# michalfratczak/habdec

Measured on AMD Instinct MI355X. Metric: IQ Msamples/s (batched 2.048 MS/s streams), higher is better.
Workload: dtype f32

## Files before the change

### habdec_amd/csrc/engine.cpp

```cpp
#include <hip/hip_runtime.h>
#include <rocfft/rocfft.h>

#include <algorithm>
#include <atomic>
#include <chrono>
#include <cmath>
#include <cstdio>
#include <cstdlib>
#include <cstring>
#include <memory>
#include <condition_variable>
#include <mutex>
#include <thread>
#include <string>
#include <vector>

#include "../../include/habdec_amd.h"
#include "dev_types.h"
#include "host/afc_tracker.hpp"
#include "host/decim_plan.hpp"
#include "host/fir_design.hpp"
#include "host/iq_file_batch.hpp"
#include "host/text_stage.hpp"
#include "host/tune_host.hpp"
#include "kernels/launch.h"

#define HDK(fn, ...) (e->fast ? hd::fast::fn(__VA_ARGS__) : hd::exact::fn(__VA_ARGS__))

namespace {

thread_local std::string g_err;
int fail(int code, const std::string& msg) { g_err = msg; return code; }

#define HD_HIP(call)                                                                                   \
    do {                                                                                               \
        hipError_t e_ = (call);                                                                        \
        if (e_ != hipSuccess) return fail(HD_ERR_DEVICE, std::string(#call) + ": " + hipGetErrorString(e_)); \
    } while (0)

template <typename T>
struct DevBuf {
    T* p = nullptr;
    size_t n = 0;
    hipError_t alloc(size_t count)
    {
        n = count;
        hipError_t e = hipMalloc(reinterpret_cast<void**>(&p), std::max<size_t>(count, 1) * sizeof(T));
        if (e == hipSuccess) e = hipMemset(p, 0, std::max<size_t>(count, 1) * sizeof(T));
        return e;
    }
    ~DevBuf() { if (p) (void)hipFree(p); }
};
template <typename T>
struct PinBuf {
    T* p = nullptr;
    T* dev = nullptr;
    size_t n = 0;
    hipError_t alloc(size_t count)
    {
        n = count;
        hipError_t e = hipHostMalloc(reinterpret_cast<void**>(&p), std::max<size_t>(count, 1) * sizeof(T), hipHostMallocMapped | hipHostMallocCoherent);
        if (e == hipSuccess) std::memset(p, 0, std::max<size_t>(count, 1) * sizeof(T));
        if (e == hipSuccess) e = hipHostGetDevicePointer(reinterpret_cast<void**>(&dev), p, 0);
        return e;
    }
    ~PinBuf() { if (p) (void)hipHostFree(p); }
};

struct SizeState {
    size_t stage_buf[2] = {0, 0};
    size_t pending = 0;
    size_t fft_fill = 0;
    size_t fir_buf = 0;
    uint32_t fir_T_run = 0;
    uint32_t head_n = 0;
    uint64_t head_call = ~0ull;
    bool head_aside = false;
    uint32_t tune_phase = 0;
    uint32_t front_phase = 0;
    uint32_t win_ub = 0, inflight_m = 0;
    uint32_t last_n2 = 0, last_pend_before = 0, last_m = 0;
    int last_buf = 0;
};

struct StreamHost {
    double baud = 300;
    float lp_bw = 1500, lp_trans = 0.025f;
    bool dc = false;
    hd::LowpassDesigner lp;
    bool taps_dirty = false;
    uint32_t tune_step = 0;
    uint32_t held = 0;
    bool sym_reset = true;
    hd::TextStage text;
    hd::AfcTracker afc;
    hd::SpectrumStats stats{};
    bool have_spectrum = false;
    uint64_t spectra = 0;
    uint32_t last_nbits = 0, last_nflips = 0;
    uint64_t flip_list_full = 0;
    uint64_t bits_total = 0;
    std::vector<uint32_t> last_words;
    uint32_t demod_ck[2] = {0, 0}, demod_ck_n = 0xFFFFFFFFu;
    uint64_t demod_ck_call = 0;
    uint64_t demod_ck_hash = 0xCBF29CE484222325ull;
    uint64_t demod_ck_calls = 0, demod_ck_unknown = 0;
    double tune_hz = 0;
    uint64_t tune_from = 0, retunes = 0;
    bool auto_afc = false;
    double afc_hold_s = 6.0, afc_min_hz = 100.0;
    uint64_t afc_elapsed = 0;
    double front_hz = 0;
    uint32_t front_step = 0;
    uint64_t front_from = 0;
};

}

struct hd_engine {
    hd_engine_config cfg{};
    double fs = 0, fsd = 0;
    std::vector<hd::DecimStage> stages;
    uint32_t S = 0, D = 1;
    uint32_t n1_cap = 0, n2_cap = 0;
    uint32_t taps_cap = 0, fir_hist_cap = 0;
    size_t fbuf_stride = 0;
    uint32_t tail_cap = 0, backlog_cap = 0, slot_words = 0, flips_cap = 0, max_R = 0, min_R = 4;
    int bins_sep = 8;
    bool decode_enabled = true;
    bool fast = false;
    bool one_stream = false;
    bool no_tail = false;
    uint32_t tail_max_n2 = 2048;
    int last_route = -1;
    struct PendingTail { bool valid = false; hd::TailArgs ta{}; int slot = 0; int r2 = 0, t2 = 0; } pend;
    DevBuf<float2> fft_tw;
    bool no_claim = false;
    uint32_t step_run = 0;
    bool no_cu_step = false;
    uint32_t ring_run = 0;
    uint32_t ring_short_pct = 25;
    static constexpr uint32_t kS1Loaders = 2;
#ifndef HD_S1_SLOTS_BATCH
#define HD_S1_SLOTS_BATCH 4
#endif
    static constexpr uint32_t kS1Slots = HD_S1_SLOTS_BATCH;
    PinBuf<unsigned int> ring_gave_up;
    std::string fail_cause;
    bool device_failed = false;
    uint64_t step_launches = 0;
    DevBuf<unsigned int> step_ctr;
    uint32_t pend_max_taps = 0;
    bool dec_wgs_forced = false;
#ifdef HD_TIMING_EXPERIMENT
    int cu_exp = 0;
#else
    static constexpr int cu_exp = 0;
#endif
    uint32_t n_cus = 0, dec_wgs_per_cu = 0;
    hipStream_t qa = nullptr, qb = nullptr, qc = nullptr;
    hipStream_t qh = nullptr;
    DevBuf<float2> staging2;
    hipEvent_t ev_copy[2] = {nullptr, nullptr}, ev_staging_free[2] = {nullptr, nullptr};
    bool staging_used[2] = {false, false};
    uint64_t host_calls = 0, host_calls_in_place = 0;
    uint32_t timing_every = 8;
    hd_timing last_timing{};
    static constexpr uint32_t kLpFftMinTaps = 1024;
    uint32_t lpf_N[2] = {0, 0};
    rocfft_plan lpf_fwd[2] = {nullptr, nullptr}, lpf_inv[2] = {nullptr, nullptr};
    rocfft_execution_info lpf_info = nullptr;
    DevBuf<char> lpf_workbuf;
    DevBuf<float2> lpf_x, lpf_k;
    PinBuf<uint32_t> lpf_ntaps;
    uint32_t lpf_k_N = 0;
    bool lpf_k_stale = true;
    uint64_t lpf_calls = 0;

    DevBuf<float2> staging, dec1, dec1b, dec1c, hist1[2], hist2[2], fbuf[3], fft_in, spec, filtered;
    DevBuf<float> stage_taps[2], lp_taps, power, demod, tail, weight;
    DevBuf<unsigned long long> flipmask;
    DevBuf<uint32_t> flips_dbg;
    DevBuf<hd::SymState> d_symstate;
    DevBuf<hd::DemodCarry> carry[2];
    DevBuf<float2> fir_head;
    DevBuf<float> tune_tab;
    DevBuf<uint32_t> demod_ck_acc;
    uint32_t head_cap = 0;
    DevBuf<hd::SymbolParams> d_sym;
    PinBuf<hd::SymbolParams> h_sym;
    static constexpr int kSlots = 4;
    struct CallSlot {
        DevBuf<hd::StreamCall> d_call;
        PinBuf<hd::StreamCall> h_call;
        PinBuf<uint32_t> h_slots;
        PinBuf<hd::SpectrumStatsDev> h_stats;
        PinBuf<uint2> h_tune;
        PinBuf<uint2> h_front;
        bool timed = false, timed_step = false;
        hipEvent_t ev_front = nullptr, ev_done = nullptr, ev_params = nullptr, ev_spec = nullptr, t0 = nullptr, t1 = nullptr, t2 = nullptr, t3 = nullptr;
        bool busy = false;
        uint32_t seq = 0;
        uint64_t total_in = 0;
        uint32_t r1 = 1;
        ~CallSlot() { for (hipEvent_t ev : {ev_front, ev_done, ev_params, ev_spec, t0, t1, t2, t3}) if (ev) (void)hipEventDestroy(ev); }
    } slot[kSlots];
    uint64_t calls = 0;
    uint64_t delivered = 0;
    int cur = 0;
    int hist_cur = 0;
    int carry_cur = 0;
    bool sym_dirty = true;

    std::vector<StreamHost> st;
    std::vector<SizeState> mirror, mirror_next;
    std::recursive_mutex mtx;
    bool in_callback = false;
    hd_sentence_cb sentence_cb = nullptr; void* sentence_user = nullptr;
    hd_match_cb match_cb = nullptr; void* match_user = nullptr;
    hd_chars_cb chars_cb = nullptr; void* chars_user = nullptr;
    uint64_t sentences_ok = 0;

    ~hd_engine()
    {
        for (rocfft_plan pl : {lpf_fwd[0], lpf_fwd[1], lpf_inv[0], lpf_inv[1]}) if (pl) rocfft_plan_destroy(pl);
        if (lpf_info) rocfft_execution_info_destroy(lpf_info);
        if (qa) (void)hipStreamDestroy(qa);
        if (qb && qb != qa) (void)hipStreamDestroy(qb);
        if (qc && qc != qa) (void)hipStreamDestroy(qc);
        if (qh) (void)hipStreamDestroy(qh);
        for (hipEvent_t ev : {ev_copy[0], ev_copy[1], ev_staging_free[0], ev_staging_free[1]}) if (ev) (void)hipEventDestroy(ev);
    }
};

namespace {

std::once_flag g_rocfft_once;

hd::SymbolParams symbol_params(const hd_engine* e, const StreamHost& s)
{
    hd::SymbolParams p{};
    p.float_abs = e->cfg.lookup_mode ? 1u : 0u;
    p.min_held = 0xFFFFFFFFu;
    p.spb = 0; p.R = 4;
    if (e->fsd > 0 && s.baud > 0) {
        const double spb = std::round(e->fsd / s.baud);
        if (spb >= 1 && spb < 1e9) {
            p.spb = (uint32_t)spb;
            p.R = (uint32_t)std::max(4, int(p.spb / 4));
            p.min_held = (uint32_t)std::ceil(e->fsd / s.baud * 3);
        }
    }
    return p;
}

float cutoff_rel(const hd_engine* e, const StreamHost& s) { return (float)(s.lp_bw / e->fsd); }

int check_stream(const hd_engine* e, uint32_t s)
{
    if (!e) return fail(HD_ERR_INVALID, "null engine");
    if (s >= e->S) return fail(HD_ERR_INVALID, "stream index out of range");
    return HD_OK;
}

}

extern "C" {

const char* hd_last_error(void) { return g_err.c_str(); }

uint32_t hd_min_chunk(uint32_t decimation)
{
    std::vector<hd::DecimStage> st;
    if (!hd::decim_plan(decimation, st)) return 0;
    uint64_t need = decimation ? decimation : 1;
    uint64_t r = 1;
    for (const auto& g : st) { need = std::max<uint64_t>(need, (uint64_t)(g.taps.size() - 1) * r); r *= (uint64_t)g.ratio; }
    const uint64_t d = decimation ? decimation : 1;
    return (uint32_t)((need + d - 1) / d * d);
}

void hd_engine_config_default(hd_engine_config* c)
{
    std::memset(c, 0, sizeof(*c));
    c->device = 0; c->n_streams = 1; c->max_chunk = 65536; c->sampling_rate = 2.048e6; c->decimation = 64;
    c->baud = 300; c->rtty_bits = 8; c->rtty_stops = 2; c->lowpass_bw_hz = 1500; c->lowpass_trans = 0.025f;
    c->dc_remove = 0; c->lookup_mode = 1; c->enable_spectrum = 1; c->ungated = 0; c->keep_filtered = 0; c->pipeline = 0; c->arith = HD_ARITH_EXACT;
}

int hd_engine_create(const hd_engine_config* cfg, hd_engine** out)
{
    if (!cfg || !out) return fail(HD_ERR_INVALID, "null argument");
    *out = nullptr;
    if (cfg->n_streams < 1) return fail(HD_ERR_INVALID, "n_streams must be >= 1");
    if (!(cfg->sampling_rate > 0)) return fail(HD_ERR_INVALID, "sampling_rate must be > 0");
    if (cfg->max_chunk < 1) return fail(HD_ERR_INVALID, "max_chunk must be >= 1");
    if (cfg->arith != HD_ARITH_EXACT && cfg->arith != HD_ARITH_FAST) return fail(HD_ERR_INVALID, "arith must be HD_ARITH_EXACT (0) or HD_ARITH_FAST (1)");
    std::unique_ptr<hd_engine> e(new hd_engine);
    e->cfg = *cfg;
    e->fast = cfg->arith == HD_ARITH_FAST;
    if (!hd::decim_plan(cfg->decimation, e->stages))
        return fail(HD_ERR_INVALID, "Unsupported decimation factor: " + std::to_string(cfg->decimation));
    e->S = cfg->n_streams;
    e->D = cfg->decimation;
    if (cfg->max_chunk % e->D) return fail(HD_ERR_INVALID, "max_chunk must be a multiple of the decimation factor");
    e->fs = (double)(float)cfg->sampling_rate;
    e->fsd = e->fs / (double)e->D;
    e->decode_enabled = cfg->ungated || !(e->fsd > 4 * 40e3);
    if (cfg->baud > 0 && e->fsd / cfg->baud < 3.5)
        return fail(HD_ERR_UNSUPPORTED, "symbol rate above a third of the decimated rate (fewer than 4 samples per bit): the symbol extractor's windows would overlap");
    {
        const float rel = (float)(500.0f / e->fsd);
        e->bins_sep = std::max(8, (int)std::round((double)rel * (double)hd::kFftBins));
    }

    int ndev = 0;
    if (hipGetDeviceCount(&ndev) != hipSuccess || ndev <= cfg->device || cfg->device < 0)
        return fail(HD_ERR_DEVICE, "no HIP device " + std::to_string(cfg->device) + " (this library has no CPU path)");
    HD_HIP(hipSetDevice(cfg->device));
    HD_HIP(hipStreamCreateWithFlags(&e->qa, hipStreamNonBlocking));
    e->one_stream = cfg->pipeline == 0;
    e->no_tail = getenv("HD_NO_TAIL") != nullptr;
    e->no_claim = getenv("HD_NO_CLAIM") != nullptr;
    if (const char* v = getenv("HD_STEP_RUN")) e->step_run = (uint32_t)atoi(v);
    e->no_cu_step = getenv("HD_NO_CU_STEP") != nullptr;
    if (const char* v = getenv("HD_RING_RUN")) e->ring_run = (uint32_t)atoi(v);
    if (const char* v = getenv("HD_RING_SHORT_PCT")) e->ring_short_pct = std::min<uint32_t>((uint32_t)atoi(v), 100u);
    if (const char* v = getenv("HD_TAIL_MAX_N2")) e->tail_max_n2 = (uint32_t)strtoul(v, nullptr, 0);
    {
        hipDeviceProp_t prop;
        HD_HIP(hipGetDeviceProperties(&prop, cfg->device));
        e->n_cus = (uint32_t)prop.multiProcessorCount;
        e->dec_wgs_per_cu = cfg->pipeline ? 6u : 8u;
        if (const char* v = getenv("HD_DEC_WGS_PER_CU")) { e->dec_wgs_per_cu = (uint32_t)atoi(v); e->dec_wgs_forced = true; }
#ifdef HD_TIMING_EXPERIMENT
        if (const char* v = getenv("HD_CU_EXP")) e->cu_exp = atoi(v);
#endif
    }
    for (hipEvent_t* ev : {&e->ev_copy[0], &e->ev_copy[1], &e->ev_staging_free[0], &e->ev_staging_free[1]}) HD_HIP(hipEventCreateWithFlags(ev, hipEventDisableTiming));
    if (e->one_stream) e->qb = e->qc = e->qa;
    else {
        if (!e->qb) HD_HIP(hipStreamCreateWithFlags(&e->qb, hipStreamNonBlocking));
        HD_HIP(hipStreamCreateWithFlags(&e->qc, hipStreamNonBlocking));
    }
    for (auto& sl : e->slot) {
        static const unsigned ev_flags = (unsigned)hipEventDisableSystemFence;
        HD_HIP(hipEventCreateWithFlags(&sl.ev_front, hipEventDisableTiming | ev_flags));
        HD_HIP(hipEventCreateWithFlags(&sl.ev_done, hipEventDisableTiming | ev_flags));
        HD_HIP(hipEventCreateWithFlags(&sl.ev_params, hipEventDisableTiming | ev_flags));
        HD_HIP(hipEventCreateWithFlags(&sl.ev_spec, hipEventDisableTiming | ev_flags));
        for (hipEvent_t* ev : {&sl.t0, &sl.t1, &sl.t2, &sl.t3}) HD_HIP(hipEventCreateWithFlags(ev, ev_flags));
    }

    const uint32_t S = e->S;
    const uint32_t r0 = e->stages.size() > 0 ? e->stages[0].ratio : 1;
    e->n1_cap = cfg->max_chunk / r0;
    e->n2_cap = cfg->max_chunk / e->D;
    const uint32_t m_cap = ((e->n2_cap + hd::kFirBatch - 1) / hd::kFirBatch) * hd::kFirBatch + hd::kFirBatch;
    e->taps_cap = (m_cap | 1u) + 1u;
    e->fir_hist_cap = (e->taps_cap + 1u) & ~1u;
    e->fbuf_stride = (size_t)e->fir_hist_cap + hd::kFirBatch + e->n2_cap + 2;
    e->fbuf_stride = (e->fbuf_stride + 1) & ~(size_t)1;
    e->backlog_cap = hd::kVentLimit + 1 + m_cap;
    e->tail_cap = 1u;
    while (e->tail_cap < hd::kVentLimit + 1 + m_cap + 1024) e->tail_cap <<= 1;

    e->st.resize(S);
    e->mirror.resize(S);
    e->mirror_next.resize(S);
    for (auto& s : e->st) {
        s.baud = cfg->baud; s.lp_bw = cfg->lowpass_bw_hz; s.lp_trans = cfg->lowpass_trans; s.dc = cfg->dc_remove != 0;
        s.text.framer.nbits = cfg->rtty_bits; s.text.framer.nstops = cfg->rtty_stops;
        s.lp.float_trig = cfg->lookup_mode != 0;
    }
    {
        const hd::SymbolParams p = symbol_params(e.get(), e->st[0]);
        const uint32_t spb = std::max<uint32_t>(p.spb, 1);
        uint32_t bits = 3u * e->backlog_cap / spb + 64u;
        bits = std::max<uint32_t>(256u, (bits + 31u) & ~31u);
        e->slot_words = (uint32_t)(sizeof(hd::BitsHeader) / 4) + bits / 32;
        e->max_R = std::max<uint32_t>(p.R, 4);
        e->min_R = e->max_R;
    }
    e->flips_cap = cfg->keep_filtered ? 256 : 0;

    HD_HIP(e->staging.alloc((size_t)S * cfg->max_chunk));
    if (e->stages.size() == 2) for (auto* b : {&e->dec1, &e->dec1b, &e->dec1c}) HD_HIP(b->alloc((size_t)S * e->n1_cap));
    HD_HIP(e->step_ctr.alloc(2 * 16 * 32 + 32));
    HD_HIP(e->ring_gave_up.alloc(4));
    e->ring_gave_up.p[0] = 0;
    if (!e->no_claim && e->n_cus % 32u == 0) {
        const uint32_t n_xcd = e->n_cus / 32u;
        HD_HIP(hipDeviceSynchronize());
        const uint32_t seen = HDK(probe_xcc_mask, e->qa, e->n_cus, e->step_ctr.p + 2 * 16 * 32);
        if (n_xcd > 16 || seen != (n_xcd >= 32 ? 0xFFFFFFFFu : (1u << n_xcd) - 1u)) e->no_claim = true;
    } else
        e->no_claim = true;
    if (e->stages.size() >= 1) {
        for (auto& h : e->hist1) HD_HIP(h.alloc((size_t)S * (e->stages[0].taps.size() - 1)));
        HD_HIP(e->stage_taps[0].alloc(e->stages[0].taps.size() + 1));
        HD_HIP(hipMemcpy(e->stage_taps[0].p, e->stages[0].taps.data(), e->stages[0].taps.size() * 4, hipMemcpyHostToDevice));
    }
    if (e->stages.size() == 2) {
        for (auto& h : e->hist2) HD_HIP(h.alloc((size_t)S * (e->stages[1].taps.size() - 1)));
        HD_HIP(e->stage_taps[1].alloc(e->stages[1].taps.size() + 1));
        HD_HIP(hipMemcpy(e->stage_taps[1].p, e->stages[1].taps.data(), e->stages[1].taps.size() * 4, hipMemcpyHostToDevice));
    }
    for (auto& b : e->fbuf) HD_HIP(b.alloc((size_t)S * e->fbuf_stride));
    HD_HIP(e->lp_taps.alloc((size_t)S * e->taps_cap));
    HD_HIP(e->demod.alloc((size_t)S * m_cap));
    if (cfg->keep_filtered) HD_HIP(e->filtered.alloc((size_t)S * m_cap));
    HD_HIP(e->tail.alloc((size_t)S * e->tail_cap));
    HD_HIP(e->weight.alloc((size_t)S * e->tail_cap));
    HD_HIP(e->flipmask.alloc((size_t)S * (e->tail_cap / 64)));
    HD_HIP(e->d_symstate.alloc(S));
    if (e->flips_cap) HD_HIP(e->flips_dbg.alloc((size_t)S * e->flips_cap));
    for (auto& c : e->carry) HD_HIP(c.alloc(S));
    e->head_cap = std::min<uint32_t>(e->taps_cap, 8192u);
    HD_HIP(e->fir_head.alloc((size_t)S * e->head_cap));
    HD_HIP(e->demod_ck_acc.alloc((size_t)2 * S));
    HD_HIP(e->d_sym.alloc(S));
    HD_HIP(e->h_sym.alloc(S));
    for (auto& sl : e->slot) {
        HD_HIP(sl.d_call.alloc(S));
        HD_HIP(sl.h_call.alloc(S));
        HD_HIP(sl.h_slots.alloc((size_t)S * e->slot_words));
        HD_HIP(sl.h_tune.alloc(S));
        HD_HIP(sl.h_front.alloc(S));
    }
    {
        std::vector<float> tab(4 * hd::kTuneTable);
        hd::tune_tables(tab.data(), tab.data() + 2 * hd::kTuneTable);
        HD_HIP(e->tune_tab.alloc(tab.size()));
        HD_HIP(hipMemcpy(e->tune_tab.p, tab.data(), tab.size() * sizeof(float), hipMemcpyHostToDevice));
    }
    if (cfg->enable_spectrum) {
        HD_HIP(e->fft_in.alloc((size_t)S * hd::kFftBins));
        HD_HIP(e->spec.alloc((size_t)S * hd::kFftBins));
        HD_HIP(e->power.alloc((size_t)S * hd::kFftBins));
        for (auto& sl : e->slot) HD_HIP(sl.h_stats.alloc(S));
        {
            std::vector<float2> tw(hd::kFftBins);
            for (size_t m = 0; m < hd::kFftBins; ++m) {
                const double a = 2.0 * 3.14159265358979323846264338327950288 * (double)m / (double)hd::kFftBins;
                tw[m] = make_float2((float)std::cos(a), (float)-std::sin(a));
            }
            HD_HIP(e->fft_tw.alloc(hd::kFftBins));
            HD_HIP(hipMemcpy(e->fft_tw.p, tw.data(), tw.size() * sizeof(float2), hipMemcpyHostToDevice));
        }
    }
    if (e->fast && e->taps_cap >= hd_engine::kLpFftMinTaps && getenv("HD_NO_LP_FFT") == nullptr) {
        std::call_once(g_rocfft_once, [] { rocfft_setup(); });
        uint32_t N = 1;
        while (N < m_cap + e->taps_cap) N <<= 1;
        e->lpf_N[1] = N; e->lpf_N[0] = N / 2;
        size_t wmax = 0;
        for (int w = 0; w < 2; ++w) {
            const size_t len = e->lpf_N[w];
            if (rocfft_plan_create(&e->lpf_fwd[w], rocfft_placement_inplace, rocfft_transform_type_complex_forward, rocfft_precision_single, 1, &len, S, nullptr) != rocfft_status_success ||
                rocfft_plan_create(&e->lpf_inv[w], rocfft_placement_inplace, rocfft_transform_type_complex_inverse, rocfft_precision_single, 1, &len, S, nullptr) != rocfft_status_success)
                return fail(HD_ERR_DEVICE, "rocfft_plan_create (low-pass transforms) failed");
            for (rocfft_plan pl : {e->lpf_fwd[w], e->lpf_inv[w]}) { size_t wsz = 0; rocfft_plan_get_work_buffer_size(pl, &wsz); wmax = std::max(wmax, wsz); }
        }
        if (rocfft_execution_info_create(&e->lpf_info) != rocfft_status_success) return fail(HD_ERR_DEVICE, "rocfft_execution_info_create failed");
        if (wmax) { HD_HIP(e->lpf_workbuf.alloc(wmax)); rocfft_execution_info_set_work_buffer(e->lpf_info, e->lpf_workbuf.p, wmax); }
        HD_HIP(e->lpf_x.alloc((size_t)S * N));
        HD_HIP(e->lpf_k.alloc((size_t)S * N));
        HD_HIP(e->lpf_ntaps.alloc(S));
    }
    {
        hd_engine::CallSlot& sl = e->slot[0];
        hipStream_t q = e->qa;
        const uint32_t T1 = e->stages.size() > 0 ? (uint32_t)e->stages[0].taps.size() : 0, T2 = e->stages.size() > 1 ? (uint32_t)e->stages[1].taps.size() : 0;
        if (e->stages.empty()) HDK(launch_passthrough, q, S, 1, e->staging.p, cfg->max_chunk, e->fbuf[0].p, e->fbuf_stride, sl.d_call.p, e->fir_hist_cap);
        if (e->stages.size() >= 1)
            HDK(launch_decimate, q, e->stages[0].ratio, T1, S, 1, e->staging.p, cfg->max_chunk, e->hist1[0].p, e->hist1[1].p, e->stage_taps[0].p,
                                e->stages.size() == 1 ? e->fbuf[0].p : e->dec1.p, e->stages.size() == 1 ? e->fbuf_stride : e->n1_cap, sl.d_call.p, 0,
                                e->stages.size() == 1, e->fir_hist_cap, nullptr);
        if (e->stages.size() >= 1)
            HDK(launch_decimate_tuned, q, e->stages[0].ratio, T1, S, 1, e->staging.p, cfg->max_chunk, e->hist1[0].p, e->hist1[1].p, e->stage_taps[0].p,
                                      e->stages.size() == 1 ? e->fbuf[0].p : e->dec1.p, e->stages.size() == 1 ? e->fbuf_stride : e->n1_cap, sl.d_call.p,
                                      e->stages.size() == 1, e->fir_hist_cap, nullptr, 0u, sl.h_front.dev, e->tune_tab.p);
        if (e->stages.size() == 2)
            HDK(launch_decimate, q, e->stages[1].ratio, T2, S, 1, e->dec1.p, e->n1_cap, e->hist2[0].p, e->hist2[1].p, e->stage_taps[1].p, e->fbuf[0].p,
                                e->fbuf_stride, sl.d_call.p, 1, 1, e->fir_hist_cap, nullptr);
        HDK(launch_chunk_post, q, S, e->fbuf[0].p, e->fbuf_stride, sl.d_call.p, e->fir_hist_cap, nullptr, e->tune_tab.p);
        if (cfg->enable_spectrum) {
            HDK(launch_fft_feed, q, S, e->fbuf[0].p, e->fbuf_stride, e->fft_in.p, sl.d_call.p, e->fir_hist_cap);
            hd::launch_spectrum_wave(q, S, e->fft_in.p, e->fft_tw.p, e->spec.p, e->power.p, sl.h_stats.dev, sl.d_call.p, e->fsd, e->bins_sep, 0u);
        }
        HDK(launch_fir_demod, q, S, 0, 0, e->fbuf[0].p, e->fbuf_stride, e->lp_taps.p, e->taps_cap, e->demod.p, e->demod.n / S, nullptr, e->carry[0].p,
                             e->carry[1].p, sl.d_call.p, e->fir_hist_cap, e->tail.p, e->tail_cap, e->d_symstate.p, e->fbuf[1].p,
                             e->fir_head.p, e->head_cap, e->fbuf[2].p);
        HDK(launch_symbols, q, S, 1, 1, e->max_R, e->tail.p, e->tail_cap, e->d_symstate.p, e->flipmask.p, e->weight.p, e->d_sym.p, sl.d_call.p,
                           sl.h_slots.dev, e->slot_words, nullptr, 0, e->min_R, 0u);
        HD_HIP(hipStreamSynchronize(q));
        HD_HIP(hipGetLastError());
        for (auto& h : e->hist1) if (h.p) HD_HIP(hipMemset(h.p, 0, h.n * sizeof(float2)));
        for (auto& h : e->hist2) if (h.p) HD_HIP(hipMemset(h.p, 0, h.n * sizeof(float2)));
        for (auto& c : e->carry) HD_HIP(hipMemset(c.p, 0, c.n * sizeof(hd::DemodCarry)));
        HD_HIP(hipMemset(e->d_symstate.p, 0, S * sizeof(hd::SymState)));
        if (const char* b0 = getenv("HD_SYM_BASE0")) {
            hd::SymState st0{};
            st0.base = st0.cached = st0.run_pos = (uint32_t)strtoul(b0, nullptr, 0);
            std::vector<hd::SymState> v(S, st0);
            HD_HIP(hipMemcpy(e->d_symstate.p, v.data(), S * sizeof(hd::SymState), hipMemcpyHostToDevice));
        }
    }
    HD_HIP(hipDeviceSynchronize());
    *out = e.release();
    return HD_OK;
}

void hd_engine_destroy(hd_engine* e)
{
    if (!e) return;
    (void)hipSetDevice(e->cfg.device);
    (void)hipDeviceSynchronize();
    delete e;
}

uint32_t hd_engine_streams(const hd_engine* e) { return e ? e->S : 0; }
uint32_t hd_engine_decimation(const hd_engine* e) { return e ? e->D : 0; }
double hd_engine_decimated_rate(const hd_engine* e) { return e ? e->fsd : 0; }
uint64_t hd_engine_sentences_ok(const hd_engine* e) { return e ? e->sentences_ok : 0; }
void hd_engine_set_timing(hd_engine* e, int on) { if (e) e->timing_every = on < 0 ? 0u : (uint32_t)on; }
int hd_engine_timing(hd_engine* e, hd_timing* out)
{
    if (!e || !out) return fail(HD_ERR_INVALID, "null argument");
    *out = e->last_timing;
    out->host_calls_in_place = e->host_calls_in_place;
    out->lowpass_fft_calls = e->lpf_calls;
    return HD_OK;
}

extern "C" int hd_debug_step_counters(hd_engine* e, unsigned int* out32)
{
    if (!e || !out32) return HD_ERR_INVALID;
    std::vector<unsigned int> h(2 * 16 * 32);
    if (hipDeviceSynchronize() != hipSuccess || hipMemcpy(h.data(), e->step_ctr.p, h.size() * 4, hipMemcpyDeviceToHost) != hipSuccess) return HD_ERR_DEVICE;
    for (int i = 0; i < 32; ++i) out32[i] = h[(size_t)i * 32];
    return HD_OK;
}

void hd_set_sentence_callback(hd_engine* e, hd_sentence_cb cb, void* user) { if (e) { e->sentence_cb = cb; e->sentence_user = user; } }
void hd_set_match_callback(hd_engine* e, hd_match_cb cb, void* user) { if (e) { e->match_cb = cb; e->match_user = user; } }
void hd_set_chars_callback(hd_engine* e, hd_chars_cb cb, void* user) { if (e) { e->chars_cb = cb; e->chars_user = user; } }


int hd_stream_set_baud(hd_engine* e, uint32_t s, double baud)
{
    if (int r = check_stream(e, s)) return r;
    std::lock_guard<std::recursive_mutex> l(e->mtx);
    if (baud > 0 && e->fsd / baud < 3.5)
        return fail(HD_ERR_UNSUPPORTED, "symbol rate above a third of the decimated rate (fewer than 4 samples per bit): the symbol extractor's windows would overlap");
    StreamHost probe = e->st[s];
    probe.baud = baud;
    const hd::SymbolParams p = symbol_params(e, probe);
    if (p.spb) {
        const uint32_t need = 3u * e->backlog_cap / p.spb + 64u;
        if (need > (e->slot_words - sizeof(hd::BitsHeader) / 4) * 32)
            return fail(HD_ERR_CAPACITY, "baud too high for the result slots sized at engine creation");
        if (p.R > e->max_R) e->max_R = p.R;
        if (p.R < e->min_R) e->min_R = std::max<uint32_t>(p.R, 4);
    }
    e->st[s].baud = baud;
    e->st[s].sym_reset = true;
    e->sym_dirty = true;
    return HD_OK;
}
int hd_stream_set_rtty(hd_engine* e, uint32_t s, uint32_t bits, float stops)
{
    if (int r = check_stream(e, s)) return r;
    std::lock_guard<std::recursive_mutex> l(e->mtx);
    e->st[s].text.framer.nbits = bits;
    e->st[s].text.framer.nstops = stops;
    return HD_OK;
}
int hd_stream_set_lowpass_bw(hd_engine* e, uint32_t s, float hz)
{
    if (int r = check_stream(e, s)) return r;
    std::lock_guard<std::recursive_mutex> l(e->mtx);
    StreamHost& st = e->st[s];
    st.lp_bw = hz;
    if (st.lp.design(cutoff_rel(e, st), st.lp_trans)) st.taps_dirty = true;
    return HD_OK;
}
int hd_stream_set_lowpass_trans(hd_engine* e, uint32_t s, float trans)
{
    if (int r = check_stream(e, s)) return r;
    std::lock_guard<std::recursive_mutex> l(e->mtx);
    StreamHost& st = e->st[s];
    st.lp_trans = trans;
    if (st.lp.design(cutoff_rel(e, st), st.lp_trans)) st.taps_dirty = true;
    return HD_OK;
}
int hd_stream_set_dc_remove(hd_engine* e, uint32_t s, int on)
{
    if (int r = check_stream(e, s)) return r;
    std::lock_guard<std::recursive_mutex> l(e->mtx);
    e->st[s].dc = on != 0;
    return HD_OK;
}
int hd_stream_reset_frequency_correction(hd_engine* e, uint32_t s, double c)
{
    if (int r = check_stream(e, s)) return r;
    std::lock_guard<std::recursive_mutex> l(e->mtx);
    e->st[s].afc.reset(c, hd::kFftBins, e->fsd);
    return HD_OK;
}
int hd_stream_set_tune(hd_engine* e, uint32_t s, double offset_hz)
{
    if (int r = check_stream(e, s)) return r;
    std::lock_guard<std::recursive_mutex> l(e->mtx);
    uint32_t d = 0;
    if (!hd::tune_step(offset_hz, e->fsd, &d)) return fail(HD_ERR_INVALID, "tuning offset outside (-fs_dec/2, fs_dec/2)");
    StreamHost& st = e->st[s];
    st.tune_hz = offset_hz; st.tune_step = d; st.tune_from = e->calls;
    if (offset_hz == 0) e->mirror[s].tune_phase = 0;
    return HD_OK;
}
int hd_stream_set_front_tune(hd_engine* e, uint32_t s, double offset_hz)
{
    if (int r = check_stream(e, s)) return r;
    std::lock_guard<std::recursive_mutex> l(e->mtx);
    if (e->stages.empty()) return fail(HD_ERR_UNSUPPORTED, "an engine without a decimation stage has no input-rate tuning: hd_stream_set_tune is the same thing there");
    uint32_t d = 0;
    if (!hd::tune_step(offset_hz, e->fs, &d)) return fail(HD_ERR_INVALID, "tuning offset outside (-fs/2, fs/2)");
    StreamHost& st = e->st[s];
    st.front_hz = offset_hz; st.front_step = d; st.front_from = e->calls;
// ... 55 lines not shown
    if (!sl.busy) return HD_OK;
    if (e->pend.valid && &e->slot[e->pend.slot] == &sl) { if (const int r = run_pending_tail(e)) return r; }
    const auto w0 = std::chrono::steady_clock::now();
    HD_HIP(hipEventSynchronize(sl.ev_done));
    const auto w1 = std::chrono::steady_clock::now();
    sl.busy = false;
    if (sl.timed) {
        float a = 0, b = 0;
        HD_HIP(hipEventElapsedTime(&b, sl.t1, sl.t2));
        if (sl.timed_step) a = b; else HD_HIP(hipEventElapsedTime(&a, sl.t0, sl.t3));
        e->last_timing.ms_total = a;
        e->last_timing.ms_front = b;
        e->last_timing.samples = sl.total_in;
        e->last_timing.front_bytes = sl.total_in * 8 + (sl.total_in / sl.r1) * 8;
        ++e->last_timing.timed_calls;
    }
    int rc = HD_OK;
    {
        const auto t_lim = std::chrono::steady_clock::now() + std::chrono::milliseconds(200);
        const bool timing_experiment = e->cu_exp != 0;
        auto await = [&](const volatile uint32_t* tag, const char* what, uint32_t s) {
            for (uint32_t spins = 0; *tag != sl.seq; ++spins) {
                if (std::chrono::steady_clock::now() > t_lim) {
                    e->device_failed = true;
                    e->fail_cause = std::string(what) + " of stream " + std::to_string(s) + " does not carry its call's tag 200 ms after the completion event";
                    rc = fail(HD_ERR_DEVICE, e->fail_cause + ": the results of this engine are unreliable -- destroy the engine");
                    return;
                }
                if (spins > 64u) std::this_thread::yield();
            }
        };
        for (uint32_t s = 0; s < e->S && !e->device_failed && !timing_experiment; ++s) {
            await(&reinterpret_cast<const volatile hd::BitsHeader*>(sl.h_slots.p + (size_t)s * e->slot_words)->seq, "result slot", s);
            if (!e->device_failed && e->cfg.enable_spectrum && sl.h_stats.p && sl.h_call.p[s].fft_run)
                await(reinterpret_cast<const volatile uint32_t*>(&sl.h_stats.p[s].seq), "spectrum statistics", s);
        }
        std::atomic_thread_fence(std::memory_order_acquire);
    }
    if (e->ring_gave_up.p && e->ring_gave_up.p[0] && !e->device_failed) {
        e->device_failed = true;
        e->fail_cause = "k_stage1_cu (loader / consumer waves): a bounded wait ran out inside a launch (word " + std::to_string(e->ring_gave_up.p[0]) + ")";
    }
    if (e->device_failed && rc == HD_OK)
        rc = fail(HD_ERR_DEVICE, e->fail_cause + ": the results of this and of every later call of this engine are unreliable -- destroy the engine");
    if (e->device_failed) {
        e->last_timing.host_wait_us = std::chrono::duration<double, std::micro>(w1 - w0).count();
        e->last_timing.host_text_us = 0;
        return rc;
    }
    for (uint32_t s = 0; s < e->S; ++s) {
        StreamHost& st = e->st[s];
        const hd::StreamCall& c = sl.h_call.p[s];
        if (c.fft_run) {
            std::memcpy(&st.stats, &sl.h_stats.p[s], sizeof(st.stats));
            st.have_spectrum = true;
            ++st.spectra;
        }
        const bool past_batch_gate = c.fir_m || c.clear_pending;
        if (past_batch_gate && e->cfg.enable_spectrum) st.afc.step(st.have_spectrum, st.stats, hd::kFftBins, e->fsd);
        st.afc_elapsed += c.n_in;
        if (st.auto_afc && (double)st.afc_elapsed >= st.afc_hold_s * e->fs && std::abs(st.afc.correction) > st.afc_min_hz) {
            const double corr = st.afc.correction;
            uint32_t d = 0;
            if (hd::tune_step(st.tune_hz + corr, e->fsd, &d)) {
                st.tune_hz += corr; st.tune_step = d; st.tune_from = e->calls;
                if (!d) e->mirror[s].tune_phase = 0;
                st.afc.reset(corr, hd::kFftBins, e->fsd);
                st.afc_elapsed = 0;
                ++st.retunes;
            }
        }
        const uint32_t* slot = sl.h_slots.p + (size_t)s * e->slot_words;
        const hd::BitsHeader* hdr = reinterpret_cast<const hd::BitsHeader*>(slot);
        SizeState& sz = e->mirror[s];
        st.held = hdr->held_after;
        sz.inflight_m -= c.fir_m;
        sz.win_ub = hdr->uncached + sz.inflight_m;
        st.last_nbits = hdr->nbits; st.last_nflips = hdr->nflips;
        st.bits_total += hdr->nbits;
        st.demod_ck[0] = hdr->demod_ck[0]; st.demod_ck[1] = hdr->demod_ck[1]; st.demod_ck_n = hdr->demod_n; st.demod_ck_call = e->delivered;
        if (hdr->demod_n != 0xFFFFFFFFu) {
            for (const uint32_t x : {hdr->demod_n, hdr->demod_ck[0], hdr->demod_ck[1]}) st.demod_ck_hash = (st.demod_ck_hash ^ x) * 0x100000001B3ull;
            ++st.demod_ck_calls;
        } else ++st.demod_ck_unknown;
        if (hdr->overflow & 1u) rc = fail(HD_ERR_CAPACITY, "symbol result slot overflow on stream " + std::to_string(s));
        if (hdr->overflow & 2u) ++st.flip_list_full;
        const uint32_t* words = slot + sizeof(hd::BitsHeader) / 4;
        st.last_words.assign(words, words + (hdr->nbits + 31) / 32);
        if (!c.fir_m) continue;
        if (hdr->nbits) st.text.framer.push_packed(words, hdr->nbits);
        const std::string chars = st.text.run(hdr->nbits != 0, [&](const hd::SentenceMatch& m) {
            ++e->sentences_ok;
            if (e->sentence_cb) { e->in_callback = true; e->sentence_cb(e->sentence_user, s, m.callsign.c_str(), m.data.c_str(), m.crc.c_str()); e->in_callback = false; }
        }, [&](const hd::SentenceMatch& m, bool ok) {
            if (e->match_cb) { e->in_callback = true; e->match_cb(e->match_user, s, m.callsign.c_str(), m.data.c_str(), m.crc.c_str(), ok ? 1 : 0); e->in_callback = false; }
        });
        if (!chars.empty() && e->chars_cb) { e->in_callback = true; e->chars_cb(e->chars_user, s, chars.data(), chars.size()); e->in_callback = false; }
    }
    e->last_timing.host_wait_us = std::chrono::duration<double, std::micro>(w1 - w0).count();
    e->last_timing.host_text_us = std::chrono::duration<double, std::micro>(std::chrono::steady_clock::now() - w1).count();
    return rc;
}

int deliver(hd_engine* e, uint64_t depth)
{
    int rc = HD_OK;
    while (e->calls - e->delivered > depth) {
        if (const int r = collect(e, e->slot[e->delivered % hd_engine::kSlots])) rc = r;
        ++e->delivered;
    }
    return rc;
}

int flush_locked(hd_engine* e)
{
    if (e->delivered < e->calls) { if (const int r = run_pending_tail(e)) return r; }
    return deliver(e, 0);
}


enum class Route : uint32_t {
    separate = 0,
    tail = 2,
    step = 3,
};

struct CallPlan {
    size_t nst = 0;
    uint32_t R1 = 1, R2 = 1, T1 = 0, T2 = 0;
    uint32_t max_in = 0, min_in = 0xFFFFFFFFu, max_n1 = 0, max_n2 = 0, max_m = 0, max_taps = 0, max_new = 0, max_pend = 0;
    uint64_t total_in = 0;
    bool any_fft = false, any_dc = false, any_zero1 = false, any_tune = false, any_lp_restart = false;
    bool any_front = false;
};

struct CallRoute {
    Route route = Route::separate;
    int tail_lanes = 64;
    hd::TailArgs ta{}, ta_step{};
    bool lean = false, free_front = false, host_params = false, any_post = false, spectrum_on_qc = false;
    const hd::StreamCall* dcall = nullptr;
    float2* feed = nullptr;
};

struct CallBufs {
    float2 *fcur, *fnext, *fprev, *d1;
    int hin, hout, cin, cout;
};

CallBufs call_bufs(const hd_engine* e)
{
    CallBufs b;
    b.fcur = e->fbuf[e->cur].p; b.fnext = e->fbuf[(e->cur + 1) % 3].p; b.fprev = e->fbuf[(e->cur + 2) % 3].p;
    b.d1 = (e->calls % 3 == 0) ? e->dec1.p : (e->calls % 3 == 1) ? e->dec1b.p : e->dec1c.p;
    b.hin = e->hist_cur; b.hout = e->hist_cur ^ 1;
    b.cin = e->carry_cur; b.cout = e->carry_cur ^ 1;
    return b;
}

int plan_call(hd_engine* e, hd_engine::CallSlot& sl, const uint32_t* n_per_stream, uint32_t n_uniform, CallPlan& p, bool& redesigned)
{
    p = CallPlan{};
    p.nst = e->stages.size();
    if (p.nst > 0) { p.R1 = e->stages[0].ratio; p.T1 = (uint32_t)e->stages[0].taps.size(); }
    if (p.nst > 1) { p.R2 = e->stages[1].ratio; p.T2 = (uint32_t)e->stages[1].taps.size(); }
    redesigned = false;
    for (uint32_t s = 0; s < e->S; ++s) {
        StreamHost& st = e->st[s];
        SizeState& nx = e->mirror_next[s];
        nx = e->mirror[s];
        hd::StreamCall c{};
        const uint32_t n = n_per_stream ? n_per_stream[s] : n_uniform;
        c.n_in = n;
        c.n1 = n / p.R1;
        c.n2 = c.n1 / p.R2;
        if (n) {
            if (p.nst > 0) { const size_t want = (size_t)n + p.T1 + p.R1; if (nx.stage_buf[0] < want) { nx.stage_buf[0] = want; c.zero_hist1 = 1; } }
            if (p.nst > 1) { const size_t want = (size_t)c.n1 + p.T2 + p.R2; if (nx.stage_buf[1] < want) { nx.stage_buf[1] = want; c.zero_hist2 = 1; } }
        }
        c.dc_remove = st.dc && c.n2;
        sl.h_tune.p[s] = make_uint2(st.tune_step, nx.tune_phase);
        if (st.tune_step) { p.any_tune = true; nx.tune_phase += c.n2 * st.tune_step; }
        sl.h_front.p[s] = make_uint2(st.front_step, nx.front_phase);
        if (st.front_step | nx.front_phase) { p.any_front = true; nx.front_phase += n * st.front_step; }
        c.pend_before = (uint32_t)nx.pending;
        nx.pending += c.n2;
        c.fft_fill = (uint32_t)nx.fft_fill;
        if (e->cfg.enable_spectrum && n && nx.fft_fill < (size_t)hd::kFftBins && c.n2) {
            c.fft_take = (uint32_t)std::min<size_t>(hd::kFftBins - nx.fft_fill, c.n2);
            nx.fft_fill += c.fft_take;
        }
        if (e->cfg.enable_spectrum && n && nx.fft_fill >= (size_t)hd::kFftBins) { c.fft_run = 1; nx.fft_fill = 0; p.any_fft = true; }
        const bool past_batch_gate = n && nx.pending >= hd::kFirBatch;
        nx.last_m = 0;
        if (past_batch_gate && !e->decode_enabled) { c.clear_pending = 1; nx.pending = 0; }
        else if (past_batch_gate) {
            const uint32_t m = (uint32_t)(nx.pending - nx.pending % hd::kFirBatch);
            st.lp.batch = m;
            if (st.lp.design(cutoff_rel(e, st), st.lp_trans)) {
                st.taps_dirty = true;
                redesigned = true;
            }
            const uint32_t T = (uint32_t)st.lp.taps.size();
            if (!T) return fail(HD_ERR_UNSUPPORTED, "low-pass transition width leaves no taps (reference filters nothing then)");
            if (T > e->taps_cap) return fail(HD_ERR_CAPACITY, "low-pass tap count exceeds engine capacity");
            if (nx.fir_buf < (size_t)m + T) { nx.fir_buf = (size_t)m + T; c.fir_zero_hist = 1; }
            c.fir_m = m; c.fir_taps = T;
            c.fir_taps_prev = hd::sc_pack_taps_prev(nx.fir_T_run ? nx.fir_T_run : T, nx.head_n, !nx.head_aside && nx.head_call + 1 == e->calls, false);
            nx.fir_T_run = T;
            nx.head_n = std::min<uint32_t>(m, std::min<uint32_t>(e->head_cap, 0x3FFFu)); nx.head_call = e->calls; nx.head_aside = false;
            nx.pending -= m;
            nx.last_m = m;
            p.max_m = std::max(p.max_m, m);
            p.max_taps = std::max(p.max_taps, T);
            p.any_lp_restart |= c.fir_zero_hist != 0;
            const uint32_t pending_windows = st.sym_reset ? std::max(st.held, nx.win_ub) : nx.win_ub;
            p.max_new = std::max(p.max_new, pending_windows + m + 64u);
            nx.inflight_m += m;
            nx.win_ub += m;
        }
        if (!c.fir_m && nx.head_n && !nx.head_aside) {
            if (nx.head_call + 1 == e->calls) c.fir_taps_prev = hd::sc_pack_taps_prev(0, nx.head_n, false, true);
            else nx.head_n = 0;
            nx.head_aside = true;
        }
        c.pend_after = (uint32_t)nx.pending;
        p.max_pend = std::max(p.max_pend, std::max(c.pend_before, c.pend_after));
        nx.last_n2 = c.n2; nx.last_pend_before = c.pend_before; nx.last_buf = e->cur;
        sl.h_call.p[s] = c;
        p.max_in = std::max(p.max_in, n); p.min_in = std::min(p.min_in, n); p.max_n1 = std::max(p.max_n1, c.n1); p.max_n2 = std::max(p.max_n2, c.n2);
        p.any_dc |= c.dc_remove != 0;
        p.any_zero1 |= c.zero_hist1 != 0;
        p.total_in += n;
    }
    sl.total_in = p.total_in;
    sl.r1 = p.R1;
    sl.seq = (uint32_t)(e->calls + 1u);
    if (!sl.seq) sl.seq = 1u;
    return HD_OK;
}

void route_call(hd_engine* e, hd_engine::CallSlot& sl, const CallPlan& p, CallRoute& r)
{
    const uint32_t S = e->S;
    const int R2 = (int)p.R2, T2 = (int)p.T2;
    r = CallRoute{};
    r.tail_lanes = S >= 2 * e->n_cus ? 64 : 256;
    const bool tail = p.nst == 2 && !p.any_dc && !e->no_tail && p.max_n2 <= e->tail_max_n2 &&
                      ((r.tail_lanes == 256 && p.max_n2 >= 512u && HDK(tail_layout, r.ta, r.tail_lanes, R2, T2, p.max_taps, e->max_R, e->min_R, e->tail_cap, p.max_pend, 64 * 1024, 4)) ||
                       HDK(tail_layout, r.ta, r.tail_lanes, R2, T2, p.max_taps, e->max_R, e->min_R, e->tail_cap, p.max_pend, 64 * 1024));
    const uint32_t step_lds = (p.R1 == 32 || p.R1 == 64) ? HDK(step_lds_bytes, (int)p.R1, (int)p.T1) : 0u;
    const bool step = tail && !p.any_front && e->cfg.pipeline && !e->one_stream && p.min_in == p.max_in && p.max_in && step_lds &&
                      HDK(tail_layout, r.ta_step, 64, R2, T2, p.max_taps, e->max_R, e->min_R, e->tail_cap, p.max_pend, step_lds);
    r.route = step ? Route::step : tail ? Route::tail : Route::separate;
    r.any_post = p.any_dc || (p.any_tune && !tail);
    r.lean = tail && !e->one_stream;
    r.free_front = !tail && p.nst == 2 && !e->one_stream;
    r.host_params = tail && !step && e->one_stream;
    r.dcall = r.host_params ? sl.h_call.dev : sl.d_call.p;
    r.feed = (e->cfg.enable_spectrum && !r.any_post) ? e->fft_in.p : nullptr;
    if (r.route != Route::separate || !e->cfg.enable_spectrum || r.any_post || !p.any_fft) return;
    for (uint32_t s = 0; s < S; ++s) {
        hd::StreamCall& c = sl.h_call.p[s];
        if (c.fft_run == 1 && c.fft_fill == 0 && c.fft_take == (uint32_t)hd::kFftBins) { c.fft_take = 0; c.fft_run = 2; }
    }
    r.spectrum_on_qc = !e->one_stream && p.nst != 0;
    for (uint32_t s = 0; s < S && r.spectrum_on_qc; ++s) r.spectrum_on_qc = sl.h_call.p[s].fft_run != 1u;
}

void fill_tail(const hd_engine* e, const hd_engine::CallSlot& sl, const CallPlan& p, const CallRoute& r, const CallBufs& b, hd::TailArgs& t)
{
    t.dec1 = b.d1; t.dec1_stride = e->n1_cap; t.hist2_in = e->hist2[b.hin].p; t.hist2_out = e->hist2[b.hout].p; t.taps2 = e->stage_taps[1].p;
    t.fbuf = b.fcur; t.fbuf_next = b.fnext; t.fbuf_stride = e->fbuf_stride; t.fir_hist_cap = e->fir_hist_cap;
    t.lp_taps = e->lp_taps.p; t.taps_stride = e->taps_cap; t.demod = e->demod.p; t.demod_stride = e->demod.n / e->S;
    t.filtered = e->cfg.keep_filtered ? e->filtered.p : nullptr; t.carry_in = e->carry[b.cin].p; t.carry_out = e->carry[b.cout].p;
    t.tune = p.any_tune ? sl.h_tune.dev : nullptr; t.tune_tab = e->tune_tab.p;
    t.call = r.dcall; t.fft_in = r.feed; t.head_buf = e->fir_head.p; t.fbuf_prev = b.fprev; t.head_cap = e->head_cap;
    t.n_streams = e->S;
    t.ring = e->tail.p; t.ring_cap = e->tail_cap; t.sym = e->d_symstate.p; t.flipmask = e->flipmask.p; t.wsum = e->weight.p;
    t.sp = e->d_sym.p; t.slots = sl.h_slots.dev; t.slot_words = e->slot_words; t.seq = sl.seq;
    t.flips_dbg = e->flips_cap ? e->flips_dbg.p : nullptr; t.flips_cap = e->flips_cap;
    t.fft_tw = r.feed ? e->fft_tw.p : nullptr;
    t.spec = e->spec.p; t.power = e->power.p; t.stats = sl.h_stats.dev; t.rate = e->fsd; t.bins_sep = e->bins_sep;
}

hd::StepClaim make_claim(const hd_engine* e, const CallPlan& p, uint32_t lin_wgs ,
                         uint32_t run_len_cu )
{
    hd::StepClaim claim{};
    const int R1 = (int)p.R1, T1 = (int)p.T1;
    const uint64_t S = e->S;
    const uint32_t ntiles = run_len_cu ? HDK(ring_tiles, R1, T1, p.max_in) : (p.max_n1 + 63) / 64, n_xcd = e->n_cus / 32u, run_len = run_len_cu ? run_len_cu : e->step_run >= 2 ? e->step_run : 4u;
    const uint64_t runs = S * ntiles / run_len;
    const bool shape_ok = run_len_cu ? (HDK(stage1_cu_supported, R1, T1) && p.max_in % 2048u == 0) : ((R1 == 32 || R1 == 64) && p.max_n1 % 64 == 0);
    if (!e->no_claim && (p.nst == 2 || (run_len_cu && p.nst == 1)) && shape_ok && p.min_in == p.max_in && p.max_in && !p.any_zero1 && n_xcd && e->n_cus % 32u == 0 && n_xcd <= 16 &&
        ntiles && (ntiles % run_len == 0 || (run_len_cu && R1 >= 32 && (S * ntiles) % run_len == 0)) && runs % n_xcd == 0 && S * ntiles < (1ull << 32) && (uint64_t)ntiles * S >= 4ull * lin_wgs) {
        claim.ctr = e->step_ctr.p + (size_t)(e->step_launches & 1u) * 16 * 32;
        claim.ctr_next = e->step_ctr.p + (size_t)((e->step_launches & 1u) ^ 1u) * 16 * 32;
        claim.n_xcd = n_xcd; claim.runs_per_xcd = (uint32_t)(runs / n_xcd); claim.run_len = run_len;
        if (run_len_cu && R1 >= 32 && e->ring_short_pct) {
            const uint32_t tpx = claim.runs_per_xcd * run_len, whole = (uint32_t)((uint64_t)tpx * (100u - e->ring_short_pct) / 100u) / run_len;
            claim.tiles_per_xcd = tpx; claim.short_from = whole; claim.runs_per_xcd = whole + (tpx - whole * run_len);
        }
    }
    return claim;
}

uint32_t pick_ring_run(const hd_engine* e, uint32_t R1, uint32_t ntiles)
{
    const uint64_t S = e->S;
    const uint32_t n_xcd = e->n_cus / 32u ? e->n_cus / 32u : 1u, want = R1 >= 32 ? 4u : 8u;
    auto ok = [&](uint32_t r) { return r >= 2u && r <= ntiles && (R1 >= 32 ? (S * ntiles) % r == 0 : ntiles % r == 0) && (S * ntiles / r) % n_xcd == 0; };
    if (e->ring_run >= 2 && ok(e->ring_run)) return e->ring_run;
    for (uint32_t d = 0; d <= 8u; ++d) {
        if (ok(want + d)) return want + d;
        if (d && d < want && ok(want - d)) return want - d;
    }
    return 2u;
}

int enqueue_uploads(hd_engine* e, hd_engine::CallSlot& sl, const CallRoute& r)
{
    const uint32_t S = e->S;
    hipStream_t qa = e->qa;
    if (e->last_route >= 0 && e->last_route != (int)r.route) {
        if (const int rc = run_pending_tail(e)) return rc;
        HD_HIP(hipStreamSynchronize(qa)); HD_HIP(hipStreamSynchronize(e->qb));
    }
    e->last_route = (int)r.route;
    e->last_timing.path = (uint32_t)r.route;
    if (!r.lean && !r.free_front && e->calls >= 2 && !e->one_stream) HD_HIP(hipStreamWaitEvent(qa, e->slot[(e->calls - 2) % hd_engine::kSlots].ev_done, 0));
    const bool step = r.route == Route::step;
    sl.timed = e->timing_every && (e->calls % e->timing_every) == 0;
    sl.timed_step = sl.timed && step;
    if (sl.timed && !step) HD_HIP(hipEventRecord(sl.t0, qa));
    if (!r.lean && !r.free_front && !r.host_params) {
        HDK(launch_fetch_params, e->qc, sl.h_call.dev, sl.d_call.p, S * sizeof(hd::StreamCall));
        if (!e->one_stream) { HD_HIP(hipEventRecord(sl.ev_params, e->qc)); HD_HIP(hipStreamWaitEvent(qa, sl.ev_params, 0)); }
    }
    for (uint32_t s = 0; s < S; ++s) {
        StreamHost& st = e->st[s];
        if (!st.taps_dirty) continue;
        HD_HIP(hipMemcpyAsync(e->lp_taps.p + (size_t)s * e->taps_cap, st.lp.taps.data(), st.lp.taps.size() * 4, hipMemcpyHostToDevice, qa));
        st.taps_dirty = false;
        e->lpf_k_stale = true;
    }
    if (e->sym_dirty) {
        uint32_t mr = 4;
        for (uint32_t s = 0; s < S; ++s) {
            e->h_sym.p[s] = symbol_params(e, e->st[s]);
            e->h_sym.p[s].reset = e->st[s].sym_reset ? 1u : 0u;
            mr = std::max(mr, e->h_sym.p[s].R);
        }
        e->max_R = mr;
        { uint32_t lo = mr; for (uint32_t s2 = 0; s2 < S; ++s2) lo = std::min(lo, std::max<uint32_t>(e->h_sym.p[s2].R, 4)); e->min_R = lo; }
        HD_HIP(hipMemcpyAsync(e->d_sym.p, e->h_sym.p, S * sizeof(hd::SymbolParams), hipMemcpyHostToDevice, qa));
        e->sym_dirty = false;
        for (uint32_t s = 0; s < S; ++s)
            if (e->st[s].sym_reset) { e->st[s].sym_reset = false; e->sym_dirty = true; }
    }
    return HD_OK;
}

int enqueue_step(hd_engine* e, hd_engine::CallSlot& sl, const CallPlan& p, CallRoute& r, const float2* iq, size_t stride)
{
    const uint32_t S = e->S;
    const int R1 = (int)p.R1, T1 = (int)p.T1, R2 = (int)p.R2, T2 = (int)p.T2;
    hipStream_t qa = e->qa;
    const CallBufs b = call_bufs(e);
    const uint32_t ring_nt = HDK(ring_tiles, R1, T1, p.max_in), ring_run = pick_ring_run(e, p.R1, ring_nt), n_xcd = e->n_cus / 32u;
    const bool runs_ok = ring_nt && n_xcd && ring_run >= 2u && ((uint64_t)S * ring_nt) % ring_run == 0 && ((uint64_t)S * ring_nt / ring_run) % n_xcd == 0;
    const bool cu_shape = !e->no_cu_step && !e->no_claim && !p.any_zero1 && p.max_in % 2048u == 0 && runs_ok && HDK(step_cu_supported, R1, T1, R2, T2);
    const uint32_t cu_tail = cu_shape ? HDK(step_cu_tail_lds, R1, T1) : 0u;
    if (cu_tail) {
        hd::TailArgs tacu{};
        if (HDK(tail_layout, tacu, 64, R2, T2, p.max_taps, e->max_R, e->min_R, e->tail_cap, p.max_pend, cu_tail)) r.ta_step = tacu;
    }
    fill_tail(e, sl, p, r, b, r.ta_step);
    hd_engine::PendingTail prev = e->pend;
    hd_engine::CallSlot* ps = prev.valid ? &e->slot[prev.slot] : nullptr;
    const int cu_exp = e->cu_exp;
    const bool want_cu = cu_tail && ((cu_exp & 1) || (r.ta_step.lds_bytes <= cu_tail && (!prev.valid || prev.ta.lds_bytes <= cu_tail)));
    const hd::StepClaim claim = make_claim(e, p, 0, want_cu ? ring_run : 0u);
    bool launched = false;
    if (want_cu && claim.ctr) {
        const uint32_t tb = std::max(r.ta_step.lds_bytes, prev.valid ? prev.ta.lds_bytes : 0u);
        hd::StepClaim cl = claim;
        if (cu_exp & 2) { cl.runs_per_xcd = 0; cl.tiles_per_xcd = 0; cl.short_from = 0xFFFFFFFFu; }
        launched = HDK(launch_step_cu, qa, R1, T1, prev.valid ? prev.r2 : R2, prev.valid ? prev.t2 : T2, S, e->n_cus, iq, stride,
                                      e->hist1[b.hin].p, e->hist1[b.hout].p, e->stage_taps[0].p, b.d1, e->n1_cap, sl.h_call.dev, sl.d_call.p, prev.ta,
                                      (prev.valid && !(cu_exp & 1)) ? S : 0u, p.max_in, cl, tb,
                                      sl.timed ? sl.t1 : nullptr, sl.timed ? sl.t2 : ps ? ps->ev_done : nullptr);
    }
    e->last_timing.step_variant = launched ? 1u : 0u;
    if (launched) ++e->step_launches;
    else {
        if (sl.timed) HD_HIP(hipEventRecord(sl.t1, qa));
        const hd::StepClaim fb = (want_cu && claim.ctr) ? hd::StepClaim{} : claim;
        const uint32_t wgs = (fb.ctr ? 8u : 32u) * e->n_cus;
        if (prev.valid && prev.ta.lds_bytes > HDK(step_lds_bytes, R1, T1)) {
            if (const int rc = run_pending_tail(e)) return rc;
            prev.valid = false; ps = nullptr;
        }
        if (!HDK(launch_step, qa, R1, T1, prev.valid ? prev.r2 : R2, prev.valid ? prev.t2 : T2, S, p.max_n1, iq, stride, e->hist1[b.hin].p,
                             e->hist1[b.hout].p, e->stage_taps[0].p, b.d1, e->n1_cap, sl.h_call.dev, sl.d_call.p, wgs, prev.ta, prev.valid ? S : 0u,
                             p.any_zero1 ? 0u : p.max_in, fb))
            return fail(HD_ERR_INVALID, "no step kernel for this decimation plan");
        if (fb.ctr) ++e->step_launches;
    }
    if (sl.timed && !launched) HD_HIP(hipEventRecord(sl.t2, qa));
    if (ps && (!launched || sl.timed)) HD_HIP(hipEventRecord(ps->ev_done, qa));
    HD_HIP(hipGetLastError());
    return HD_OK;
}

void call_spectrum(hd_engine* e, hipStream_t q, hd_engine::CallSlot& sl, const CallPlan& p, const CallRoute& r)
{
    if (!(e->cfg.enable_spectrum && p.max_n2)) return;
    const float2* fcur = e->fbuf[e->cur].p;
    if (r.any_post || p.nst == 0) HDK(launch_fft_feed, q, e->S, fcur, e->fbuf_stride, e->fft_in.p, r.dcall, e->fir_hist_cap);
    if (!p.any_fft) return;
    hd::launch_spectrum_wave(q, e->S, e->fft_in.p, e->fft_tw.p, e->spec.p, e->power.p, sl.h_stats.dev, r.dcall, e->fsd, e->bins_sep, sl.seq, fcur, e->fbuf_stride, e->fir_hist_cap);
}

int enqueue_front(hd_engine* e, hd_engine::CallSlot& sl, const CallPlan& p, const CallRoute& r, const float2* iq, size_t stride)
{
    const uint32_t S = e->S, R1 = p.R1, T1 = p.T1;
    const bool tail = r.route == Route::tail;
    hipStream_t qa = e->qa;
    const CallBufs b = call_bufs(e);
    if (p.nst == 0) {
        if (sl.timed) HD_HIP(hipEventRecord(sl.t1, qa));
        HDK(launch_passthrough, qa, S, p.max_in, iq, stride, b.fcur, e->fbuf_stride, r.dcall, e->fir_hist_cap);
        if (sl.timed) HD_HIP(hipEventRecord(sl.t2, qa));
    } else {
        const bool single = p.nst == 1;
        float2* out1 = single ? b.fcur : b.d1;
        const size_t out1_stride = single ? e->fbuf_stride : e->n1_cap;
        const uint32_t wgs_cu = (R1 == 64 && !e->dec_wgs_forced && e->dec_wgs_per_cu > 4u) ? 4u : e->dec_wgs_per_cu;
        const uint32_t lin1 = (p.min_in == p.max_in && p.max_in) ? wgs_cu * e->n_cus : 0u;
        bool s1_cu = false;
        if (!p.any_front && (single ? R1 == 4 : R1 != 4) && p.min_in == p.max_in && p.max_in && !e->no_cu_step && !p.any_zero1 && p.max_in % 2048u == 0 && HDK(stage1_cu_supported, (int)R1, (int)T1)) {
            const hd::StepClaim cl = make_claim(e, p, 0, pick_ring_run(e, R1, HDK(ring_tiles, (int)R1, (int)T1, p.max_in)));
            if (cl.ctr) {
                if (sl.timed) HD_HIP(hipEventRecord(sl.t1, qa));
                s1_cu = HDK(launch_stage1_cu, qa, (int)R1, (int)T1, e->n_cus, iq, stride, e->hist1[b.hin].p, e->hist1[b.hout].p, e->stage_taps[0].p, out1, out1_stride,
                                             p.max_in, cl, e->ring_gave_up.dev, hd_engine::kS1Loaders, 16u, (e->cfg.pipeline && !tail && !single) ? hd_engine::kS1Slots : 8u,
                                             single ? r.dcall : nullptr, e->fir_hist_cap, single ? r.feed : nullptr);
                if (s1_cu) ++e->step_launches;
            }
        }
        e->last_timing.step_variant = s1_cu ? 1u : 0u;
        if (!s1_cu) {
            if (sl.timed) HD_HIP(hipEventRecord(sl.t1, qa));
            const hd::StreamCall* call1 = (r.lean || r.free_front) ? sl.h_call.dev : r.dcall;
            if (!(p.any_front ? HDK(launch_decimate_tuned, qa, R1, T1, S, p.max_n1, iq, stride, e->hist1[b.hin].p, e->hist1[b.hout].p, e->stage_taps[0].p, out1, out1_stride,
                                                          call1, single ? 1 : 0, e->fir_hist_cap, single ? r.feed : nullptr, lin1, sl.h_front.dev, e->tune_tab.p)
                              : HDK(launch_decimate, qa, R1, T1, S, p.max_n1, iq, stride, e->hist1[b.hin].p, e->hist1[b.hout].p, e->stage_taps[0].p, out1, out1_stride,
                                                    call1, 0, single ? 1 : 0, e->fir_hist_cap, single ? r.feed : nullptr, lin1)))
                return fail(HD_ERR_INVALID, "no kernel for this decimation stage");
        }
        if (sl.timed) HD_HIP(hipEventRecord(sl.t2, qa));
        if (r.free_front) HDK(launch_fetch_params, qa, sl.h_call.dev, sl.d_call.p, S * sizeof(hd::StreamCall));
        if (!single && !tail) {
            if (!HDK(launch_decimate, qa, p.R2, p.T2, S, p.max_n2, b.d1, e->n1_cap, e->hist2[b.hin].p, e->hist2[b.hout].p, e->stage_taps[1].p, b.fcur,
                                     e->fbuf_stride, r.dcall, 1, 1, e->fir_hist_cap, r.feed))
                return fail(HD_ERR_INVALID, "no kernel for this decimation stage");
        }
    }
    if (!tail) {
        if (r.any_post) HDK(launch_chunk_post, qa, S, b.fcur, e->fbuf_stride, r.dcall, e->fir_hist_cap, p.any_tune ? sl.h_tune.dev : nullptr, e->tune_tab.p);
        if (!r.spectrum_on_qc) call_spectrum(e, qa, sl, p, r);
    }
    if (!e->one_stream) HD_HIP(hipEventRecord(sl.ev_front, qa));
    if (r.spectrum_on_qc) {
        HD_HIP(hipStreamWaitEvent(e->qc, sl.ev_front, 0));
        call_spectrum(e, e->qc, sl, p, r);
        HD_HIP(hipEventRecord(sl.ev_spec, e->qc));
    }
    return HD_OK;
}

int lowpass_transforms(hd_engine* e, const CallPlan& p, const CallRoute& r, const CallBufs& b, uint32_t* lpN)
{
    *lpN = 0;
    if (!e->fast || !e->lpf_N[1] || p.max_taps < hd_engine::kLpFftMinTaps || !p.max_m || p.any_lp_restart) return HD_OK;
    const uint32_t S = e->S, Lmax = p.max_m + p.max_taps - 1;
    const int w = Lmax <= e->lpf_N[0] ? 0 : Lmax <= e->lpf_N[1] ? 1 : -1;
    if (w < 0) return HD_OK;
    const uint32_t N = e->lpf_N[w];
    hipStream_t qb = e->qb;
    rocfft_execution_info_set_stream(e->lpf_info, qb);
    if (e->lpf_k_stale || e->lpf_k_N != N) {
        for (uint32_t s = 0; s < S; ++s) e->lpf_ntaps.p[s] = (uint32_t)e->st[s].lp.taps.size();
        HDK(launch_lp_taps_gather, qb, S, e->lp_taps.p, e->taps_cap, e->lpf_ntaps.dev, e->lpf_k.p, N);
        void* kb[1] = {e->lpf_k.p};
        if (rocfft_execute(e->lpf_fwd[w], kb, nullptr, e->lpf_info) != rocfft_status_success) return fail(HD_ERR_DEVICE, "rocfft_execute (low-pass taps) failed");
        e->lpf_k_N = N; e->lpf_k_stale = false;
    }
    HDK(launch_lp_gather, qb, S, b.fcur, e->fbuf_stride, e->lpf_x.p, N, r.dcall, e->fir_hist_cap, e->fir_head.p, e->head_cap, b.fprev);
    void* xb[1] = {e->lpf_x.p};
    if (rocfft_execute(e->lpf_fwd[w], xb, nullptr, e->lpf_info) != rocfft_status_success) return fail(HD_ERR_DEVICE, "rocfft_execute (low-pass forward) failed");
    HDK(launch_lp_mul, qb, S, e->lpf_x.p, e->lpf_k.p, N, r.dcall);
    if (rocfft_execute(e->lpf_inv[w], xb, nullptr, e->lpf_info) != rocfft_status_success) return fail(HD_ERR_DEVICE, "rocfft_execute (low-pass inverse) failed");
    ++e->lpf_calls;
    *lpN = N;
    return HD_OK;
}

int enqueue_back(hd_engine* e, hd_engine::CallSlot& sl, const CallPlan& p, CallRoute& r)
{
    const uint32_t S = e->S;
    hipStream_t qb = e->qb;
    const CallBufs b = call_bufs(e);
    if (!e->one_stream) HD_HIP(hipStreamWaitEvent(qb, sl.ev_front, 0));
    const bool ev_ride = !sl.timed && e->one_stream;
    if (r.route == Route::tail) {
        if (r.lean) HDK(launch_fetch_params, qb, sl.h_call.dev, sl.d_call.p, S * sizeof(hd::StreamCall));
        fill_tail(e, sl, p, r, b, r.ta);
        if (!HDK(launch_tail, qb, r.tail_lanes, (int)p.R2, (int)p.T2, S, r.ta, ev_ride ? sl.ev_done : nullptr)) return fail(HD_ERR_INVALID, "stream tail refused a shape it was selected for");
    } else {
        uint32_t lpN = 0;
        if (const int rc = lowpass_transforms(e, p, r, b, &lpN)) return rc;
        HDK(launch_fir_demod, qb, S, p.max_m, lpN ? 0u : p.max_taps, b.fcur, e->fbuf_stride, e->lp_taps.p, e->taps_cap, e->demod.p, e->demod.n / S,
                             e->cfg.keep_filtered ? e->filtered.p : nullptr, e->carry[b.cin].p, e->carry[b.cout].p, r.dcall, e->fir_hist_cap,
                             e->tail.p, e->tail_cap, e->d_symstate.p, b.fnext, e->fir_head.p, e->head_cap, b.fprev, e->demod_ck_acc.p,
                             lpN ? e->lpf_x.p : nullptr, lpN, lpN ? 1.0f / (float)lpN : 1.0f);
        HDK(launch_symbols, qb, S, p.max_m, p.max_new, e->max_R, e->tail.p, e->tail_cap, e->d_symstate.p, e->flipmask.p, e->weight.p, e->d_sym.p,
                           r.dcall, sl.h_slots.dev, e->slot_words, e->flips_cap ? e->flips_dbg.p : nullptr, e->flips_cap, e->min_R, sl.seq, ev_ride ? sl.ev_done : nullptr,
                           e->demod_ck_acc.p);
    }
    if (sl.timed) HD_HIP(hipEventRecord(sl.t3, qb));
    if (r.spectrum_on_qc) HD_HIP(hipStreamWaitEvent(qb, sl.ev_spec, 0));
    if (!ev_ride) HD_HIP(hipEventRecord(sl.ev_done, qb));
    HD_HIP(hipGetLastError());
    return HD_OK;
}

void commit_call(hd_engine* e, hd_engine::CallSlot& sl, const CallPlan& p, const CallRoute& r)
{
    e->mirror.swap(e->mirror_next);
    sl.busy = true;
    if (r.route == Route::step) {
        e->pend.valid = true; e->pend.ta = r.ta_step; e->pend.slot = (int)(e->calls % hd_engine::kSlots);
        e->pend.r2 = (int)p.R2; e->pend.t2 = (int)p.T2; e->pend_max_taps = p.max_taps;
    }
    e->cur = (e->cur + 1) % 3;
    e->carry_cur ^= 1;
    if (p.max_in && p.nst) e->hist_cur ^= 1;
    ++e->calls;
}

}

extern "C" {

int hd_flush(hd_engine* e)
{
    if (!e) return fail(HD_ERR_INVALID, "null engine");
    std::lock_guard<std::recursive_mutex> lock(e->mtx);
    if (e->in_callback) return fail(HD_ERR_INVALID, "hd_flush cannot be called from a sentence / character callback (the delivery it would join is the one running)");
    HD_HIP(hipSetDevice(e->cfg.device));
    const int rc = flush_locked(e);
    if (e->device_failed) return fail(HD_ERR_DEVICE, "this engine is in its failed state (" + e->fail_cause + ") -- destroy the engine");
    return rc;
}

int hd_process_device(hd_engine* e, const void* d_iq, size_t stride, const uint32_t* n_per_stream, uint32_t n_uniform)
{
    if (!e) return fail(HD_ERR_INVALID, "null engine");
    if (!d_iq) return fail(HD_ERR_INVALID, "null IQ pointer");
    if ((reinterpret_cast<uintptr_t>(d_iq) & 15) || (stride & 1)) return fail(HD_ERR_INVALID, "IQ base must be 16-byte aligned and stream_stride even");
    std::lock_guard<std::recursive_mutex> lock(e->mtx);
    if (e->in_callback) return fail(HD_ERR_INVALID, "hd_process_* cannot be called from a sentence / character callback");
    if (e->device_failed) return fail(HD_ERR_DEVICE, "this engine is in its failed state (" + e->fail_cause + "): no new calls are accepted -- destroy the engine");
    const auto h0 = std::chrono::steady_clock::now();
    HD_HIP(hipSetDevice(e->cfg.device));
    const size_t nst = e->stages.size();
    const uint32_t T1 = nst > 0 ? (uint32_t)e->stages[0].taps.size() : 0, T2 = nst > 1 ? (uint32_t)e->stages[1].taps.size() : 0;
    const uint32_t R1 = nst > 0 ? e->stages[0].ratio : 1;

    for (uint32_t s = 0; s < e->S; ++s) {
        const uint32_t n = n_per_stream ? n_per_stream[s] : n_uniform;
        if (n > e->cfg.max_chunk) return fail(HD_ERR_CAPACITY, "more samples than max_chunk");
        if (n % e->D) return fail(HD_ERR_INVALID, "sample count must be a multiple of the decimation factor (queue the remainder)");
        if (n && nst > 0 && n + 1 < T1) return fail(HD_ERR_UNSUPPORTED, "chunk shorter than the first stage's history (undefined in the reference)");
        if (n && nst > 1 && n / R1 + 1 < T2) return fail(HD_ERR_UNSUPPORTED, "chunk shorter than the second stage's history (undefined in the reference)");
    }
    if (const int rc = deliver(e, hd_engine::kSlots - 1)) return rc;
    bool tables_dirty = e->sym_dirty;
    for (uint32_t s = 0; s < e->S && !tables_dirty; ++s) tables_dirty = e->st[s].taps_dirty;
    if (tables_dirty) { if (const int rc = flush_locked(e)) return rc; }
    hd_engine::CallSlot& sl = e->slot[e->calls % hd_engine::kSlots];
    CallPlan p;
    bool redesigned = false;
    do {
        if (redesigned) { if (const int rc = flush_locked(e)) return rc; }
        if (const int rc = plan_call(e, sl, n_per_stream, n_uniform, p, redesigned)) return rc;
    } while (redesigned);
    CallRoute r;
    route_call(e, sl, p, r);

    const float2* iq = static_cast<const float2*>(d_iq);
    int rc = enqueue_uploads(e, sl, r);
    if (!rc) rc = r.route == Route::step ? enqueue_step(e, sl, p, r, iq, stride) : enqueue_front(e, sl, p, r, iq, stride);
    if (!rc && r.route != Route::step) rc = enqueue_back(e, sl, p, r);
// ... 299 lines not shown
```

### habdec_amd/csrc/kernels/decimate.hip

```cpp
#include <hip/hip_runtime.h>
#include <hip/hip_ext.h>
#include <type_traits>
#include <cstdlib>

#include "launch.h"
#include "tune.h"
#include "tail_body.h"
#include "stage1_ring.h"

#ifndef HD_FRONT_SWEEPS
#define HD_FRONT_SWEEPS 2
#endif
#define HD_DEC_MAXW 4

namespace hd {
namespace HD_ARITH_NS {

#ifdef HD_STAMP_DEC
#ifndef HD_STAMP_DEC_D
#define HD_STAMP_DEC_D 32
#endif
__device__ unsigned long long g_dec_stamps[4096 * 8];
extern "C" void HD_DBG_NAME(hd_debug_dec_stamps)(unsigned long long* host, size_t n) { (void)hipMemcpyFromSymbol(host, HIP_SYMBOL(g_dec_stamps), n * 8); }
#define DSTAMP_DECL unsigned long long ds_t = __builtin_amdgcn_s_memtime(), ds_acc[4] = {0, 0, 0, 0}; const unsigned long long ds_r0 = __builtin_amdgcn_s_memrealtime(); unsigned long long ds_r1 = 0
// ... 222 lines not shown
        if (claimed && done + 2 == count)
            ticket = draw();
        if (claimed && done + 1 == count) {
            const unsigned int tk = drawn(ticket);
            if (tk == claim.runs_per_xcd) retire();
            if (tk < claim.runs_per_xcd) {
                const uint32_t g0 = (xcd * claim.runs_per_xcd + tk) * claim.run_len;
                pf_s = g0 / lin_ntiles;
                const uint32_t pf_tile = g0 - pf_s * lin_ntiles;
                pf_do = true; pf_which = pf_tile;
                count = (uint32_t)__builtin_amdgcn_readfirstlane((int)(count + claim.run_len));
                jump = true; jump_s = pf_s; jump_first = pf_tile;
            }
        } else
        if (done + 1 < count) {
            uint32_t pf_tile = tile_i + 1;
            if (linear && pf_tile == ntiles) {
                pf_tile = 0; ++pf_s;
                if (!uniform_n) c_next = *reinterpret_cast<const CallHead*>(call + pf_s);
                if constexpr (TUNED) ft.tn_next = ftune[pf_s];
                pf_zero_hist = (stage == 0 ? c_next.zero_hist1 : c_next.zero_hist2) != 0;
            }
            pf_do = true; pf_which = pf_tile;
        }
        if (pf_do) load_tile(pf_which, true);
        DSTAMP(2);

        float2 yq[OPL];
        if constexpr (OPL == 1 && D >= 32 && (D % 16) == 0) {
            constexpr int CH = 16;
            constexpr int NS = T + JS;
            constexpr int NCH = NS / CH;
            static_assert(NCH >= 3, "filter shorter than three chunks");
            static_assert((TO - 1) * (RD + 2) + (NCH * CH + CH - 1) + 2 * ((NCH * CH + CH - 1) / D) < 2 * dec_tile_f4<D, T, TO>(),
                          "the look-ahead read of the last chunk must stay inside the workgroup's LDS");
            f32x2 acc = {0.f, 0.f};
            f32x4 xa[8], xb[8];
            f32x2 ka[8], kb[8];
            auto rd = [&](f32x4 (&x)[8], f32x2 (&k)[8], const int c, auto j0, auto j1) {
                const float2* pc = p + c * CH + 2 * ((c * CH) / D);
#pragma unroll
                for (int q = 0; q < 8; ++q) x[q] = *reinterpret_cast<const f32x4*>(pc + 2 * q);
                const float* tb = taps + (c * CH - JS);
#pragma unroll
                for (int j = 0; j < 16; j += 2) {
                    k[j >> 1].x = (j >= decltype(j0)::value && j < decltype(j1)::value) ? tb[j] : 0.f;
                    k[j >> 1].y = (j + 1 >= decltype(j0)::value && j + 1 < decltype(j1)::value) ? tb[j + 1] : 0.f;
                }
            };
            auto mac_part = [&](const f32x4 (&x)[8], const f32x2 (&k)[8], auto j0, auto j1) {
                HD_FIR_ARITH
#pragma unroll
                for (int j = decltype(j0)::value; j < decltype(j1)::value; ++j) {
                    const f32x2 smp = (j & 1) ? x[j >> 1].zw : x[j >> 1].xy;
                    acc = acc + smp * ((j & 1) ? k[j >> 1].y : k[j >> 1].x);
                }
            };
            using I0 = std::integral_constant<int, 0>;
            using I16 = std::integral_constant<int, 16>;
            using IJS = std::integral_constant<int, JS>;
            using IRem = std::integral_constant<int, NS % CH>;
            rd(xa, ka, 0, IJS{}, I16{});
            rd(xb, kb, 1, I0{}, I16{});
            if constexpr (JS == 0) ring_mac16_asm(acc, xa, ka); else mac_part(xa, ka, IJS{}, I16{});
            int c = 1;
#pragma unroll 1
            for (; c + 1 < NCH; c += 2) {
                rd(xa, ka, c + 1, I0{}, I16{});
                ring_mac16_asm(acc, xb, kb);
                if (c + 2 < NCH) rd(xb, kb, c + 2, I0{}, I16{});
                else rd(xb, kb, NCH, I0{}, IRem{});
                ring_mac16_asm(acc, xa, ka);
            }
            if constexpr ((NCH - 1) % 2) {
                rd(xa, ka, NCH, I0{}, IRem{});
                ring_mac16_asm(acc, xb, kb);
                if constexpr (NS % CH) mac_part(xa, ka, I0{}, IRem{});
            } else {
                if constexpr (NS % CH) mac_part(xb, kb, I0{}, IRem{});
            }
            yq[0] = make_float2(acc.x, acc.y);
        } else
        if constexpr (OPL == 1) {
            float ar = 0.f, ai = 0.f;
            auto mac = [&](float xr, float xi, float k) { HD_FIR_ARITH ar = ar + xr * k; ai = ai + xi * k; };
            constexpr int B = D >= 32 ? 32 : 16;
            constexpr int NS = T + JS;
            constexpr int NFULL = NS / B;
            {
                constexpr int END = NS < B ? NS : B;
    #pragma unroll
                for (int jj = 0; jj + 1 < END + 1; jj += 2) {
                    if (jj + 1 < END || jj < END) {
                        const float4 x = *reinterpret_cast<const float4*>(p + jj + 2 * (jj / D));
                        if (jj >= JS && jj < END) mac(x.x, x.y, taps[jj - JS]);
                        if (jj + 1 < END) mac(x.z, x.w, taps[jj + 1 - JS]);
                    }
                }
            }
            if (NFULL > 1) {
    #pragma unroll 1
                for (int b = 1; b < NFULL; ++b) {
                    const int j0 = b * B;
                    const float2* pb = p + j0 + 2 * (j0 / D);
                    const float* tb = taps + (j0 - JS);
                    float4 x[B / 2];
    #pragma unroll
                    for (int q = 0; q < B / 2; ++q) x[q] = *reinterpret_cast<const float4*>(pb + 2 * q + 2 * ((2 * q) / D));
    #pragma unroll
                    for (int q = 0; q < B / 2; ++q) {
                        mac(x[q].x, x[q].y, tb[2 * q]);
                        mac(x[q].z, x[q].w, tb[2 * q + 1]);
                    }
                }
            }
            if (NS >= B && NS % B) {
                constexpr int J0 = NFULL * B;
    #pragma unroll
                for (int jj = J0; jj < NS; jj += 2) {
                    const float4 x = *reinterpret_cast<const float4*>(p + jj + 2 * (jj / D));
                    mac(x.x, x.y, taps[jj - JS]);
                    if (jj + 1 < NS) mac(x.z, x.w, taps[jj + 1 - JS]);
                }
            }
            yq[0] = make_float2(ar, ai);
        } else {
            float ar[OPL], ai[OPL];
#pragma unroll
            for (int q = 0; q < OPL; ++q) { ar[q] = 0.f; ai[q] = 0.f; }
            constexpr int B = 16;
            constexpr int W = (OPL - 1) * D + T + JS;
            constexpr int NB = (W + B - 1) / B;
            constexpr int B_LO = (JS + (OPL - 1) * D + B - 1) / B;
            constexpr int B_HI = (T + JS) / B - 1;
            auto edge_block = [&](auto bc) {
                HD_FIR_ARITH
                constexpr int j0 = decltype(bc)::value * B;
#pragma unroll
                for (int k = 0; k < B; k += 2) {
                    if (j0 + k < W) {
                        const float4 x = *reinterpret_cast<const float4*>(p + j0 + k + 2 * ((j0 + k) / RD));
#pragma unroll
                        for (int q = 0; q < OPL; ++q) {
                            const int t0 = j0 + k - JS - q * D, t1 = t0 + 1;
                            if (t0 >= 0 && t0 < T) { ar[q] = ar[q] + x.x * taps[t0]; ai[q] = ai[q] + x.y * taps[t0]; }
                            if (t1 >= 0 && t1 < T) { ar[q] = ar[q] + x.z * taps[t1]; ai[q] = ai[q] + x.w * taps[t1]; }
                        }
                    }
                }
            };
            auto for_blocks = [&](auto lo, auto hi, auto self) {
                if constexpr (decltype(lo)::value < decltype(hi)::value) {
                    edge_block(lo);
                    self(std::integral_constant<int, decltype(lo)::value + 1>{}, hi, self);
                }
            };
            constexpr int HEAD_END = B_LO < NB ? (B_LO <= B_HI ? B_LO : NB) : NB;
            for_blocks(std::integral_constant<int, 0>{}, std::integral_constant<int, HEAD_END>{}, for_blocks);
            if constexpr (B_LO <= B_HI) {
#pragma unroll 1
                for (int b = B_LO; b <= B_HI; ++b) {
                    HD_FIR_ARITH
                    const int j0 = b * B;
                    const float2* pb = p + j0 + 2 * (j0 / RD);
                    const float* tb = taps + (j0 - JS);
                    float4 x[B / 2];
#pragma unroll
                    for (int k = 0; k < B / 2; ++k) x[k] = *reinterpret_cast<const float4*>(pb + 2 * k + 2 * ((2 * k) / RD));
#pragma unroll
                    for (int k = 0; k < B / 2; ++k) {
#pragma unroll
                        for (int q = 0; q < OPL; ++q) {
                            const float k0 = tb[2 * k - q * D], k1 = tb[2 * k + 1 - q * D];
                            ar[q] = ar[q] + x[k].x * k0; ai[q] = ai[q] + x[k].y * k0;
                            ar[q] = ar[q] + x[k].z * k1; ai[q] = ai[q] + x[k].w * k1;
                        }
                    }
                }
                for_blocks(std::integral_constant<int, B_HI + 1>{}, std::integral_constant<int, NB>{}, for_blocks);
            }
#pragma unroll
            for (int q = 0; q < OPL; ++q) yq[q] = make_float2(ar[q], ai[q]);
        }
        const uint32_t o = (tile_i * TO + threadIdx.x) * OPL;
#pragma unroll
        for (int q = 0; q < OPL; ++q) { y_prev[q] = yq[q]; ytile[threadIdx.x * OPL + q] = yq[q]; }
        nv_prev = o < nout ? min((uint32_t)OPL, nout - o) : 0u;
        dst_prev = out + (size_t)s * out_stride + (final_stage ? (size_t)fir_hist_cap + c.pend_before : 0) + o;
        nf_prev = (fft_in && o < c.fft_take) ? min((uint32_t)OPL, c.fft_take - o) : 0u;
        fdst_prev = fft_in ? fft_in + (size_t)s * kFftBins + c.fft_fill + o : nullptr;
        __syncthreads();
        DSTAMP(3);
        ++tile_i;
        const bool seam = tile_i == ntiles;
        if (seam) {
            if (n) {
                float2* hout = hist_out + (size_t)s * (T - 1);
                const float2* in_s = in + (size_t)s * in_stride;
                for (uint32_t j = threadIdx.x; j < (uint32_t)(T - 1); j += TO) {
                    const uint32_t idx = n - (T - 1) + j;
                    if constexpr (TUNED) {
                        const uint2 tn = ft.tn;
                        const float2 x = in_s[idx];
                        float yr = x.x, yi = x.y;
                        if (tn.x | tn.y) tune_rotate1(ftab, tn.y + idx * tn.x, x.x, x.y, yr, yi);
                        hout[j] = idx < nout ? ytile[idx] : make_float2(yr, yi);
                    } else
                    hout[j] = idx < nout ? ytile[idx] : in_s[idx];
                }
            }
            if (!jump && done + 1 < count) {
                __syncthreads();
                ++s; tile_i = 0; c = c_next;
                if constexpr (TUNED) ft.tn = ft.tn_next;
                leave_copy(s);
            }
        }
        if (jump) {
            __syncthreads();
            s = jump_s; tile_i = jump_first; jump = false;
            if constexpr (TUNED) ft.tn = ftune[s];
            if (!tile_i) leave_copy(s);
        }
    }
    store_prev();
    flush_copy();
    DSTAMP_WRITE();
}

template <int D, int T, int TO>
__global__ __launch_bounds__(TO) __attribute__((amdgpu_waves_per_eu(D == 64 ? 1 : 2, TO == 64 ? 2 : HD_DEC_MAXW))) void k_decimate(const float2* __restrict__ in, size_t in_stride,
                                                   const float2* __restrict__ hist_in, float2* __restrict__ hist_out,
                                                   const float* __restrict__ taps,
                                                   float2* __restrict__ out, size_t out_stride,
                                                   const StreamCall* __restrict__ call, int stage, int final_stage,
                                                   uint32_t fir_hist_cap, uint32_t tiles_per_wg, float2* __restrict__ fft_in,
                                                   uint32_t n_streams, uint32_t lin_ntiles, StreamCall* __restrict__ call_copy,
                                                   const uint32_t uniform_n, const StepClaim claim)
{
    __shared__ float4 tile4[dec_tile_f4<D, T, TO>()];
    decimate_body<D, T, TO>(in, in_stride, hist_in, hist_out, taps, out, out_stride, call, stage, final_stage, fir_hist_cap, tiles_per_wg, fft_in,
                            n_streams, lin_ntiles, call_copy, blockIdx.x, blockIdx.y, gridDim.x, tile4, TO == 64 ? uniform_n : 0u,
                            TO == 64 ? claim : StepClaim{});
}

template <int TO> constexpr bool front_tab_in_lds()
{
#ifdef HD_FRONT_TAB_GLOBAL
    return false;
#else
    return TO > 64;
#endif
}

template <int D, int T, int TO>
__global__ __launch_bounds__(TO) __attribute__((amdgpu_waves_per_eu(D == 64 ? 1 : 2, TO == 64 ? 2 : HD_DEC_MAXW))) void k_decimate_tuned(const float2* __restrict__ in, size_t in_stride,
                                                   const float2* __restrict__ hist_in, float2* __restrict__ hist_out,
                                                   const float* __restrict__ taps,
                                                   float2* __restrict__ out, size_t out_stride,
                                                   const StreamCall* __restrict__ call, int final_stage,
                                                   uint32_t fir_hist_cap, uint32_t tiles_per_wg, float2* __restrict__ fft_in,
                                                   uint32_t n_streams, uint32_t lin_ntiles,
                                                   const uint2* __restrict__ ftune, const float* __restrict__ ftab)
{
    constexpr bool kLds = front_tab_in_lds<TO>();
    __shared__ float4 tile4[dec_tile_f4<D, T, TO>()];
    __shared__ float4 tab4[kLds ? kTuneTable : 1];
    if constexpr (kLds) {
        for (uint32_t i = threadIdx.x; i < kTuneTable; i += TO) tab4[i] = reinterpret_cast<const float4*>(ftab)[i];
        __syncthreads();
    }
    decimate_body<D, T, TO, true>(in, in_stride, hist_in, hist_out, taps, out, out_stride, call, 0, final_stage, fir_hist_cap, tiles_per_wg, fft_in,
                                  n_streams, lin_ntiles, nullptr, blockIdx.x, blockIdx.y, gridDim.x, tile4, 0u, StepClaim{}, ftune,
                                  kLds ? reinterpret_cast<const float*>(tab4) : ftab);
}

template <int D, int T, int D2, int T2>
__global__ __launch_bounds__(64) __attribute__((amdgpu_waves_per_eu(D == 64 ? 1 : 2, 2))) void k_step(const float2* __restrict__ in, size_t in_stride,
                                                   const float2* __restrict__ hist_in, float2* __restrict__ hist_out,
                                                   const float* __restrict__ taps,
                                                   float2* __restrict__ out, size_t out_stride,
                                                   const StreamCall* __restrict__ call, uint32_t n_streams, uint32_t lin_ntiles,
                                                   StreamCall* __restrict__ call_copy, const TailArgs ta, const uint32_t n_tail,
                                                   const uint32_t uniform_n, const StepClaim claim)
{
    constexpr int kF4 = dec_tile_f4<D, T, 64>() > (int)(kStepLdsBytes / 16) ? dec_tile_f4<D, T, 64>() : (int)(kStepLdsBytes / 16);
    __shared__ float4 tile4[kF4];
    if (blockIdx.x < n_tail) {
#define HD_STEP_PRIO 3
        __builtin_amdgcn_s_setprio(HD_STEP_PRIO);
        tail_body<64, 4, D2, T2>(ta, blockIdx.x, reinterpret_cast<unsigned char*>(tile4));
        return;
    }
    decimate_body<D, T, 64>(in, in_stride, hist_in, hist_out, taps, out, out_stride, call, 0, 0, 0u, 0u, nullptr, n_streams, lin_ntiles, call_copy,
                            blockIdx.x - n_tail, 0u, gridDim.x - n_tail, tile4, uniform_n, claim);
}

template <int T, int D2, int T2>
__global__ __launch_bounds__(512) void k_step_cu(const RingArgs ra, const StreamCall* __restrict__ call, StreamCall* __restrict__ call_copy,
                                                 const TailArgs ta, const uint32_t n_tail, const uint32_t n_streams, const uint32_t tail_bytes )
{
    extern __shared__ __attribute__((aligned(16))) unsigned char cu_lds[];
    RingCtl* ctl = reinterpret_cast<RingCtl*>(cu_lds);
    unsigned char* slots = cu_lds + kRingCtlBytes;
    unsigned char* tails = slots + 4 * kWorkSlotBytes;
    ring_ctl_init(ctl, 0u);
    __syncthreads();
    const uint32_t simd = (__builtin_amdgcn_s_getreg((2 - 1) << 11 | 4 << 6 | 4)) & 3u;
    uint32_t rank = 0;
    if ((threadIdx.x & 63u) == 0) rank = __hip_atomic_fetch_add(&ctl->simd_rank[simd], 1u, __ATOMIC_RELAXED, __HIP_MEMORY_SCOPE_WORKGROUP);
    rank = (uint32_t)__builtin_amdgcn_readfirstlane((int)rank);
    uint32_t w = rank ? 4u + simd : simd;
    if (rank < 2u && (threadIdx.x & 63u) == 0) (void)__hip_atomic_fetch_or(&ctl->roles_taken, 1u << w, __ATOMIC_RELAXED, __HIP_MEMORY_SCOPE_WORKGROUP);
    __syncthreads();
    if (rank >= 2u) {
        uint32_t pick = 0;
        if ((threadIdx.x & 63u) == 0) {
            for (;;) {
                const uint32_t taken = __hip_atomic_load(&ctl->roles_taken, __ATOMIC_RELAXED, __HIP_MEMORY_SCOPE_WORKGROUP);
                pick = (uint32_t)__builtin_ctz(~taken);
                if (!(__hip_atomic_fetch_or(&ctl->roles_taken, 1u << pick, __ATOMIC_RELAXED, __HIP_MEMORY_SCOPE_WORKGROUP) & (1u << pick))) break;
            }
        }
        w = (uint32_t)__builtin_amdgcn_readfirstlane((int)pick);
    }
    if (w < 4u) {
        ring_worker<T>(ra, slots + w * (uint32_t)kWorkSlotBytes, w);
    } else {
        const uint32_t k = w - 4u, lane = threadIdx.x & 63u;
        const uint32_t s = blockIdx.x * 4u + k;
        if (s < n_streams) {
            if (s < n_tail) {
                __builtin_amdgcn_s_setprio(HD_STEP_PRIO);
                tail_body<64, 4, D2, T2>(ta, s, tails + k * tail_bytes);
                __builtin_amdgcn_s_setprio(0);
            }
            if (call_copy && lane < 4) reinterpret_cast<uint4*>(call_copy + s)[lane] = reinterpret_cast<const uint4*>(call + s)[lane];
        }
        ring_worker<T>(ra, n_tail ? tails + k * tail_bytes : slots + w * (uint32_t)kWorkSlotBytes, w);
    }
}

template <int T, int D>
__global__ __launch_bounds__(D == 4 ? 1024 : D == 64 ? 256 : 512) void k_stage1_cu(const RingArgs ra, const uint32_t n_loaders, const uint32_t n_slots )
{
    extern __shared__ __attribute__((aligned(16))) unsigned char cu_lds[];
    if constexpr (D == 32 || D == 64) {
        ring_worker<T, D>(ra, cu_lds + (threadIdx.x >> 6) * (uint32_t)work_slot_bytes<D>(), threadIdx.x >> 6);
    } else {
    unsigned char* ring = cu_lds;
    RingCtl* ctl = reinterpret_cast<RingCtl*>(cu_lds + n_slots * ring_slot_bytes<T>());
    ring_ctl_init(ctl, n_loaders);
    __syncthreads();
    const uint32_t simd = (__builtin_amdgcn_s_getreg((2 - 1) << 11 | 4 << 6 | 4)) & 3u;
    uint32_t rank = 0;
    if ((threadIdx.x & 63u) == 0) rank = __hip_atomic_fetch_add(&ctl->simd_rank[simd], 1u, __ATOMIC_RELAXED, __HIP_MEMORY_SCOPE_WORKGROUP);
    rank = (uint32_t)__builtin_amdgcn_readfirstlane((int)rank);
    uint32_t w = simd < 2u ? (rank ? 2u + simd : simd) : 4u + 2u * (simd - 2u) + rank;
    if (rank < 2u && (threadIdx.x & 63u) == 0) (void)__hip_atomic_fetch_or(&ctl->roles_taken, 1u << w, __ATOMIC_RELAXED, __HIP_MEMORY_SCOPE_WORKGROUP);
    __syncthreads();
    if (rank >= 2u) {
        uint32_t pick = 0;
        if ((threadIdx.x & 63u) == 0) {
            for (;;) {
                const uint32_t taken = __hip_atomic_load(&ctl->roles_taken, __ATOMIC_RELAXED, __HIP_MEMORY_SCOPE_WORKGROUP);
                pick = (uint32_t)__builtin_ctz(~taken);
                if (!(__hip_atomic_fetch_or(&ctl->roles_taken, 1u << pick, __ATOMIC_RELAXED, __HIP_MEMORY_SCOPE_WORKGROUP) & (1u << pick))) break;
            }
        }
        w = (uint32_t)__builtin_amdgcn_readfirstlane((int)pick);
    }
    const RingGeom geom{ring, n_slots};
    const uint32_t h0 = n_slots / 2u;
    if (w < n_loaders) ring_loader<T>(ra, geom, ctl, (n_loaders == 1u || w == 0u) ? 0u : h0, n_loaders == 1u ? n_slots : (w == 0u ? h0 : n_slots - h0), w);
    else ring_consumer<T, D>(ra, geom, ctl, w == 2, w);
    }
}

__global__ void k_xcc_probe(unsigned int* mask)
{
    if (threadIdx.x == 0) atomicOr(mask, 1u << (__builtin_amdgcn_s_getreg((3 << 11) | (0 << 6) | 20) & 15u));
}

__global__ void k_passthrough(const float2* __restrict__ in, size_t in_stride, float2* __restrict__ out, size_t out_stride,
                              const StreamCall* __restrict__ call, uint32_t fir_hist_cap)
{
    const uint32_t s = blockIdx.y;
    const StreamCall c = call[s];
    const uint32_t i = blockIdx.x * blockDim.x + threadIdx.x;
    if (i < c.n_in) out[(size_t)s * out_stride + fir_hist_cap + c.pend_before + i] = in[(size_t)s * in_stride + i];
}

__global__ __launch_bounds__(64) void k_dc_remove(float2* __restrict__ fbuf, size_t stride, const StreamCall* __restrict__ call,
                                                   uint32_t fir_hist_cap, const uint2* __restrict__ tune, const float* __restrict__ tab)
{
    const uint32_t s = blockIdx.x;
    const StreamCall c = call[s];
    const uint2 tn = tune ? tune[s] : make_uint2(0u, 0u);
    const bool dc = c.dc_remove != 0, rot = tn.x != 0u;
    if (!c.n2 || !(dc || rot)) return;
    float2* x = fbuf + (size_t)s * stride + fir_hist_cap + c.pend_before;
    const int lane = threadIdx.x;
    const float2 x0 = x[0];
    float wr = 0.97f * x0.x, wi = 0.97f * x0.y;
    for (uint32_t base = 0; base < c.n2; base += 64) {
        const uint32_t i = base + lane;
        float2 v = i < c.n2 ? x[i] : make_float2(0.f, 0.f);
        float yr = v.x, yi = v.y;
        if (dc) {
            yr = 0.f; yi = 0.f;
#pragma unroll 8
            for (int k = 0; k < 64; ++k) {
                const float xr = __builtin_bit_cast(float, __builtin_amdgcn_readlane(__builtin_bit_cast(int, v.x), k));
                const float xi = __builtin_bit_cast(float, __builtin_amdgcn_readlane(__builtin_bit_cast(int, v.y), k));
                const float sr = 0.97f * wr, si = 0.97f * wi;
                const float nr = xr + sr, ni = xi + si;
                if (lane == k) { yr = nr - wr; yi = ni - wi; }
                if (base + k < c.n2) { wr = nr; wi = ni; }
            }
        }
        if (rot) tune_rotate1(tab, tn.y + i * tn.x, yr, yi, yr, yi);
        if (i < c.n2) x[i] = make_float2(yr, yi);
    }
}

template <int D, int T, int TO, bool TUNED = false>
static void launch_one(hipStream_t st, uint32_t n_streams, uint32_t max_out, const float2* in, size_t in_stride,
                       const float2* hist_in, float2* hist_out, const float* taps, float2* out, size_t out_stride,
                       const StreamCall* call, int stage, int final_stage, uint32_t fir_hist_cap, float2* fft_in, uint32_t lin_wgs, StreamCall* call_copy,
                       uint32_t uniform_n, const StepClaim& claim, const uint2* ftune = nullptr, const float* ftab = nullptr)
{
    constexpr uint32_t TOUT = TO * dec_opl<D>();
    const uint32_t ntiles = (max_out + TOUT - 1) / TOUT;
    if constexpr (TUNED) {
        if (TO == 64 && lin_wgs && (uint64_t)ntiles * n_streams >= 4ull * lin_wgs) {
            hipLaunchKernelGGL((k_decimate_tuned<D, T, TO>), dim3(lin_wgs), dim3(TO), 0, st, in, in_stride, hist_in, hist_out, taps, out, out_stride, call,
                               final_stage, fir_hist_cap, 0u, fft_in, n_streams, ntiles, ftune, ftab);
            return;
        }
        uint32_t per = 1;
        while (per < 16 && (uint64_t)((ntiles + 2 * per - 1) / (2 * per)) * n_streams >= 2048) per *= 2;
        hipLaunchKernelGGL((k_decimate_tuned<D, T, TO>), dim3((ntiles + per - 1) / per, n_streams), dim3(TO), 0, st, in, in_stride, hist_in, hist_out, taps,
                           out, out_stride, call, final_stage, fir_hist_cap, per, fft_in, n_streams, 0u, ftune, ftab);
        return;
    }
    if (TO == 64 && lin_wgs && (uint64_t)ntiles * n_streams >= 4ull * lin_wgs) {
        hipLaunchKernelGGL((k_decimate<D, T, TO>), dim3(lin_wgs), dim3(TO), 0, st, in, in_stride, hist_in, hist_out, taps, out, out_stride, call,
                           stage, final_stage, fir_hist_cap, 0u, fft_in, n_streams, ntiles, call_copy, final_stage ? 0u : uniform_n,
                           (final_stage || !uniform_n) ? StepClaim{} : claim);
        return;
    }
    uint32_t per = 1;
    while (per < 16 && (uint64_t)((ntiles + 2 * per - 1) / (2 * per)) * n_streams >= 2048) per *= 2;
    dim3 grid((ntiles + per - 1) / per, n_streams);
    hipLaunchKernelGGL((k_decimate<D, T, TO>), grid, dim3(TO), 0, st, in, in_stride, hist_in, hist_out, taps, out, out_stride, call,
                       stage, final_stage, fir_hist_cap, per, fft_in, n_streams, 0u, (StreamCall*)nullptr, 0u, StepClaim{});
}

bool launch_decimate(hipStream_t st, int ratio, int ntaps, uint32_t n_streams, uint32_t max_out, const float2* in, size_t in_stride,
                     const float2* hist_in, float2* hist_out, const float* taps, float2* out, size_t out_stride, const StreamCall* call,
                     int stage, int final_stage, uint32_t fir_hist_cap, float2* fft_in, uint32_t lin_wgs, StreamCall* call_copy,
                     uint32_t uniform_n, const StepClaim& claim)
{
    if (!max_out) return true;
#define HD_CASE(D, T, TO) \
    if (ratio == D && ntaps == T) { launch_one<D, T, TO>(st, n_streams, max_out, in, in_stride, hist_in, hist_out, taps, out, out_stride, call, stage, final_stage, fir_hist_cap, fft_in, lin_wgs, call_copy, uniform_n, claim); return true; }
    HD_CASE(2, 69, 256) HD_CASE(4, 139, 256) HD_CASE(8, 280, 256) HD_CASE(8, 54, 256)
    HD_CASE(16, 107, 128) HD_CASE(32, 212, 64) HD_CASE(32, 174, 64) HD_CASE(64, 348, 64)
#undef HD_CASE
    return false;
}

bool launch_decimate_tuned(hipStream_t st, int ratio, int ntaps, uint32_t n_streams, uint32_t max_out, const float2* in, size_t in_stride,
                           const float2* hist_in, float2* hist_out, const float* taps, float2* out, size_t out_stride, const StreamCall* call,
                           int final_stage, uint32_t fir_hist_cap, float2* fft_in, uint32_t lin_wgs, const uint2* ftune, const float* ftab)
{
    if (!max_out) return true;
#define HD_CASE(D, T, TO) \
    if (ratio == D && ntaps == T) { launch_one<D, T, TO, true>(st, n_streams, max_out, in, in_stride, hist_in, hist_out, taps, out, out_stride, call, 0, final_stage, fir_hist_cap, fft_in, lin_wgs, nullptr, 0u, StepClaim{}, ftune, ftab); return true; }
    HD_CASE(2, 69, 256) HD_CASE(4, 139, 256) HD_CASE(8, 280, 256) HD_CASE(8, 54, 256)
    HD_CASE(16, 107, 128) HD_CASE(32, 212, 64) HD_CASE(32, 174, 64) HD_CASE(64, 348, 64)
#undef HD_CASE
    return false;
}

uint32_t step_lds_bytes(int ratio, int ntaps)
{
    auto sz = [](int f4) { return (uint32_t)(f4 > (int)(kStepLdsBytes / 16) ? f4 : (int)(kStepLdsBytes / 16)) * 16u; };
    if (ratio == 32 && ntaps == 212) return sz(dec_tile_f4<32, 212, 64>());
    if (ratio == 32 && ntaps == 174) return sz(dec_tile_f4<32, 174, 64>());
    if (ratio == 64 && ntaps == 348) return sz(dec_tile_f4<64, 348, 64>());
    return 0;
}

bool launch_step(hipStream_t st, int ratio, int ntaps, int ratio2, int ntaps2, uint32_t n_streams, uint32_t n_out, const float2* in, size_t in_stride,
                 const float2* hist_in, float2* hist_out, const float* taps, float2* out, size_t out_stride, const StreamCall* call,
                 StreamCall* call_copy, uint32_t stage1_wgs, const TailArgs& ta, uint32_t n_tail, uint32_t uniform_n, const StepClaim& claim)
{
#define HD_STEP_CASE(D, T, D2, T2)                                                                                                    \
    if (ratio == D && ntaps == T && ratio2 == D2 && ntaps2 == T2) {                                                                   \
        const uint32_t ntiles = (n_out + 63) / 64;                                                                                    \
        hipLaunchKernelGGL((k_step<D, T, D2, T2>), dim3(n_tail + stage1_wgs), dim3(64), 0, st, in, in_stride, hist_in, hist_out, taps, out, \
                           out_stride, call, n_streams, ntiles, call_copy, ta, n_tail, uniform_n, claim);                             \
        return true;                                                                                                                  \
    }
    HD_STEP_CASE(32, 212, 2, 69) HD_STEP_CASE(32, 174, 4, 139) HD_STEP_CASE(64, 348, 4, 139)
#undef HD_STEP_CASE
    return false;
}

uint32_t ring_tiles(int ratio, int ntaps, uint32_t n)
{
    if (ratio != 32 && ratio != 64) return n / 2048u;
    const uint32_t adv = 64u - (uint32_t)((ntaps - 1 + ratio - 1) / ratio), rows = n / (uint32_t)ratio;
    return rows >= 64u ? (rows + adv - 1u) / adv : 0u;
}

static bool ring_limits_ok(uint32_t ntiles, const StepClaim& claim, bool workers = false )
{
    const uint64_t total = claim.tiles_per_xcd ? (uint64_t)claim.tiles_per_xcd * claim.n_xcd : (uint64_t)claim.runs_per_xcd * claim.n_xcd * claim.run_len;
    if (workers) return ntiles && claim.run_len >= 2u && total % ntiles == 0 && total < (1ull << 32) &&
                        (!claim.tiles_per_xcd || (uint64_t)claim.tiles_per_xcd == (uint64_t)(claim.short_from < claim.runs_per_xcd ? claim.short_from : claim.runs_per_xcd) * claim.run_len +
                                                                                    (claim.runs_per_xcd - (claim.short_from < claim.runs_per_xcd ? claim.short_from : claim.runs_per_xcd)));
    return ntiles && ntiles <= 4096u && claim.run_len && ntiles % claim.run_len == 0 && total < (1ull << 24) && total / ntiles <= (1ull << 20);
}

uint32_t step_cu_tail_lds(int ratio, int ntaps)
{
    if (ratio != 32 || (ntaps != 212 && ntaps != 174)) return 0;
    return ((163840u - (uint32_t)kRingCtlBytes - 4u * (uint32_t)kWorkSlotBytes) / 4u) & ~15u;
}

bool launch_step_cu(hipStream_t st, int ratio, int ntaps, int ratio2, int ntaps2, uint32_t n_streams, uint32_t n_cus, const float2* in, size_t in_stride,
                    const float2* hist_in, float2* hist_out, const float* taps, float2* out, size_t out_stride, const StreamCall* call,
                    StreamCall* call_copy, const TailArgs& ta, uint32_t n_tail, uint32_t uniform_n, const StepClaim& claim, uint32_t tail_bytes,
                    hipEvent_t ev_start, hipEvent_t ev_stop)
{
    if (ratio != 32 || !claim.ctr || !uniform_n || uniform_n % 2048u) return false;
    const uint32_t ntiles = ring_tiles(ratio, ntaps, uniform_n);
    if (!ring_limits_ok(ntiles, claim, true)) return false;
    if (tail_bytes < (uint32_t)kWorkSlotBytes) tail_bytes = (uint32_t)kWorkSlotBytes;
    tail_bytes = (tail_bytes + 15u) & ~15u;
    RingArgs ra{in, in_stride, hist_in, hist_out, taps, out, out_stride, uniform_n, ntiles, claim, nullptr, nullptr, 0u, nullptr};
#define HD_CU_CASE(T, D2, T2)                                                                                                         \
    if (ntaps == T && ratio2 == D2 && ntaps2 == T2) {                                                                                 \
        const uint32_t lds = (uint32_t)kRingCtlBytes + (n_tail ? 4u * (uint32_t)kWorkSlotBytes + 4u * tail_bytes : 8u * (uint32_t)kWorkSlotBytes); \
        if (lds > 163840u) return false;                                                                                              \
        static bool attr_set[64] = {};                              \
        int dev_ = 0;                                                                                                                 \
        if (hipGetDevice(&dev_) != hipSuccess || dev_ < 0 || dev_ >= 64) return false;                                                \
        if (!attr_set[dev_]) {                                                                                                        \
            if (hipFuncSetAttribute(reinterpret_cast<const void*>(k_step_cu<T, D2, T2>), hipFuncAttributeMaxDynamicSharedMemorySize, 163840) != hipSuccess) return false; \
            attr_set[dev_] = true;                                                                                                    \
        }                                                                                                                             \
        const dim3 grid_(n_cus > (n_streams + 3u) / 4u ? n_cus : (n_streams + 3u) / 4u);                                             \
             \
        if (ev_start || ev_stop) hipExtLaunchKernelGGL((k_step_cu<T, D2, T2>), grid_, dim3(512), lds, st, ev_start, ev_stop, 0u, ra, call, call_copy, ta, n_tail, n_streams, tail_bytes); \
        else hipLaunchKernelGGL((k_step_cu<T, D2, T2>), grid_, dim3(512), lds, st, ra, call, call_copy, ta, n_tail, n_streams, tail_bytes); \
        return true;                                                                                                                  \
    }
    HD_CU_CASE(212, 2, 69) HD_CU_CASE(174, 4, 139)
#undef HD_CU_CASE
    return false;
}

bool step_cu_supported(int ratio, int ntaps, int ratio2, int ntaps2)
{
    return ratio == 32 && ((ntaps == 212 && ratio2 == 2 && ntaps2 == 69) || (ntaps == 174 && ratio2 == 4 && ntaps2 == 139));
}

bool stage1_cu_supported(int ratio, int ntaps)
{
    return (ratio == 32 && (ntaps == 212 || ntaps == 174)) || (ratio == 64 && ntaps == 348) || (ratio == 8 && ntaps == 54) || (ratio == 4 && ntaps == 139);
}

bool launch_stage1_cu(hipStream_t st, int ratio, int ntaps, uint32_t n_cus, const float2* in, size_t in_stride, const float2* hist_in, float2* hist_out,
                      const float* taps, float2* out, size_t out_stride, uint32_t uniform_n, const StepClaim& claim, unsigned int* gave_up, uint32_t n_loaders, uint32_t n_waves,
                      uint32_t n_slots, const StreamCall* final_call, uint32_t fir_hist_cap, float2* fft_in)
{
    if (n_loaders != 1u) n_loaders = 2u;
    if (ratio <= 4) {
        n_loaders = 1u;
        n_waves = 16u;
    }
    if (n_slots < 2u * n_loaders || n_slots > 8u) n_slots = 8u;
    if (n_waves < 8u || n_waves > 16u) n_waves = 8u;
    if (!claim.ctr || !uniform_n || uniform_n % 2048u) return false;
    const uint32_t ntiles = ring_tiles(ratio, ntaps, uniform_n);
    if (!ring_limits_ok(ntiles, claim, ratio >= 32)) return false;
    if ((ratio <= 4) != (final_call != nullptr)) return false;
    RingArgs ra{in, in_stride, hist_in, hist_out, taps, out, out_stride, uniform_n, ntiles, claim, gave_up, final_call, fir_hist_cap, fft_in};
#define HD_S1_CASE(D, T)                                                                                                              \
    if (ratio == D && ntaps == T) {                                                                                                   \
        static_assert(D >= 32 || (uint32_t)ring_bytes<T, kRingNSLAlone>() <= 163840u, "eight tile slots must fit a CU's LDS");       \
        const uint32_t workers = D == 32 ? 8u : n_slots <= 4u ? 3u : 4u;             \
        const uint32_t lds = D >= 32 ? workers * (uint32_t)work_slot_bytes<(D >= 32 ? D : 32)>() : n_slots * (uint32_t)ring_slot_bytes<T>() + (uint32_t)kRingCtlBytes; \
        static bool attr_set[64] = {};                                                                                                \
        int dev_ = 0;                                                                                                                 \
        if (hipGetDevice(&dev_) != hipSuccess || dev_ < 0 || dev_ >= 64) return false;                                                \
        if (!attr_set[dev_]) {                                                                                                        \
            if (hipFuncSetAttribute(reinterpret_cast<const void*>(k_stage1_cu<T, D>), hipFuncAttributeMaxDynamicSharedMemorySize, 163840) != hipSuccess) return false; \
            attr_set[dev_] = true;                                                                                                    \
        }                                                                                                                             \
        hipLaunchKernelGGL((k_stage1_cu<T, D>), dim3(n_cus), dim3(64u * (D == 4 ? n_waves : D >= 32 ? workers : 8u)), lds, st, ra, n_loaders, n_slots);   \
        return true;                                                                                                                  \
    }
    HD_S1_CASE(32, 212) HD_S1_CASE(32, 174) HD_S1_CASE(64, 348) HD_S1_CASE(8, 54) HD_S1_CASE(4, 139)
#undef HD_S1_CASE
    return false;
}

uint32_t probe_xcc_mask(hipStream_t st, uint32_t n_cus, unsigned int* d_word)
{
    if (hipMemsetAsync(d_word, 0, 4, st) != hipSuccess) return 0;
    hipLaunchKernelGGL(k_xcc_probe, dim3(n_cus * 8u), dim3(64), 0, st, d_word);
    unsigned int h = 0;
    if (hipMemcpyAsync(&h, d_word, 4, hipMemcpyDeviceToHost, st) != hipSuccess || hipStreamSynchronize(st) != hipSuccess) return 0;
    return h;
}

void launch_passthrough(hipStream_t st, uint32_t n_streams, uint32_t max_n, const float2* in, size_t in_stride, float2* out,
                        size_t out_stride, const StreamCall* call, uint32_t fir_hist_cap)
{
    if (!max_n) return;
    dim3 grid((max_n + 255) / 256, n_streams);
    hipLaunchKernelGGL(k_passthrough, grid, dim3(256), 0, st, in, in_stride, out, out_stride, call, fir_hist_cap);
}

void launch_chunk_post(hipStream_t st, uint32_t n_streams, float2* fbuf, size_t stride, const StreamCall* call, uint32_t fir_hist_cap,
                       const uint2* tune, const float* tune_tab)
{
    hipLaunchKernelGGL(k_dc_remove, dim3(n_streams), dim3(64), 0, st, fbuf, stride, call, fir_hist_cap, tune, tune_tab);
}

}
}
```

### habdec_amd/csrc/kernels/launch.h

```cpp
#pragma once
#include <hip/hip_runtime.h>
#include <stddef.h>
#include <stdint.h>

#include "../dev_types.h"

namespace hd {

struct DemodCarry {
    float re, im;
    uint32_t primed;
    uint32_t _pad;
};

struct StepClaim {
    unsigned int* ctr = nullptr;
    unsigned int* ctr_next = nullptr;
    uint32_t n_xcd = 0, runs_per_xcd = 0, run_len = 0;
    uint32_t short_from = 0xFFFFFFFFu, tiles_per_xcd = 0;
};

struct TailArgs {
    const float2* dec1; size_t dec1_stride;
    const float2* hist2_in; float2* hist2_out; const float* taps2;
    float2* fbuf; float2* fbuf_next; size_t fbuf_stride; uint32_t fir_hist_cap;
    const float* lp_taps; uint32_t taps_stride;
    float* demod; size_t demod_stride; float2* filtered;
    const DemodCarry* carry_in; DemodCarry* carry_out;
    const StreamCall* call; float2* fft_in;
    float2* head_buf ; const float2* fbuf_prev ; uint32_t head_cap, n_streams;
    float* ring; uint32_t ring_cap; SymState* sym; unsigned long long* flipmask; float* wsum; const SymbolParams* sp;
    uint32_t* slots; uint32_t slot_words; uint32_t* flips_dbg; uint32_t flips_cap;
    uint32_t seq;
    const float2* fft_tw; float2* spec; float* power; SpectrumStatsDev* stats; double rate; int bins_sep;
    uint32_t pend_max, f_off, v_off, ws_off, words_off, tp_off, h2_off, flips_off, fl_cap, strips_off, dyn_off, lds_bytes;
    uint32_t op;
    const uint2* tune; const float* tune_tab;
};

constexpr uint32_t kStepLdsBytes = 20480;

void launch_spectrum_wave(hipStream_t st, uint32_t n_streams, const float2* fft_in, const float2* tw4096, float2* spec, float* power,
                          SpectrumStatsDev* stats, const StreamCall* call, double rate, int bins_sep,
                          uint32_t seq ,
                          const float2* chunk = nullptr ,
                          size_t chunk_stride = 0, uint32_t fir_hist_cap = 0);

namespace exact {
#include "launch_decls.inc"
}
namespace fast {
#include "launch_decls.inc"
}

}
```

### habdec_amd/csrc/kernels/stage1_ring.h

```cpp
#pragma once
#include <hip/hip_runtime.h>

#include "arith.h"
#include "launch.h"

namespace hd {
namespace HD_ARITH_NS {

typedef float r_f32x2 __attribute__((ext_vector_type(2)));
typedef float r_f32x4 __attribute__((ext_vector_type(4)));

constexpr int kRingRowBytes = 272;
constexpr int kRingNSLAlone = 4;
constexpr int kWorkSlotBytes = 64 * kRingRowBytes;
constexpr int kRingCtlBytes = 384;
constexpr uint32_t kRingSpinLimit = 1u << 22;
template <int T> constexpr int ring_halo_rows() { return (T - 1 + 31) / 32; }
template <int T> constexpr int ring_slot_bytes() { return (64 + ring_halo_rows<T>()) * kRingRowBytes; }
template <int T, int NSL = kRingNSLAlone> constexpr int ring_bytes() { return 2 * NSL * ring_slot_bytes<T>() + kRingCtlBytes; }
template <int T> constexpr int ring_adv() { return 64 - ring_halo_rows<T>(); }

__host__ __device__ constexpr uint32_t ring_sys_tiles(uint32_t n, uint32_t adv) { return (n / 32u + adv - 1u) / adv; }

#ifdef HD_STAMP_RING
__device__ unsigned long long g_ring_stamps[512 * 8 * 8];
extern "C" void HD_DBG_NAME(hd_debug_ring_stamps)(unsigned long long* host, size_t n) { (void)hipMemcpyFromSymbol(host, HIP_SYMBOL(g_ring_stamps), n * 8); }
#define RSTAMP_DECL unsigned long long rs_t = __builtin_amdgcn_s_memtime(), rs_acc[6] = {0, 0, 0, 0, 0, 0}; const unsigned long long rs_r0 = __builtin_amdgcn_s_memrealtime()
#define RSTAMP(i) do { const unsigned long long t_ = __builtin_amdgcn_s_memtime(); rs_acc[i] += t_ - rs_t; rs_t = t_; } while (0)
#define RSTAMP_WRITE(wave_, n_) do { if ((threadIdx.x & 63u) == 0 && blockIdx.x < 512 && (wave_) < 8u) { unsigned long long* g_ = g_ring_stamps + ((size_t)blockIdx.x * 8 + (wave_)) * 8; \
        for (int i_ = 0; i_ < 5; ++i_) g_[i_] = rs_acc[i_]; g_[5] = (n_); g_[6] = rs_r0; g_[7] = __builtin_amdgcn_s_memrealtime(); } } while (0)
#else
#define RSTAMP_DECL do { } while (0)
#define RSTAMP(i) do { } while (0)
#define RSTAMP_WRITE(wave_, n_) do { } while (0)
#endif

#ifdef HD_RING_FAULT
__device__ unsigned int g_ring_fault_fired, g_ring_fault_mode;
static void ring_fault_arm(unsigned int mode) { const unsigned int z = 0; (void)hipMemcpyToSymbol(HIP_SYMBOL(g_ring_fault_mode), &mode, sizeof mode); (void)hipMemcpyToSymbol(HIP_SYMBOL(g_ring_fault_fired), &z, sizeof z); }
extern "C" void HD_DBG_NAME(hd_debug_ring_fault_arm)() { ring_fault_arm(0u); }
extern "C" void HD_DBG_NAME(hd_debug_ring_fault_arm_starve)() { ring_fault_arm(1u); }
#endif

constexpr uint32_t kSlotFree = 0u, kSlotReady = 1u, kSlotTaken = 2u;
struct RingCtl {
    unsigned long long slot[16];
    uint32_t live;
    uint32_t run_tail;
    uint32_t run_head;
    uint32_t _pad0;
    uint32_t run_q[4];
    uint32_t simd_rank[4];
    uint32_t roles_taken;
    uint32_t _pad[3];
};
static_assert(sizeof(RingCtl) <= kRingCtlBytes, "ring control block");
__device__ __forceinline__ void ring_ctl_init(RingCtl* ctl, const uint32_t n_live)
{
    const uint32_t i = threadIdx.x;
    if (i < (uint32_t)kRingCtlBytes / 4u) reinterpret_cast<uint32_t*>(ctl)[i] = i == (uint32_t)offsetof(RingCtl, live) / 4u ? n_live : 0u;
}

struct RingGeom {
    unsigned char* ring; uint32_t nb;
};

struct RingArgs {
    const float2* in; size_t in_stride;
    const float2* hist_in; float2* hist_out;
    const float* taps;
    float2* out; size_t out_stride;
    uint32_t n;
    uint32_t ntiles;
    StepClaim claim;
    unsigned int* gave_up;
    const StreamCall* call; uint32_t fir_hist_cap; float2* fft_in;
};

__device__ __forceinline__ uint32_t lds_addr_of(const void* p)
{
    return (uint32_t)(uintptr_t)(const __attribute__((address_space(3))) void*)p;
}

__device__ __forceinline__ void wait_vmcnt(uint32_t n)
{
#define HD_VMC(k) case k: asm volatile("s_waitcnt vmcnt(" #k ")" ::: "memory"); break;
    switch (n) {
        HD_VMC(0) HD_VMC(1) HD_VMC(2) HD_VMC(3) HD_VMC(4) HD_VMC(5) HD_VMC(6) HD_VMC(7) HD_VMC(8) HD_VMC(9)
        HD_VMC(10) HD_VMC(11) HD_VMC(12) HD_VMC(13) HD_VMC(14) HD_VMC(15) HD_VMC(16) HD_VMC(17) HD_VMC(18) HD_VMC(19)
        HD_VMC(20) HD_VMC(21) HD_VMC(22) HD_VMC(23) HD_VMC(24) HD_VMC(25) HD_VMC(26) HD_VMC(27) HD_VMC(28) HD_VMC(29)
        HD_VMC(30) HD_VMC(31) HD_VMC(32) HD_VMC(33) HD_VMC(34) HD_VMC(35) HD_VMC(36) HD_VMC(37) HD_VMC(38) HD_VMC(39)
        HD_VMC(40) HD_VMC(41) HD_VMC(42) HD_VMC(43) HD_VMC(44) HD_VMC(45) HD_VMC(46) HD_VMC(47) HD_VMC(48) HD_VMC(49)
        HD_VMC(50) HD_VMC(51) HD_VMC(52) HD_VMC(53) HD_VMC(54) HD_VMC(55) HD_VMC(56) HD_VMC(57) HD_VMC(58) HD_VMC(59)
        HD_VMC(60) HD_VMC(61) HD_VMC(62)
        default: asm volatile("s_waitcnt vmcnt(63)" ::: "memory"); break;
    }
#undef HD_VMC
}

__device__ __forceinline__ void glds16(const void* base, uint32_t off, uint32_t lds_dst)
{
    unsigned keep;
    asm volatile("s_mov_b32 %0, m0\n\ts_mov_b32 m0, %3\n\ts_nop 0\n\tglobal_load_lds_dwordx4 %1, %2\n\ts_mov_b32 m0, %0"
                 : "=&s"(keep) : "v"(off), "s"(base), "s"(lds_dst) : "memory");
}
__device__ __forceinline__ void glds4(const void* base, uint32_t off, uint32_t lds_dst)
{
    unsigned keep;
    asm volatile("s_mov_b32 %0, m0\n\ts_mov_b32 m0, %3\n\ts_nop 0\n\tglobal_load_lds_dword %1, %2\n\ts_mov_b32 m0, %0"
                 : "=&s"(keep) : "v"(off), "s"(base), "s"(lds_dst) : "memory");
}

template <bool HEAD_KEPT = false >
__device__ __forceinline__ void glds16_x17(const void* base, const uint32_t (&off)[17], uint32_t lds_dst)
{
    unsigned keep, scc_keep;
#define HD_GLDS_BODY_POLICY " nt"
#define HD_G1(n) "global_load_lds_dwordx4 %" #n ", %19" HD_GLDS_BODY_POLICY "\n\ts_add_u32 m0, m0, 0x400\n\ts_nop 0\n\t"
#define HD_G1D(n) "global_load_lds_dwordx4 %" #n ", %19\n\ts_add_u32 m0, m0, 0x400\n\ts_nop 0\n\t"
#define HD_G17_OPS : "=&s"(keep), "=&s"(scc_keep)                                                                                                                   \
                   : "v"(off[0]), "v"(off[1]), "v"(off[2]), "v"(off[3]), "v"(off[4]), "v"(off[5]), "v"(off[6]), "v"(off[7]), "v"(off[8]), "v"(off[9]),              \
                     "v"(off[10]), "v"(off[11]), "v"(off[12]), "v"(off[13]), "v"(off[14]), "v"(off[15]), "v"(off[16]), "s"(base), "s"(lds_dst)                      \
                   : "memory"
    if constexpr (HEAD_KEPT)
        asm volatile("s_cselect_b32 %1, 1, 0\n\ts_mov_b32 %0, m0\n\ts_mov_b32 m0, %20\n\ts_nop 0\n\t"
                     HD_G1D(2) HD_G1D(3) HD_G1(4) HD_G1(5) HD_G1(6) HD_G1(7) HD_G1(8) HD_G1(9) HD_G1(10) HD_G1(11) HD_G1(12) HD_G1(13) HD_G1(14) HD_G1(15) HD_G1(16) HD_G1D(17)
                     "global_load_lds_dwordx4 %18, %19\n\ts_mov_b32 m0, %0\n\ts_cmp_lg_u32 %1, 0" HD_G17_OPS);
    else
        asm volatile("s_cselect_b32 %1, 1, 0\n\ts_mov_b32 %0, m0\n\ts_mov_b32 m0, %20\n\ts_nop 0\n\t"
                     HD_G1(2) HD_G1(3) HD_G1(4) HD_G1(5) HD_G1(6) HD_G1(7) HD_G1(8) HD_G1(9) HD_G1(10) HD_G1(11) HD_G1(12) HD_G1(13) HD_G1(14) HD_G1(15) HD_G1(16) HD_G1D(17)
                     "global_load_lds_dwordx4 %18, %19\n\ts_mov_b32 m0, %0\n\ts_cmp_lg_u32 %1, 0" HD_G17_OPS);
#undef HD_G17_OPS
#undef HD_G1D
#undef HD_G1
}
template <int HR>
__device__ __forceinline__ void glds4_rows(const void* base, const uint32_t (&off)[HR], uint32_t lds_dst)
{
#pragma unroll
    for (int r = 0; r < HR; ++r) glds4(base, off[r], lds_dst + (uint32_t)r * kRingRowBytes);
}

__device__ __forceinline__ const void* uniform_ptr(const void* p)
{
    const uint64_t b = reinterpret_cast<uint64_t>(p);
    return reinterpret_cast<const void*>(((uint64_t)(uint32_t)__builtin_amdgcn_readfirstlane((int)(uint32_t)(b >> 32)) << 32) |
                                         (uint64_t)(uint32_t)__builtin_amdgcn_readfirstlane((int)(uint32_t)b));
}

template <int T>
__device__ __forceinline__ void ring_loader(const RingArgs& a, const RingGeom& geo, RingCtl* __restrict__ ctl, const uint32_t slot0, const uint32_t nslots,
                                            const uint32_t stamp_row )
{
    constexpr int HR = ring_halo_rows<T>();
    constexpr int SLOT = ring_slot_bytes<T>();
    constexpr int NBODY = 17;
    constexpr int NHALO = (HR * 17 + 63) / 64;
    const uint32_t lane = threadIdx.x & 63u;
    const uint32_t gs = slot0 + lane;
    const uint32_t my_dst = lds_addr_of(geo.ring) + gs * (uint32_t)SLOT;

    uint32_t boff[NBODY], hoff[NHALO], hist_off[HR];
#pragma unroll
    for (int i = 0; i < NBODY; ++i) { const uint32_t P = 64u * i + lane, row = P / 17u, col = P - row * 17u; boff[i] = row * 256u + (col < 16u ? col : 15u) * 16u; }
#pragma unroll
    for (int i = 0; i < NHALO; ++i) {
        uint32_t P = 64u * i + lane; if (P >= (uint32_t)(HR * 17)) P = HR * 17 - 1;
        const uint32_t row = P / 17u, col = P - row * 17u; hoff[i] = row * 256u + (col < 16u ? col : 15u) * 16u;
    }
#pragma unroll
    for (int r = 0; r < HR; ++r) {
        const int h = (r - HR) * 32 + (int)(lane >> 1) + (T - 1);
        hist_off[r] = (uint32_t)(h < 0 ? 0 : h) * 8u + (lane & 1u) * 4u;
    }

    const uint32_t run_len = a.claim.run_len;
    bool have = false, ended = false, claimed = false;
    uint32_t s = 0, tile = 0, left = 0, my_run = 0;
    uint32_t issued = 0, landed = 0;
    uint32_t inflight_instr = 0;
    unsigned long long fifo = 0, sfifo = 0;
    const uint32_t max_fly = nslots >= 3u ? 3u : 2u;
    uint32_t my_state = 0, my_desc = 0;
    uint32_t idle_spins = 0;
    RSTAMP_DECL;

    for (;;) {
        RSTAMP(0);
        unsigned long long w = 0;
        if (lane < nslots) w = __hip_atomic_load(&ctl->slot[gs], __ATOMIC_RELAXED, __HIP_MEMORY_SCOPE_WORKGROUP);
        if (my_state == 2u && (uint32_t)(w >> 32) == kSlotFree) my_state = 0u;
        while (issued != landed) {
            const uint32_t ib = __builtin_amdgcn_s_getreg((32 - 1) << 11 | 0 << 6 | 7);
            const uint32_t oldest = (uint32_t)(fifo & 0xFFu), younger = inflight_instr - oldest;
            if (((ib & 15u) | (((ib >> 22) & 3u) << 4)) > younger) break;
            wait_vmcnt(younger);
            const uint32_t lslot = (uint32_t)(sfifo & 0xFFu) - slot0;
            inflight_instr -= oldest; fifo >>= 8; sfifo >>= 8;
            ++landed;
#ifdef HD_RING_FAULT
            if (landed == 2u && g_ring_fault_mode == 0u) {
                unsigned int won = 1u;
                if (lane == 0) won = atomicCAS(&g_ring_fault_fired, 0u, 1u);
                if ((unsigned int)__builtin_amdgcn_readfirstlane((int)won) == 0u) { RSTAMP_WRITE(stamp_row, issued); return; }
            }
#endif
            if (lane == lslot) {
                __hip_atomic_store(&ctl->slot[gs], ((unsigned long long)kSlotReady << 32) | my_desc, __ATOMIC_RELEASE, __HIP_MEMORY_SCOPE_WORKGROUP);
                my_state = 2u;
            }
        }
        RSTAMP(2);
        if (!have && !ended) {
            if (!claimed) {
                uint32_t idx = 0;
                if (lane == 0) idx = __hip_atomic_fetch_add(&ctl->run_head, 1u, __ATOMIC_RELAXED, __HIP_MEMORY_SCOPE_WORKGROUP);
                my_run = (uint32_t)__builtin_amdgcn_readfirstlane((int)idx);
                claimed = true;
            }
            const uint32_t tail = __hip_atomic_load(&ctl->run_tail, __ATOMIC_ACQUIRE, __HIP_MEMORY_SCOPE_WORKGROUP);
            if ((int32_t)(tail - my_run) > 0) {
                const uint32_t rr = (uint32_t)__builtin_amdgcn_readfirstlane((int)ctl->run_q[my_run & 3u]);
                claimed = false;
                if (rr != 0xFFFFFFFFu) {
                    const uint32_t g0 = rr * run_len;
                    s = g0 / a.ntiles; tile = g0 - s * a.ntiles; left = run_len; have = true;
                } else {
                    ended = true;
                }
            }
        }
        unsigned long long free_mask = 0;
        if (have && issued - landed < max_fly && inflight_instr + (uint32_t)(NBODY + (HR > NHALO ? HR : NHALO)) <= 63u)
            free_mask = __ballot(lane < nslots && my_state == 0u);
        if (free_mask) {
            const uint32_t slot = (uint32_t)__builtin_amdgcn_readfirstlane((int)__builtin_ctzll(free_mask));
            const uint32_t dst = (uint32_t)__builtin_amdgcn_readlane((int)my_dst, (int)slot);
            if (lane == slot) { my_state = 1u; my_desc = (s << 12) | tile; }
            uint32_t cnt = NBODY;
            const unsigned char* body = reinterpret_cast<const unsigned char*>(a.in + (size_t)s * a.in_stride) + (size_t)tile * (64u * 256u);
            if (tile == 0) {
                const unsigned char* hb = reinterpret_cast<const unsigned char*>(a.hist_in + (size_t)s * (T - 1));
                glds4_rows<HR>(hb, hist_off, dst);
                cnt += HR;
            } else {
                const unsigned char* hb = body - HR * 256;
#pragma unroll
                for (int i = 0; i < NHALO; ++i) {
                    if (64 * (i + 1) <= HR * 17 || lane < (uint32_t)(HR * 17 - 64 * i)) glds16(hb, hoff[i], dst + 1024u * i);
                }
                cnt += NHALO;
            }
            glds16_x17(body, boff, dst + (uint32_t)(HR * kRingRowBytes));
            fifo |= (unsigned long long)cnt << (8u * (issued - landed));
            sfifo |= (unsigned long long)(slot0 + slot) << (8u * (issued - landed));
            inflight_instr += cnt;
            ++issued;
            ++tile; --left;
            if (!left) have = false;
            idle_spins = 0;
            RSTAMP(1);
            continue;
        }
        if (!have && ended && issued == landed) break;
        if (issued == landed && ++idle_spins > kRingSpinLimit) {
            if (lane == 0) __hip_atomic_store(a.gave_up, 0x10000u, __ATOMIC_RELAXED, __HIP_MEMORY_SCOPE_SYSTEM);
            break;
        }
        __builtin_amdgcn_s_sleep(1);
        RSTAMP(3);
    }
    if (lane == 0) (void)__hip_atomic_fetch_sub(&ctl->live, 1u, __ATOMIC_RELEASE, __HIP_MEMORY_SCOPE_WORKGROUP);
    RSTAMP_WRITE(stamp_row, issued);
}

__device__ __forceinline__ void ring_mac16_asm(r_f32x2& acc, const r_f32x4 (&x)[8], const r_f32x2 (&kp)[8])
{
#ifdef HD_FAST_ARITH
#define HD_FMA_E(xi, ki) "v_pk_fma_f32 %0, %" #xi ", %" #ki ", %0 op_sel_hi:[1,0,1]\n\t"
#define HD_FMA_O(xi, ki) "v_pk_fma_f32 %0, %" #xi ", %" #ki ", %0 op_sel:[0,1,0]\n\t"
    asm volatile(
        HD_FMA_E(1, 17) HD_FMA_O(2, 17) HD_FMA_E(3, 18) HD_FMA_O(4, 18) HD_FMA_E(5, 19) HD_FMA_O(6, 19) HD_FMA_E(7, 20) HD_FMA_O(8, 20)
        HD_FMA_E(9, 21) HD_FMA_O(10, 21) HD_FMA_E(11, 22) HD_FMA_O(12, 22) HD_FMA_E(13, 23) HD_FMA_O(14, 23) HD_FMA_E(15, 24) "v_pk_fma_f32 %0, %16, %24, %0 op_sel:[0,1,0]"
        : "+v"(acc)
        : "v"(x[0].xy), "v"(x[0].zw), "v"(x[1].xy), "v"(x[1].zw), "v"(x[2].xy), "v"(x[2].zw), "v"(x[3].xy), "v"(x[3].zw),
          "v"(x[4].xy), "v"(x[4].zw), "v"(x[5].xy), "v"(x[5].zw), "v"(x[6].xy), "v"(x[6].zw), "v"(x[7].xy), "v"(x[7].zw),
          "s"(kp[0]), "s"(kp[1]), "s"(kp[2]), "s"(kp[3]), "s"(kp[4]), "s"(kp[5]), "s"(kp[6]), "s"(kp[7]));
#undef HD_FMA_E
#undef HD_FMA_O
#else
    r_f32x2 t0, t1, t2, t3;
#define HD_MUL_E(t, xi, ki) "v_pk_mul_f32 %" #t ", %" #xi ", %" #ki " op_sel_hi:[1,0]\n\t"
#define HD_MUL_O(t, xi, ki) "v_pk_mul_f32 %" #t ", %" #xi ", %" #ki " op_sel:[0,1]\n\t"
#define HD_ADD(t) "v_pk_add_f32 %0, %0, %" #t "\n\t"
    asm volatile(
        HD_MUL_E(1, 5, 21) HD_MUL_O(2, 6, 21) HD_MUL_E(3, 7, 22)
        HD_ADD(1) HD_MUL_O(4, 8, 22)
        HD_ADD(2) HD_MUL_E(1, 9, 23)
        HD_ADD(3) HD_MUL_O(2, 10, 23)
        HD_ADD(4) HD_MUL_E(3, 11, 24)
        HD_ADD(1) HD_MUL_O(4, 12, 24)
        HD_ADD(2) HD_MUL_E(1, 13, 25)
        HD_ADD(3) HD_MUL_O(2, 14, 25)
        HD_ADD(4) HD_MUL_E(3, 15, 26)
        HD_ADD(1) HD_MUL_O(4, 16, 26)
        HD_ADD(2) HD_MUL_E(1, 17, 27)
        HD_ADD(3) HD_MUL_O(2, 18, 27)
        HD_ADD(4) HD_MUL_E(3, 19, 28)
        HD_ADD(1) HD_MUL_O(4, 20, 28)
        HD_ADD(2) HD_ADD(3) "v_pk_add_f32 %0, %0, %4"
        : "+v"(acc), "=&v"(t0), "=&v"(t1), "=&v"(t2), "=&v"(t3)
        : "v"(x[0].xy), "v"(x[0].zw), "v"(x[1].xy), "v"(x[1].zw), "v"(x[2].xy), "v"(x[2].zw), "v"(x[3].xy), "v"(x[3].zw),
          "v"(x[4].xy), "v"(x[4].zw), "v"(x[5].xy), "v"(x[5].zw), "v"(x[6].xy), "v"(x[6].zw), "v"(x[7].xy), "v"(x[7].zw),
          "s"(kp[0]), "s"(kp[1]), "s"(kp[2]), "s"(kp[3]), "s"(kp[4]), "s"(kp[5]), "s"(kp[6]), "s"(kp[7]));
#undef HD_MUL_E
#undef HD_MUL_O
#undef HD_ADD
#endif
}
#ifdef HD_FAST_ARITH
__device__ __forceinline__ void ring_fma16x2(r_f32x2& a, r_f32x2& b, const r_f32x4 (&x)[8], const r_f32x2 (&kp)[8])
{
#define HD_FMA_A(xi, ki) "v_pk_fma_f32 %0, %" #xi ", %" #ki ", %0 op_sel_hi:[1,0,1]\n\t"
#define HD_FMA_B(xi, ki) "v_pk_fma_f32 %1, %" #xi ", %" #ki ", %1 op_sel:[0,1,0]\n\t"
    asm volatile(
        HD_FMA_A(2, 18) HD_FMA_B(3, 18) HD_FMA_A(4, 19) HD_FMA_B(5, 19) HD_FMA_A(6, 20) HD_FMA_B(7, 20) HD_FMA_A(8, 21) HD_FMA_B(9, 21)
        HD_FMA_A(10, 22) HD_FMA_B(11, 22) HD_FMA_A(12, 23) HD_FMA_B(13, 23) HD_FMA_A(14, 24) HD_FMA_B(15, 24) HD_FMA_A(16, 25) "v_pk_fma_f32 %1, %17, %25, %1 op_sel:[0,1,0]"
        : "+v"(a), "+v"(b)
        : "v"(x[0].xy), "v"(x[0].zw), "v"(x[1].xy), "v"(x[1].zw), "v"(x[2].xy), "v"(x[2].zw), "v"(x[3].xy), "v"(x[3].zw),
          "v"(x[4].xy), "v"(x[4].zw), "v"(x[5].xy), "v"(x[5].zw), "v"(x[6].xy), "v"(x[6].zw), "v"(x[7].xy), "v"(x[7].zw),
          "s"(kp[0]), "s"(kp[1]), "s"(kp[2]), "s"(kp[3]), "s"(kp[4]), "s"(kp[5]), "s"(kp[6]), "s"(kp[7]));
#undef HD_FMA_A
#undef HD_FMA_B
}
#endif

template <bool ODD>
__device__ __forceinline__ void ring_slot8(r_f32x2 (&acc)[8], const r_f32x2 smp, const r_f32x2 k0, const r_f32x2 k1, const r_f32x2 k2, const r_f32x2 k3,
                                           const r_f32x2 k4, const r_f32x2 k5, const r_f32x2 k6, const r_f32x2 k7)
{
#ifdef HD_FAST_ARITH
#define HD_S8_FMA(a, k) "v_pk_fma_f32 %" #a ", %8, %" #k ", %" #a " op_sel_hi:[1,0,1]\n\t"
#define HD_S8_FMAO(a, k) "v_pk_fma_f32 %" #a ", %8, %" #k ", %" #a " op_sel:[0,1,0]\n\t"
#define HD_S8F_OPS : "+v"(acc[0]), "+v"(acc[1]), "+v"(acc[2]), "+v"(acc[3]), "+v"(acc[4]), "+v"(acc[5]), "+v"(acc[6]), "+v"(acc[7])                      \
                   : "v"(smp), "s"(k0), "s"(k1), "s"(k2), "s"(k3), "s"(k4), "s"(k5), "s"(k6), "s"(k7)
    if constexpr (ODD)
        asm volatile(HD_S8_FMAO(0, 9) HD_S8_FMAO(1, 10) HD_S8_FMAO(2, 11) HD_S8_FMAO(3, 12) HD_S8_FMAO(4, 13) HD_S8_FMAO(5, 14) HD_S8_FMAO(6, 15) "v_pk_fma_f32 %7, %8, %16, %7 op_sel:[0,1,0]" HD_S8F_OPS);
    else
        asm volatile(HD_S8_FMA(0, 9) HD_S8_FMA(1, 10) HD_S8_FMA(2, 11) HD_S8_FMA(3, 12) HD_S8_FMA(4, 13) HD_S8_FMA(5, 14) HD_S8_FMA(6, 15) "v_pk_fma_f32 %7, %8, %16, %7 op_sel_hi:[1,0,1]" HD_S8F_OPS);
#undef HD_S8_FMA
#undef HD_S8_FMAO
#undef HD_S8F_OPS
#else
    r_f32x2 t0, t1, t2, t3, t4, t5, t6, t7;
#define HD_S8_MUL(t, k) "v_pk_mul_f32 %" #t ", %16, %" #k " op_sel_hi:[1,0]\n\t"
#define HD_S8_MULO(t, k) "v_pk_mul_f32 %" #t ", %16, %" #k " op_sel:[0,1]\n\t"
#define HD_S8_ADDS "v_pk_add_f32 %0, %0, %8\n\tv_pk_add_f32 %1, %1, %9\n\tv_pk_add_f32 %2, %2, %10\n\tv_pk_add_f32 %3, %3, %11\n\t" \
                   "v_pk_add_f32 %4, %4, %12\n\tv_pk_add_f32 %5, %5, %13\n\tv_pk_add_f32 %6, %6, %14\n\tv_pk_add_f32 %7, %7, %15"
#define HD_S8_OPS : "+v"(acc[0]), "+v"(acc[1]), "+v"(acc[2]), "+v"(acc[3]), "+v"(acc[4]), "+v"(acc[5]), "+v"(acc[6]), "+v"(acc[7]),                       \
                    "=&v"(t0), "=&v"(t1), "=&v"(t2), "=&v"(t3), "=&v"(t4), "=&v"(t5), "=&v"(t6), "=&v"(t7)                                            \
                  : "v"(smp), "s"(k0), "s"(k1), "s"(k2), "s"(k3), "s"(k4), "s"(k5), "s"(k6), "s"(k7)
    if constexpr (ODD)
        asm volatile(HD_S8_MULO(8, 17) HD_S8_MULO(9, 18) HD_S8_MULO(10, 19) HD_S8_MULO(11, 20) HD_S8_MULO(12, 21) HD_S8_MULO(13, 22) HD_S8_MULO(14, 23) HD_S8_MULO(15, 24) HD_S8_ADDS HD_S8_OPS);
    else
        asm volatile(HD_S8_MUL(8, 17) HD_S8_MUL(9, 18) HD_S8_MUL(10, 19) HD_S8_MUL(11, 20) HD_S8_MUL(12, 21) HD_S8_MUL(13, 22) HD_S8_MUL(14, 23) HD_S8_MUL(15, 24) HD_S8_ADDS HD_S8_OPS);
#undef HD_S8_MUL
#undef HD_S8_MULO
#undef HD_S8_ADDS
#undef HD_S8_OPS
#endif
}
template <bool ODD>
__device__ __forceinline__ void ring_slot1(r_f32x2& acc, const r_f32x2 smp, const r_f32x2 k)
{
#ifdef HD_FAST_ARITH
    if constexpr (ODD) asm volatile("v_pk_fma_f32 %0, %1, %2, %0 op_sel:[0,1,0]" : "+v"(acc) : "v"(smp), "s"(k));
    else asm volatile("v_pk_fma_f32 %0, %1, %2, %0 op_sel_hi:[1,0,1]" : "+v"(acc) : "v"(smp), "s"(k));
#else
    r_f32x2 t;
    if constexpr (ODD) asm volatile("v_pk_mul_f32 %1, %2, %3 op_sel:[0,1]\n\tv_pk_add_f32 %0, %0, %1" : "+v"(acc), "=&v"(t) : "v"(smp), "s"(k));
    else asm volatile("v_pk_mul_f32 %1, %2, %3 op_sel_hi:[1,0]\n\tv_pk_add_f32 %0, %0, %1" : "+v"(acc), "=&v"(t) : "v"(smp), "s"(k));
#endif
}

template <class F, int... I>
__device__ __forceinline__ void ring_for_each_index(F&& f, std::integer_sequence<int, I...>) { (f(std::integral_constant<int, I>{}), ...); }

template <int T, int D>
__device__ __forceinline__ void ring_consumer(const RingArgs& a, const RingGeom& geo, RingCtl* __restrict__ ctl, const bool feeder,
                                              const uint32_t role )
{
    constexpr int HR = ring_halo_rows<T>();
    constexpr int JS = HR * 32 - (T - 1);
    constexpr int C0 = JS / 16;
    static_assert(D == 16 || D == 8 || D == 4 || D == 2, "a lane's row of 32 samples is 32 / D outputs (the /32 stages run ring_worker)");
    static_assert(T <= 64 || (32 / D) % 8 == 0, "long filters of the small ratios: outputs in groups of eight");
    const uint32_t lane = threadIdx.x & 63u;
    typedef const float __attribute__((address_space(4)))* ctaps_t;
    const ctaps_t taps = (ctaps_t)(uintptr_t)a.taps - JS;
    auto coff = [](int c) { return (c >> 1) * kRingRowBytes + (c & 1) * 128; };
    RSTAMP_DECL;
#ifdef HD_STAMP_RING
    uint32_t n_done = 0;
#endif
    const uint32_t my_wave = role; (void)my_wave;
    const bool feeding = feeder;
    uint32_t fed = 0;
#ifdef HD_RING_FAULT
    uint32_t starving = 0;
#endif
    bool exhausted = false;
    const uint32_t xcd0 = __builtin_amdgcn_s_getreg((3 << 11) | (0 << 6) | 20) & 15u;
    const uint32_t xcd = xcd0 < a.claim.n_xcd ? xcd0 : a.claim.n_xcd - 1;
    unsigned int* my_ctr = a.claim.ctr + (size_t)xcd * 32;
    unsigned int* next_ctr = a.claim.ctr_next + (size_t)xcd * 32;
    auto feed = [&]() {
        while (feeding) {
            const uint32_t head = __hip_atomic_load(&ctl->run_head, __ATOMIC_ACQUIRE, __HIP_MEMORY_SCOPE_WORKGROUP);
            if ((int32_t)(fed - head) >= 2) break;
            uint32_t v = 0xFFFFFFFFu;
            if (!exhausted) {
#ifdef HD_RING_FAULT
                if (fed >= 2u && g_ring_fault_mode == 1u) {
                    if (!starving) { unsigned int won = 1u; if (lane == 0) won = atomicCAS(&g_ring_fault_fired, 0u, 1u); starving = (unsigned int)__builtin_amdgcn_readfirstlane((int)won) == 0u ? 1u : 2u; }
                    if (starving == 1u) break;
                }
#endif
                unsigned int t = 0;
                if (lane == 0) t = __hip_atomic_fetch_add(my_ctr, 1u, __ATOMIC_RELAXED, __HIP_MEMORY_SCOPE_AGENT);
                t = (unsigned int)__builtin_amdgcn_readfirstlane((int)t);
                if (t == a.claim.runs_per_xcd && lane == 0) (void)__hip_atomic_exchange(next_ctr, 0u, __ATOMIC_RELAXED, __HIP_MEMORY_SCOPE_AGENT);
                if (t < a.claim.runs_per_xcd) v = xcd * a.claim.runs_per_xcd + t; else exhausted = true;
            }
            if (lane == 0) {
                ctl->run_q[fed & 3u] = v;
                __hip_atomic_store(&ctl->run_tail, fed + 1u, __ATOMIC_RELEASE, __HIP_MEMORY_SCOPE_WORKGROUP);
            }
            ++fed;
        }
    };

    const uint32_t n_slots_all = geo.nb;
    const uint32_t look_from = (role * 5u) & 15u;
    for (;;) {
        RSTAMP(2);
        unsigned long long pw = 0;
        uint32_t slot = 0;
        bool last_look = false;
        for (uint32_t spin = 0;; ++spin) {
            feed();
            unsigned long long w = 0;
            if (lane < n_slots_all) w = __hip_atomic_load(&ctl->slot[lane], __ATOMIC_RELAXED, __HIP_MEMORY_SCOPE_WORKGROUP);
            const uint32_t ready = (uint32_t)__ballot((uint32_t)(w >> 32) == kSlotReady) & 0xFFFFu;
            if (ready) {
                const uint32_t rot = ((ready >> look_from) | (ready << (16u - look_from))) & 0xFFFFu;
                slot = (uint32_t)__builtin_amdgcn_readfirstlane((int)((uint32_t)__builtin_ctz(rot) + look_from)) & 15u;
                pw = ((unsigned long long)(uint32_t)__builtin_amdgcn_readlane((int)(uint32_t)(w >> 32), (int)slot) << 32) |
                     (uint32_t)__builtin_amdgcn_readlane((int)(uint32_t)w, (int)slot);
                uint32_t won = 0;
                if (lane == 0) {
                    unsigned long long expect = pw;
                    won = __hip_atomic_compare_exchange_strong(&ctl->slot[slot], &expect, (unsigned long long)kSlotTaken << 32, __ATOMIC_ACQUIRE, __ATOMIC_RELAXED,
                                                               __HIP_MEMORY_SCOPE_WORKGROUP) ? 1u : 0u;
                }
                if ((uint32_t)__builtin_amdgcn_readfirstlane((int)won)) break;
                continue;
            }
            if (last_look) {
                RSTAMP(0); RSTAMP_WRITE(my_wave, n_done);
                return;
            }
            if (__hip_atomic_load(&ctl->live, __ATOMIC_ACQUIRE, __HIP_MEMORY_SCOPE_WORKGROUP) == 0u) {
                last_look = true;
                continue;
            }
            if (spin > kRingSpinLimit) {
                if (lane == 0) __hip_atomic_store(a.gave_up, 1u, __ATOMIC_RELAXED, __HIP_MEMORY_SCOPE_SYSTEM);
                return;
            }
            __builtin_amdgcn_s_sleep(1);
        }
        RSTAMP(0);
        const uint32_t plo = (uint32_t)pw, s = plo >> 12, tile = plo & 0xFFFu;
        const unsigned char* p = geo.ring + slot * (uint32_t)ring_slot_bytes<T>() + lane * (uint32_t)kRingRowBytes;

        {
        constexpr int OPL = 32 / D;
        constexpr int NSW = (OPL - 1) * D + T;
        constexpr int CW1 = (JS + NSW - 1) / 16;
        constexpr bool kResident = T <= 64;
        float k[kResident ? T : 1];
        if constexpr (kResident) {
#pragma unroll
            for (int t = 0; t < T; ++t) k[t] = taps[JS + t];
        }
        r_f32x2 acc[OPL];
#pragma unroll
        for (int q = 0; q < OPL; ++q) acc[q] = (r_f32x2){0.f, 0.f};
        r_f32x4 xw[2][8];
        auto rdw = [&](r_f32x4 (&x)[8], const int c) {
            const unsigned char* pc = p + coff(c);
#pragma unroll
            for (int q8 = 0; q8 < 8; ++q8) x[q8] = *reinterpret_cast<const r_f32x4*>(pc + 16 * q8);
        };
        rdw(xw[0], C0);
        if constexpr (CW1 > C0) rdw(xw[1], C0 + 1);
        ring_for_each_index([&](auto ci) {
            constexpr int c = C0 + decltype(ci)::value;
            const r_f32x4 (&x)[8] = xw[(c - C0) & 1];
            if constexpr (kResident) {
                HD_FIR_ARITH
#pragma unroll
                for (int j = 0; j < 16; ++j) {
                    const int slot_j = 16 * c + j;
                    const r_f32x2 smp = (j & 1) ? x[j >> 1].zw : x[j >> 1].xy;
#pragma unroll
                    for (int q = 0; q < OPL; ++q) {
                        const int t = slot_j - JS - D * q;
                        if (t >= 0 && t < T) acc[q] = acc[q] + smp * k[t];
                    }
                }
            } else {
                constexpr int TLO = 16 * c - JS - D * (OPL - 1) < 0 ? 0 : 16 * c - JS - D * (OPL - 1);
                constexpr int THI = 16 * c + 15 - JS >= T ? T - 1 : 16 * c + 15 - JS;
                constexpr int P0 = TLO / 2, NP = THI >= TLO ? THI / 2 - P0 + 1 : 0;
                typedef const r_f32x2 __attribute__((address_space(4)))* cpair_t;
                const cpair_t tp2 = (cpair_t)(uintptr_t)a.taps;
                r_f32x2 kp[NP > 0 ? NP : 1];
#pragma unroll
                for (int i = 0; i < NP; ++i) kp[i] = tp2[P0 + i];
                ring_for_each_index([&](auto ji) {
                    constexpr int j = decltype(ji)::value, slot_j = 16 * c + j, t0 = slot_j - JS;
                    const r_f32x2 smp = (j & 1) ? x[j >> 1].zw : x[j >> 1].xy;
                    constexpr bool odd = (t0 & 1) != 0;
                    ring_for_each_index([&](auto gi) {
                        constexpr int g = decltype(gi)::value, tg = t0 - D * 8 * g;
                        if constexpr (tg - D * 7 >= 0 && tg < T) {
                            ring_slot8<odd>(reinterpret_cast<r_f32x2 (&)[8]>(acc[8 * g]), smp, kp[(tg - 0 * D) / 2 - P0], kp[(tg - 1 * D) / 2 - P0],
                                            kp[(tg - 2 * D) / 2 - P0], kp[(tg - 3 * D) / 2 - P0], kp[(tg - 4 * D) / 2 - P0], kp[(tg - 5 * D) / 2 - P0],
                                            kp[(tg - 6 * D) / 2 - P0], kp[(tg - 7 * D) / 2 - P0]);
                        } else {
                            ring_for_each_index([&](auto qi) {
                                constexpr int q = 8 * g + decltype(qi)::value, t = t0 - D * q;
                                if constexpr (t >= 0 && t < T) ring_slot1<odd>(acc[q], smp, kp[t / 2 - P0]);
                            }, std::make_integer_sequence<int, 8>{});
                        }
                    }, std::make_integer_sequence<int, OPL / 8>{});
                }, std::make_integer_sequence<int, 16>{});
                __builtin_amdgcn_sched_barrier(0);
            }
            if constexpr (c + 2 <= CW1) rdw(xw[(c - C0) & 1], c + 2);
        }, std::make_integer_sequence<int, CW1 - C0 + 1>{});
        RSTAMP(1);
        __builtin_amdgcn_fence(__ATOMIC_RELEASE, "workgroup");
        if (lane == 0) __hip_atomic_store(&ctl->slot[slot], (unsigned long long)kSlotFree << 32, __ATOMIC_RELAXED, __HIP_MEMORY_SCOPE_WORKGROUP);
        const uint32_t o0 = (tile * 64u + lane) * (uint32_t)OPL;
        if (!a.call) {
            float2* dst = a.out + (size_t)s * a.out_stride + o0;
#pragma unroll
            for (int q = 0; q < OPL; q += 2) *reinterpret_cast<float4*>(dst + q) = make_float4(acc[q].x, acc[q].y, acc[q + 1].x, acc[q + 1].y);
        } else {
            const uint32_t pend = a.call[s].pend_before, ftake = a.call[s].fft_take, ffill = a.call[s].fft_fill;
            float2* dst = a.out + (size_t)s * a.out_stride + a.fir_hist_cap + pend + o0;
            if (((a.fir_hist_cap + pend) & 1u) == 0u) {
#pragma unroll
                for (int q = 0; q < OPL; q += 2) *reinterpret_cast<float4*>(dst + q) = make_float4(acc[q].x, acc[q].y, acc[q + 1].x, acc[q + 1].y);
            } else {
#pragma unroll
                for (int q = 0; q < OPL; ++q) dst[q] = make_float2(acc[q].x, acc[q].y);
            }
            if (a.fft_in && o0 < ftake) {
                float2* fd = a.fft_in + (size_t)s * kFftBins + ffill + o0;
                if (o0 + (uint32_t)OPL <= ftake && (ffill & 1u) == 0u) {
#pragma unroll
                    for (int q = 0; q < OPL; q += 2) *reinterpret_cast<float4*>(fd + q) = make_float4(acc[q].x, acc[q].y, acc[q + 1].x, acc[q + 1].y);
                } else {
#pragma unroll
                    for (int q = 0; q < OPL; ++q) if (o0 + (uint32_t)q < ftake) fd[q] = make_float2(acc[q].x, acc[q].y);
                }
            }
        }
        if (tile + 1 == a.ntiles) {
            const float2* in_s = a.in + (size_t)s * a.in_stride;
            float2* hout = a.hist_out + (size_t)s * (T - 1);
            for (uint32_t j = lane; j < (uint32_t)(T - 1); j += 64u) hout[j] = in_s[a.n - (T - 1) + j];
        }
        }
    }
}


template <int D> constexpr int work_row_bytes() { return D * 8 + 16; }
template <int D> constexpr int work_slot_bytes() { return 64 * work_row_bytes<D>(); }
template <int T, int D> constexpr int work_halo_rows() { return (T - 1 + D - 1) / D; }
static_assert(work_slot_bytes<32>() == kWorkSlotBytes && work_row_bytes<32>() == kRingRowBytes, "the /32 worker slot");

template <int NT>
__device__ __forceinline__ void glds16_x11(const void* base, const uint32_t* off, uint32_t lds_dst)
{
    unsigned keep, scc_keep;
#define HD_GN(n) "global_load_lds_dwordx4 %" #n ", %13 nt\n\ts_add_u32 m0, m0, 0x400\n\ts_nop 0\n\t"
#define HD_GD(n) "global_load_lds_dwordx4 %" #n ", %13\n\ts_add_u32 m0, m0, 0x400\n\ts_nop 0\n\t"
#define HD_G11_OPS : "=&s"(keep), "=&s"(scc_keep) : "v"(off[0]), "v"(off[1]), "v"(off[2]), "v"(off[3]), "v"(off[4]), "v"(off[5]), "v"(off[6]), "v"(off[7]), "v"(off[8]), "v"(off[9]), "v"(off[10]), "s"(base), "s"(lds_dst) : "memory"
#define HD_G11_HEAD "s_cselect_b32 %1, 1, 0\n\ts_mov_b32 %0, m0\n\ts_mov_b32 m0, %14\n\ts_nop 0\n\t"
#define HD_G11_TAIL "s_mov_b32 m0, %0\n\ts_cmp_lg_u32 %1, 0"
    if constexpr (NT >= 11)
        asm volatile(HD_G11_HEAD HD_GN(2) HD_GN(3) HD_GN(4) HD_GN(5) HD_GN(6) HD_GN(7) HD_GN(8) HD_GN(9) HD_GN(10) HD_GN(11) HD_GN(12) HD_G11_TAIL HD_G11_OPS);
    else
        asm volatile(HD_G11_HEAD HD_GN(2) HD_GN(3) HD_GN(4) HD_GN(5) HD_GN(6) HD_GN(7) HD_GN(8) HD_GD(9) HD_GD(10) HD_GD(11) HD_GD(12) HD_G11_TAIL HD_G11_OPS);
#undef HD_GN
#undef HD_GD
#undef HD_G11_OPS
#undef HD_G11_HEAD
#undef HD_G11_TAIL
}

template <int T, int D = 32>
__device__ __forceinline__ void ring_worker(const RingArgs& a, unsigned char* __restrict__ slot, const uint32_t role )
{
    static_assert(D == 32 || D == 64, "a row is one output's stride");
    constexpr int HR = work_halo_rows<T, D>();
    constexpr uint32_t ADV = 64u - (uint32_t)HR;
    constexpr int JS = HR * D - (T - 1);
    constexpr int NS = JS + T;
    constexpr int CPR = D / 2 + 1;
    constexpr int ROWB = work_row_bytes<D>();
    constexpr int NX = D / 2;
    constexpr int UPS = D / 32;
    constexpr int NU = (HR + 1) * UPS;
    constexpr int NB0 = ((int)ADV * CPR + 63) / 64;
    constexpr int HQ = D / 32;
    static_assert(NS == HR * D + 1, "the window ends with slot 0 of row HR");
    const uint32_t lane = threadIdx.x & 63u;
    typedef const float __attribute__((address_space(4)))* ctaps_t;
    const ctaps_t taps = (ctaps_t)(uintptr_t)a.taps - JS;
    const uint32_t dst = (uint32_t)__builtin_amdgcn_readfirstlane((int)lds_addr_of(slot));
    const unsigned char* p = slot + lane * (uint32_t)ROWB;
    const uint32_t rows = a.n / (uint32_t)D;
    RSTAMP_DECL;
    uint32_t n_done = 0; (void)n_done;

    uint32_t boff[CPR], hist_off[HR * HQ];
#pragma unroll
    for (int i = 0; i < CPR; ++i) { const uint32_t P = 64u * i + lane, row = P / (uint32_t)CPR, col = P - row * (uint32_t)CPR; boff[i] = row * (uint32_t)(D * 8) + (col < (uint32_t)(CPR - 1) ? col : (uint32_t)(CPR - 2)) * 16u; }
#pragma unroll
    for (int r = 0; r < HR * HQ; ++r) {
        const int h = (r / HQ - HR) * D + (r % HQ) * 32 + (int)(lane >> 1) + (T - 1);
        hist_off[r] = (uint32_t)(h < 0 ? 0 : h) * 8u + (lane & 1u) * 4u;
    }
    auto issue = [&](const uint32_t s, const uint32_t tile, const bool run_start) {
        const unsigned char* in_s = reinterpret_cast<const unsigned char*>(a.in + (size_t)s * a.in_stride);
        if (tile == 0) {
            const unsigned char* hb = reinterpret_cast<const unsigned char*>(a.hist_in + (size_t)s * (T - 1));
#pragma unroll
            for (int r = 0; r < HR * HQ; ++r) glds4(hb, hist_off[r], dst + (uint32_t)((r / HQ) * ROWB + (r % HQ) * 256));
#pragma unroll
            for (int i = 0; i < NB0; ++i)
                if (64 * (i + 1) <= (int)ADV * CPR || lane < (uint32_t)((int)ADV * CPR - 64 * i)) glds16(in_s, boff[i], dst + (uint32_t)(HR * ROWB) + 1024u * i);
        } else {
            const uint32_t origin = tile * ADV < rows - ADV ? tile * ADV : rows - ADV;
            const unsigned char* src = in_s + (size_t)(origin - (uint32_t)HR) * (uint32_t)(D * 8);
            if constexpr (D == 32) { if (run_start) glds16_x17<true>(src, boff, dst); else glds16_x17<false>(src, boff, dst); }
            else { glds16_x11<11>(src, boff, dst); glds16_x11<11>(src, boff + 11, dst + 11u * 1024u); glds16_x11<7>(src, boff + 22, dst + 22u * 1024u); }
        }
    };

    const uint32_t xcd0 = __builtin_amdgcn_s_getreg((3 << 11) | (0 << 6) | 20) & 15u;
    const uint32_t xcd = xcd0 < a.claim.n_xcd ? xcd0 : a.claim.n_xcd - 1;
    unsigned int* my_ctr = a.claim.ctr + (size_t)xcd * 32;
    unsigned int* next_ctr = a.claim.ctr_next + (size_t)xcd * 32;
    const uint32_t runs = a.claim.runs_per_xcd, run_len = a.claim.run_len, short_from = a.claim.short_from < runs ? a.claim.short_from : runs;
    const uint32_t tpx = a.claim.tiles_per_xcd ? a.claim.tiles_per_xcd : runs * run_len;
    auto draw = [&]() -> unsigned int { unsigned int t = 0; if (lane == 0) t = __hip_atomic_fetch_add(my_ctr, 1u, __ATOMIC_RELAXED, __HIP_MEMORY_SCOPE_AGENT); return t; };
    uint32_t s = 0, tile = 0, left = 0, this_run = 0;
    auto take_run = [&](const unsigned int ticket) -> bool {
        const uint32_t t = (uint32_t)__builtin_amdgcn_readfirstlane((int)ticket);
        if (t == runs && lane == 0) (void)__hip_atomic_exchange(next_ctr, 0u, __ATOMIC_RELAXED, __HIP_MEMORY_SCOPE_AGENT);
        if (t >= runs) return false;
        const uint32_t g0 = xcd * tpx + (t < short_from ? t * run_len : short_from * run_len + (t - short_from));
        s = g0 / a.ntiles; tile = g0 - s * a.ntiles; left = this_run = t < short_from ? run_len : 1u;
        return true;
    };
    auto advance = [&]() { ++tile; --left; if (tile == a.ntiles) { tile = 0; ++s; } };

    asm volatile("s_waitcnt lgkmcnt(0)" ::: "memory");
    if (!take_run(draw())) { RSTAMP_WRITE(role, 0); return; }
    uint32_t cs = s, ct = tile;
    issue(cs, ct, true); advance();
    unsigned int ticket = 0;
    if (!left) ticket = draw();

    auto ldk = [&](r_f32x2 (&k)[8], auto cc) {
        constexpr int c = decltype(cc)::value;
#pragma unroll
        for (int j = 0; j < 16; j += 2) {
            k[j >> 1].x = (16 * c + j >= JS && 16 * c + j < NS) ? taps[16 * c + j] : 0.f;
            k[j >> 1].y = (16 * c + j + 1 >= JS && 16 * c + j + 1 < NS) ? taps[16 * c + j + 1] : 0.f;
        }
    };
    for (;;) {
        RSTAMP(2);
        asm volatile("s_waitcnt vmcnt(0)" ::: "memory");
        asm volatile("" : "+v"(ticket));
        RSTAMP(0);
        r_f32x2 kk[2][2][8];
        r_f32x4 x[NX];
#pragma unroll
        for (int q = 0; q < NX; ++q) x[q] = *reinterpret_cast<const r_f32x4*>(p + 16 * q);
        ldk(kk[0][0], std::integral_constant<int, 0>{}); ldk(kk[0][1], std::integral_constant<int, 1>{});
        __builtin_amdgcn_sched_barrier(0);
#pragma unroll
        for (int q = 0; q < NX; q += 8)
            asm volatile("" : "+v"(x[q]), "+v"(x[q + 1]), "+v"(x[q + 2]), "+v"(x[q + 3]), "+v"(x[q + 4]), "+v"(x[q + 5]), "+v"(x[q + 6]), "+v"(x[q + 7]) :: "memory");
        RSTAMP(3);
        bool more = true;
        if (!left) more = take_run(ticket);
        uint32_t ns = 0, nt = 0;
        if (more) {
            ns = s; nt = tile;
            issue(ns, nt, left == this_run); advance();
            if (!left) ticket = draw();
        }
        RSTAMP(4);

        const uint32_t origin = ct * ADV < rows - ADV ? ct * ADV : rows - ADV;
        r_f32x2 acc = {0.f, 0.f};
#ifdef HD_FAST_ARITH
        r_f32x2 acc_b = {0.f, 0.f};
#endif
        auto mac_chunk = [&](const r_f32x2 (&k)[8], auto cc) {
            constexpr int c = decltype(cc)::value, j0 = JS > 16 * c ? JS - 16 * c : 0, j1 = NS < 16 * c + 16 ? NS - 16 * c : 16;
            const r_f32x4 (&xh)[8] = reinterpret_cast<const r_f32x4 (&)[8]>(x[8 * (c % (D / 16))]);
#ifdef HD_FAST_ARITH
            if constexpr (j0 == 0 && j1 == 16) ring_fma16x2(acc, acc_b, xh, k);
            else {
#pragma unroll
                for (int j = j0; j < j1; ++j) {
                    const r_f32x2 smp = (j & 1) ? xh[j >> 1].zw : xh[j >> 1].xy;
                    const float kj = (j & 1) ? k[j >> 1].y : k[j >> 1].x;
                    if (j & 1) acc_b = __builtin_elementwise_fma(smp, (r_f32x2){kj, kj}, acc_b);
                    else acc = __builtin_elementwise_fma(smp, (r_f32x2){kj, kj}, acc);
                }
            }
#else
            if constexpr (j0 == 0 && j1 == 16) ring_mac16_asm(acc, xh, k);
            else {
#pragma unroll
                for (int j = j0; j < j1; ++j) {
                    const r_f32x2 smp = (j & 1) ? xh[j >> 1].zw : xh[j >> 1].xy;
                    acc = acc + smp * ((j & 1) ? k[j >> 1].y : k[j >> 1].x);
                }
            }
#endif
        };
        auto rot1 = [&](r_f32x2& v) {
            const float re = v.x, im = v.y;
            v.x = __builtin_bit_cast(float, __builtin_amdgcn_update_dpp(0, __builtin_bit_cast(int, re), 0x13C, 0xF, 0xF, false));
            v.y = __builtin_bit_cast(float, __builtin_amdgcn_update_dpp(0, __builtin_bit_cast(int, im), 0x13C, 0xF, 0xF, false));
        };
        auto rot = [&]() {
            rot1(acc);
#ifdef HD_FAST_ARITH
            rot1(acc_b);
#endif
        };
        auto arrived = [&](const r_f32x2 (&k)[2][8]) {
            asm volatile("" :: "s"(k[0][0]), "s"(k[0][1]), "s"(k[0][2]), "s"(k[0][3]), "s"(k[0][4]), "s"(k[0][5]), "s"(k[0][6]), "s"(k[0][7]),
                               "s"(k[1][0]), "s"(k[1][1]), "s"(k[1][2]), "s"(k[1][3]), "s"(k[1][4]), "s"(k[1][5]), "s"(k[1][6]), "s"(k[1][7]));
        };
        ring_for_each_index([&](auto ui) {
            constexpr int u = decltype(ui)::value;
            arrived(kk[u & 1]);
            if constexpr (u + 1 < NU) {
                ldk(kk[(u + 1) & 1][0], std::integral_constant<int, 2 * u + 2>{});
                ldk(kk[(u + 1) & 1][1], std::integral_constant<int, 2 * u + 3>{});
            }
            __builtin_amdgcn_sched_barrier(0);
            if constexpr (JS < 32 * u + 16 && 32 * u < NS) mac_chunk(kk[u & 1][0], std::integral_constant<int, 2 * u>{});
            if constexpr (32 * u + 16 < NS && JS < 32 * u + 32) mac_chunk(kk[u & 1][1], std::integral_constant<int, 2 * u + 1>{});
            if constexpr ((u + 1) % UPS == 0 && u + 1 < NU) rot();
        }, std::make_integer_sequence<int, NU>{});
#ifdef HD_FAST_ARITH
        acc = acc + acc_b;
#endif
#ifdef HD_STAMP_RING
        asm volatile("" : "+v"(acc));
        ++n_done;
#endif
        RSTAMP(1);
        if (lane >= (uint32_t)HR) a.out[(size_t)cs * a.out_stride + origin + lane - (uint32_t)HR] = make_float2(acc.x, acc.y);
        if (ct + 1 == a.ntiles) {
            const float2* in_s = a.in + (size_t)cs * a.in_stride + (a.n - (uint32_t)(T - 1));
            float2* hout = a.hist_out + (size_t)cs * (T - 1);
            constexpr int NH = (T - 1 + 63) / 64;
            float2 h[NH];
#pragma unroll
            for (int k = 0; k < NH; ++k) h[k] = in_s[lane + 64u * k < (uint32_t)(T - 1) ? lane + 64u * k : 0u];
#pragma unroll
            for (int k = 0; k < NH; ++k) if (lane + 64u * k < (uint32_t)(T - 1)) hout[lane + 64u * k] = h[k];
        }
        if (!more) break;
        cs = ns; ct = nt;
    }
    RSTAMP(2);
    RSTAMP_WRITE(role, n_done);
}

}
}
```

Baseline: 491,400.

## Chain consecutive stage-1 ring tiles to carry halo accumulators through LDS

Adds a chained tile schedule for the ratio-32 stage-1 ring decimator. Consecutive tiles in a run pass their partial halo accumulators through a small per-worker LDS keep area instead of reloading and recomputing the overlapping halo rows. Each chained tile advances by a full 64 rows rather than 64 minus the halo, which cuts redundant input loads and FMAs. In exchange it adds a more complex ticket schedule mixing chained and plain streams, LDS keep and dump buffers, and extra DPP and LDS traffic per rotation step.

```diff
diff --git a/habdec_amd/csrc/engine.cpp b/habdec_amd/csrc/engine.cpp
--- a/habdec_amd/csrc/engine.cpp
+++ b/habdec_amd/csrc/engine.cpp
@@ -139,7 +139,9 @@
     uint32_t step_run = 0;
     bool no_cu_step = false;
     uint32_t ring_run = 0;
+    uint32_t ring_chain = 1;
     uint32_t ring_short_pct = 25;
+    bool ring_short_set = false;
     static constexpr uint32_t kS1Loaders = 2;
 #ifndef HD_S1_SLOTS_BATCH
 #define HD_S1_SLOTS_BATCH 4
@@ -325,7 +327,8 @@
     if (const char* v = getenv("HD_STEP_RUN")) e->step_run = (uint32_t)atoi(v);
     e->no_cu_step = getenv("HD_NO_CU_STEP") != nullptr;
     if (const char* v = getenv("HD_RING_RUN")) e->ring_run = (uint32_t)atoi(v);
-    if (const char* v = getenv("HD_RING_SHORT_PCT")) e->ring_short_pct = std::min<uint32_t>((uint32_t)atoi(v), 100u);
+    if (const char* v = getenv("HD_RING_CHAIN")) e->ring_chain = atoi(v) ? 1u : 0u;
+    if (const char* v = getenv("HD_RING_SHORT_PCT")) { e->ring_short_pct = std::min<uint32_t>((uint32_t)atoi(v), 100u); e->ring_short_set = true; }
     if (const char* v = getenv("HD_TAIL_MAX_N2")) e->tail_max_n2 = (uint32_t)strtoul(v, nullptr, 0);
     {
         hipDeviceProp_t prop;
@@ -987,6 +990,17 @@
             const uint32_t tpx = claim.runs_per_xcd * run_len, whole = (uint32_t)((uint64_t)tpx * (100u - e->ring_short_pct) / 100u) / run_len;
             claim.tiles_per_xcd = tpx; claim.short_from = whole; claim.runs_per_xcd = whole + (tpx - whole * run_len);
         }
+        if (run_len_cu && R1 == 32 && e->ring_chain && S % n_xcd == 0) {
+            const uint32_t hr = (uint32_t)((T1 - 1 + 31) / 32), rows = p.max_in / 32u, rl = e->ring_run >= 2u ? e->ring_run : 4u, sx = (uint32_t)(S / n_xcd);
+            const hd::RingSchedule ch = hd::ring_schedule(rows, hr, rl, true), pl = hd::ring_schedule(rows, hr, 1u, false);
+            const uint32_t sp = hd::ring_plain_streams(sx, e->ring_short_set ? e->ring_short_pct : 12u);
+            if (ch.chained && pl.ntiles && (uint64_t)sx * pl.ntiles < (1ull << 31)) {
+                claim.chain_rl = ch.rl; claim.chain_sx = sx; claim.chain_sc = sx - sp;
+                claim.chain_nfull = ch.n_full; claim.chain_kclose = ch.k_close; claim.chain_ntp = pl.ntiles;
+                claim.runs_per_xcd = hd::ring_tickets(ch, pl, sx, sx - sp);
+                claim.run_len = ch.rl; claim.short_from = 0xFFFFFFFFu; claim.tiles_per_xcd = 0;
+            }
+        }
     }
     return claim;
 }
diff --git a/habdec_amd/csrc/host/ring_schedule.hpp b/habdec_amd/csrc/host/ring_schedule.hpp
--- /dev/null
+++ b/habdec_amd/csrc/host/ring_schedule.hpp
@@ -0,0 +1,94 @@
+#pragma once
+#include <stdint.h>
+
+namespace hd {
+
+struct RingTile {
+    int32_t row0;
+    uint32_t out0, out_n;
+    bool chained;
+    bool last;
+};
+
+struct RingSchedule {
+    uint32_t rows = 0, hr = 0;
+    uint32_t rl = 1;
+    uint32_t n_full = 0;
+    uint32_t k_close = 0;
+    uint32_t run_out = 0;
+    int32_t close_row0 = 0;
+    uint32_t nruns = 0;
+    uint32_t ntiles = 0;
+    bool chained = false;
+};
+
+constexpr RingSchedule ring_schedule(uint32_t rows, uint32_t hr, uint32_t run_len, bool chained)
+{
+    RingSchedule s{};
+    if (rows < 64u || rows > (1u << 30) || hr == 0u || hr >= 32u || run_len == 0u || run_len > 4096u) return s;
+    s.rows = rows; s.hr = hr;
+    const uint32_t adv = 64u - hr;
+    uint32_t rl = run_len < rows / 64u ? run_len : rows / 64u;
+    if (!chained || rl < 2u) {
+        s.rl = 1u; s.run_out = adv; s.ntiles = s.nruns = (rows + adv - 1u) / adv;
+        return s;
+    }
+    s.chained = true; s.rl = rl; s.run_out = 64u * rl - hr;
+    s.n_full = rows / s.run_out;
+    const uint32_t rem = rows - s.n_full * s.run_out;
+    s.k_close = rem ? (rem + hr + 63u) / 64u : 0u;
+    s.close_row0 = (int32_t)rows - (int32_t)(64u * s.k_close);
+    s.nruns = s.n_full + (s.k_close ? 1u : 0u);
+    s.ntiles = s.n_full * rl + s.k_close;
+    return s;
+}
+
+constexpr uint32_t ring_run_tiles(const RingSchedule& s, uint32_t r) { return s.chained ? (r < s.n_full ? s.rl : s.k_close) : 1u; }
+constexpr uint32_t ring_run_first(const RingSchedule& s, uint32_t r) { return s.chained ? r * s.rl : r; }
+constexpr int32_t ring_plain_row0(uint32_t rows, uint32_t hr, uint32_t tile)
+{
+    const uint32_t adv = 64u - hr, o = tile * adv < rows - adv ? tile * adv : rows - adv;
+    return (int32_t)o - (int32_t)hr;
+}
+constexpr int32_t ring_run_row0(const RingSchedule& s, uint32_t r)
+{
+    if (!s.chained) return ring_plain_row0(s.rows, s.hr, r);
+    return r < s.n_full ? (int32_t)(r * s.run_out) - (int32_t)s.hr : s.close_row0;
+}
+
+constexpr RingTile ring_tile(const RingSchedule& s, uint32_t k)
+{
+    RingTile t{};
+    t.last = k + 1u == s.ntiles;
+    if (!s.chained) {
+        t.row0 = ring_plain_row0(s.rows, s.hr, k);
+        t.out0 = (uint32_t)(t.row0 + (int32_t)s.hr); t.out_n = 64u - s.hr; t.chained = false;
+        return t;
+    }
+    const uint32_t r = k < s.n_full * s.rl ? k / s.rl : s.n_full, j = k - r * s.rl;
+    t.row0 = ring_run_row0(s, r) + (int32_t)(64u * j);
+    t.chained = j != 0u;
+    t.out0 = (uint32_t)(t.row0 + (int32_t)(t.chained ? 0u : s.hr)); t.out_n = t.chained ? 64u : 64u - s.hr;
+    return t;
+}
+
+struct RingTicket { uint32_t stream , tile , ntiles; int32_t row0; bool plain; };
+constexpr uint32_t ring_tickets(const RingSchedule& ch, const RingSchedule& pl, uint32_t sx, uint32_t sc) { return sc * ch.nruns + (sx - sc) * pl.ntiles; }
+constexpr uint32_t ring_tiles_total(const RingSchedule& ch, const RingSchedule& pl, uint32_t sx, uint32_t sc) { return sc * ch.ntiles + (sx - sc) * pl.ntiles; }
+constexpr RingTicket ring_ticket(const RingSchedule& ch, const RingSchedule& pl, uint32_t sc, uint32_t t)
+{
+    RingTicket k{};
+    const uint32_t nch = sc * ch.nruns;
+    if (t < nch) {
+        k.stream = t / ch.nruns;
+        const uint32_t r = t - k.stream * ch.nruns;
+        k.tile = ring_run_first(ch, r); k.ntiles = ring_run_tiles(ch, r); k.row0 = ring_run_row0(ch, r); k.plain = false;
+    } else {
+        const uint32_t u = t - nch, sl = u / pl.ntiles;
+        k.stream = sc + sl; k.tile = u - sl * pl.ntiles; k.ntiles = 1u; k.row0 = ring_plain_row0(pl.rows, pl.hr, k.tile); k.plain = true;
+    }
+    return k;
+}
+constexpr uint32_t ring_plain_streams(uint32_t sx, uint32_t short_pct) { return (uint32_t)(((uint64_t)sx * (short_pct > 100u ? 100u : short_pct) + 50u) / 100u); }
+
+}
diff --git a/habdec_amd/csrc/kernels/decimate.hip b/habdec_amd/csrc/kernels/decimate.hip
--- a/habdec_amd/csrc/kernels/decimate.hip
+++ b/habdec_amd/csrc/kernels/decimate.hip
@@ -548,7 +548,9 @@
 {
     extern __shared__ __attribute__((aligned(16))) unsigned char cu_lds[];
     RingCtl* ctl = reinterpret_cast<RingCtl*>(cu_lds);
-    unsigned char* slots = cu_lds + kRingCtlBytes;
+    unsigned char* keeps = cu_lds + 256;
+    unsigned char* dump = keeps + 4 * kWorkKeepBytes;
+    unsigned char* slots = cu_lds + kStepCtlBytes;
     unsigned char* tails = slots + 4 * kWorkSlotBytes;
     ring_ctl_init(ctl, 0u);
     __syncthreads();
@@ -571,7 +573,7 @@
         w = (uint32_t)__builtin_amdgcn_readfirstlane((int)pick);
     }
     if (w < 4u) {
-        ring_worker<T>(ra, slots + w * (uint32_t)kWorkSlotBytes, w);
+        ring_worker<T>(ra, slots + w * (uint32_t)kWorkSlotBytes, keeps + w * (uint32_t)kWorkKeepBytes, dump, w);
     } else {
         const uint32_t k = w - 4u, lane = threadIdx.x & 63u;
         const uint32_t s = blockIdx.x * 4u + k;
@@ -583,7 +585,8 @@
             }
             if (call_copy && lane < 4) reinterpret_cast<uint4*>(call_copy + s)[lane] = reinterpret_cast<const uint4*>(call + s)[lane];
         }
-        ring_worker<T>(ra, n_tail ? tails + k * tail_bytes : slots + w * (uint32_t)kWorkSlotBytes, w);
+        ring_worker<T>(ra, n_tail ? tails + k * tail_bytes : slots + w * (uint32_t)kWorkSlotBytes,
+                       n_tail ? tails + k * tail_bytes + (uint32_t)kWorkSlotBytes : slots + 8u * (uint32_t)kWorkSlotBytes + k * (uint32_t)kWorkKeepBytes, dump, w);
     }
 }
 
@@ -592,7 +595,9 @@
 {
     extern __shared__ __attribute__((aligned(16))) unsigned char cu_lds[];
     if constexpr (D == 32 || D == 64) {
-        ring_worker<T, D>(ra, cu_lds + (threadIdx.x >> 6) * (uint32_t)work_slot_bytes<D>(), threadIdx.x >> 6);
+        unsigned char* keeps = cu_lds + 8u * (uint32_t)work_slot_bytes<D>();
+        ring_worker<T, D>(ra, cu_lds + (threadIdx.x >> 6) * (uint32_t)work_slot_bytes<D>(), D == 32 ? keeps + (threadIdx.x >> 6) * (uint32_t)kWorkKeepBytes : nullptr,
+                          D == 32 ? keeps + 8 * kWorkKeepBytes : nullptr, threadIdx.x >> 6);
     } else {
     unsigned char* ring = cu_lds;
     RingCtl* ctl = reinterpret_cast<RingCtl*>(cu_lds + n_slots * ring_slot_bytes<T>());
@@ -771,10 +776,21 @@
     return ntiles && ntiles <= 4096u && claim.run_len && ntiles % claim.run_len == 0 && total < (1ull << 24) && total / ntiles <= (1ull << 20);
 }
 
+static bool ring_chain_ok(int ratio, int ntaps, uint32_t n, const StepClaim& claim, uint32_t n_streams)
+{
+    if (ratio != 32 || claim.chain_rl < 2u || !claim.n_xcd || !claim.chain_sx || claim.chain_sc > claim.chain_sx) return false;
+    const uint32_t hr = (uint32_t)((ntaps - 1 + ratio - 1) / ratio), rows = n / (uint32_t)ratio;
+    const RingSchedule ch = ring_schedule(rows, hr, claim.chain_rl, true), pl = ring_schedule(rows, hr, 1u, false);
+    if (!ch.chained || ch.rl != claim.chain_rl || ch.n_full != claim.chain_nfull || ch.k_close != claim.chain_kclose || pl.ntiles != claim.chain_ntp) return false;
+    if (!ch.ntiles || !pl.ntiles || (n_streams && (uint64_t)claim.chain_sx * claim.n_xcd != n_streams)) return false;
+    return (uint64_t)claim.chain_sx * (ch.ntiles > pl.ntiles ? ch.ntiles : pl.ntiles) * claim.n_xcd < (1ull << 32) &&
+           claim.runs_per_xcd == ring_tickets(ch, pl, claim.chain_sx, claim.chain_sc);
+}
+
 uint32_t step_cu_tail_lds(int ratio, int ntaps)
 {
     if (ratio != 32 || (ntaps != 212 && ntaps != 174)) return 0;
-    return ((163840u - (uint32_t)kRingCtlBytes - 4u * (uint32_t)kWorkSlotBytes) / 4u) & ~15u;
+    return ((163840u - (uint32_t)kStepCtlBytes - 4u * (uint32_t)kWorkSlotBytes) / 4u) & ~15u;
 }
 
 bool launch_step_cu(hipStream_t st, int ratio, int ntaps, int ratio2, int ntaps2, uint32_t n_streams, uint32_t n_cus, const float2* in, size_t in_stride,
@@ -784,13 +800,13 @@
 {
     if (ratio != 32 || !claim.ctr || !uniform_n || uniform_n % 2048u) return false;
     const uint32_t ntiles = ring_tiles(ratio, ntaps, uniform_n);
-    if (!ring_limits_ok(ntiles, claim, true)) return false;
-    if (tail_bytes < (uint32_t)kWorkSlotBytes) tail_bytes = (uint32_t)kWorkSlotBytes;
+    if (claim.chain_rl ? !ring_chain_ok(ratio, ntaps, uniform_n, claim, n_streams) : !ring_limits_ok(ntiles, claim, true)) return false;
+    if (tail_bytes < (uint32_t)(kWorkSlotBytes + kWorkKeepBytes)) tail_bytes = (uint32_t)(kWorkSlotBytes + kWorkKeepBytes);
     tail_bytes = (tail_bytes + 15u) & ~15u;
     RingArgs ra{in, in_stride, hist_in, hist_out, taps, out, out_stride, uniform_n, ntiles, claim, nullptr, nullptr, 0u, nullptr};
 #define HD_CU_CASE(T, D2, T2)                                                                                                         \
     if (ntaps == T && ratio2 == D2 && ntaps2 == T2) {                                                                                 \
-        const uint32_t lds = (uint32_t)kRingCtlBytes + (n_tail ? 4u * (uint32_t)kWorkSlotBytes + 4u * tail_bytes : 8u * (uint32_t)kWorkSlotBytes); \
+        const uint32_t lds = (uint32_t)kStepCtlBytes + (n_tail ? 4u * (uint32_t)kWorkSlotBytes + 4u * tail_bytes : 8u * (uint32_t)kWorkSlotBytes + 4u * (uint32_t)kWorkKeepBytes); \
         if (lds > 163840u) return false;                                                                                              \
         static bool attr_set[64] = {};                              \
         int dev_ = 0;                                                                                                                 \
@@ -833,14 +849,14 @@
     if (n_waves < 8u || n_waves > 16u) n_waves = 8u;
     if (!claim.ctr || !uniform_n || uniform_n % 2048u) return false;
     const uint32_t ntiles = ring_tiles(ratio, ntaps, uniform_n);
-    if (!ring_limits_ok(ntiles, claim, ratio >= 32)) return false;
+    if (claim.chain_rl ? !ring_chain_ok(ratio, ntaps, uniform_n, claim, 0u) : !ring_limits_ok(ntiles, claim, ratio >= 32)) return false;
     if ((ratio <= 4) != (final_call != nullptr)) return false;
     RingArgs ra{in, in_stride, hist_in, hist_out, taps, out, out_stride, uniform_n, ntiles, claim, gave_up, final_call, fir_hist_cap, fft_in};
 #define HD_S1_CASE(D, T)                                                                                                              \
     if (ratio == D && ntaps == T) {                                                                                                   \
         static_assert(D >= 32 || (uint32_t)ring_bytes<T, kRingNSLAlone>() <= 163840u, "eight tile slots must fit a CU's LDS");       \
         const uint32_t workers = D == 32 ? 8u : n_slots <= 4u ? 3u : 4u;             \
-        const uint32_t lds = D >= 32 ? workers * (uint32_t)work_slot_bytes<(D >= 32 ? D : 32)>() : n_slots * (uint32_t)ring_slot_bytes<T>() + (uint32_t)kRingCtlBytes; \
+        const uint32_t lds = D >= 32 ? workers * (uint32_t)work_slot_bytes<(D >= 32 ? D : 32)>() + (D == 32 ? (workers + 1u) * (uint32_t)kWorkKeepBytes : 0u) : n_slots * (uint32_t)ring_slot_bytes<T>() + (uint32_t)kRingCtlBytes; \
         static bool attr_set[64] = {};                                                                                                \
         int dev_ = 0;                                                                                                                 \
         if (hipGetDevice(&dev_) != hipSuccess || dev_ < 0 || dev_ >= 64) return false;                                                \
diff --git a/habdec_amd/csrc/kernels/launch.h b/habdec_amd/csrc/kernels/launch.h
--- a/habdec_amd/csrc/kernels/launch.h
+++ b/habdec_amd/csrc/kernels/launch.h
@@ -4,6 +4,7 @@
 #include <stdint.h>
 
 #include "../dev_types.h"
+#include "../host/ring_schedule.hpp"
 
 namespace hd {
 
@@ -18,6 +19,8 @@
     unsigned int* ctr_next = nullptr;
     uint32_t n_xcd = 0, runs_per_xcd = 0, run_len = 0;
     uint32_t short_from = 0xFFFFFFFFu, tiles_per_xcd = 0;
+    uint32_t chain_rl = 0, chain_sx = 0, chain_sc = 0;
+    uint32_t chain_nfull = 0, chain_kclose = 0, chain_ntp = 0;
 };
 
 struct TailArgs {
diff --git a/habdec_amd/csrc/kernels/stage1_ring.h b/habdec_amd/csrc/kernels/stage1_ring.h
--- a/habdec_amd/csrc/kernels/stage1_ring.h
+++ b/habdec_amd/csrc/kernels/stage1_ring.h
@@ -13,6 +13,8 @@
 constexpr int kRingRowBytes = 272;
 constexpr int kRingNSLAlone = 4;
 constexpr int kWorkSlotBytes = 64 * kRingRowBytes;
+constexpr int kWorkKeepBytes = 128;
+constexpr int kStepCtlBytes = 256 + 5 * kWorkKeepBytes;
 constexpr int kRingCtlBytes = 384;
 constexpr uint32_t kRingSpinLimit = 1u << 22;
 template <int T> constexpr int ring_halo_rows() { return (T - 1 + 31) / 32; }
@@ -111,7 +113,7 @@
                  : "=&s"(keep) : "v"(off), "s"(base), "s"(lds_dst) : "memory");
 }
 
-template <bool HEAD_KEPT = false >
+template <int POLICY = 0>
 __device__ __forceinline__ void glds16_x17(const void* base, const uint32_t (&off)[17], uint32_t lds_dst)
 {
     unsigned keep, scc_keep;
@@ -122,7 +124,11 @@
                    : "v"(off[0]), "v"(off[1]), "v"(off[2]), "v"(off[3]), "v"(off[4]), "v"(off[5]), "v"(off[6]), "v"(off[7]), "v"(off[8]), "v"(off[9]),              \
                      "v"(off[10]), "v"(off[11]), "v"(off[12]), "v"(off[13]), "v"(off[14]), "v"(off[15]), "v"(off[16]), "s"(base), "s"(lds_dst)                      \
                    : "memory"
-    if constexpr (HEAD_KEPT)
+    if constexpr (POLICY == 2)
+        asm volatile("s_cselect_b32 %1, 1, 0\n\ts_mov_b32 %0, m0\n\ts_mov_b32 m0, %20\n\ts_nop 0\n\t"
+                     HD_G1(2) HD_G1(3) HD_G1(4) HD_G1(5) HD_G1(6) HD_G1(7) HD_G1(8) HD_G1(9) HD_G1(10) HD_G1(11) HD_G1(12) HD_G1(13) HD_G1(14) HD_G1(15) HD_G1(16) HD_G1(17)
+                     "global_load_lds_dwordx4 %18, %19" HD_GLDS_BODY_POLICY "\n\ts_mov_b32 m0, %0\n\ts_cmp_lg_u32 %1, 0" HD_G17_OPS);
+    else if constexpr (POLICY == 1)
         asm volatile("s_cselect_b32 %1, 1, 0\n\ts_mov_b32 %0, m0\n\ts_mov_b32 m0, %20\n\ts_nop 0\n\t"
                      HD_G1D(2) HD_G1D(3) HD_G1(4) HD_G1(5) HD_G1(6) HD_G1(7) HD_G1(8) HD_G1(9) HD_G1(10) HD_G1(11) HD_G1(12) HD_G1(13) HD_G1(14) HD_G1(15) HD_G1(16) HD_G1D(17)
                      "global_load_lds_dwordx4 %18, %19\n\ts_mov_b32 m0, %0\n\ts_cmp_lg_u32 %1, 0" HD_G17_OPS);
@@ -616,7 +622,9 @@
 }
 
 template <int T, int D = 32>
-__device__ __forceinline__ void ring_worker(const RingArgs& a, unsigned char* __restrict__ slot, const uint32_t role )
+__device__ __forceinline__ void ring_worker(const RingArgs& a, unsigned char* __restrict__ slot, unsigned char* keep_lds ,
+                                            unsigned char* dump_lds ,
+                                            const uint32_t role )
 {
     static_assert(D == 32 || D == 64, "a row is one output's stride");
     constexpr int HR = work_halo_rows<T, D>();
@@ -648,9 +656,9 @@
         const int h = (r / HQ - HR) * D + (r % HQ) * 32 + (int)(lane >> 1) + (T - 1);
         hist_off[r] = (uint32_t)(h < 0 ? 0 : h) * 8u + (lane & 1u) * 4u;
     }
-    auto issue = [&](const uint32_t s, const uint32_t tile, const bool run_start) {
+    auto issue = [&](const uint32_t s, const int32_t row0, const bool run_start, const bool chained) {
         const unsigned char* in_s = reinterpret_cast<const unsigned char*>(a.in + (size_t)s * a.in_stride);
-        if (tile == 0) {
+        if (row0 < 0) {
             const unsigned char* hb = reinterpret_cast<const unsigned char*>(a.hist_in + (size_t)s * (T - 1));
 #pragma unroll
             for (int r = 0; r < HR * HQ; ++r) glds4(hb, hist_off[r], dst + (uint32_t)((r / HQ) * ROWB + (r % HQ) * 256));
@@ -658,9 +666,8 @@
             for (int i = 0; i < NB0; ++i)
                 if (64 * (i + 1) <= (int)ADV * CPR || lane < (uint32_t)((int)ADV * CPR - 64 * i)) glds16(in_s, boff[i], dst + (uint32_t)(HR * ROWB) + 1024u * i);
         } else {
-            const uint32_t origin = tile * ADV < rows - ADV ? tile * ADV : rows - ADV;
-            const unsigned char* src = in_s + (size_t)(origin - (uint32_t)HR) * (uint32_t)(D * 8);
-            if constexpr (D == 32) { if (run_start) glds16_x17<true>(src, boff, dst); else glds16_x17<false>(src, boff, dst); }
+            const unsigned char* src = static_cast<const unsigned char*>(uniform_ptr(in_s + (size_t)(uint32_t)row0 * (uint32_t)(D * 8)));
+            if constexpr (D == 32) { if (chained) glds16_x17<2>(src, boff, dst); else if (run_start) glds16_x17<1>(src, boff, dst); else glds16_x17<0>(src, boff, dst); }
             else { glds16_x11<11>(src, boff, dst); glds16_x11<11>(src, boff + 11, dst + 11u * 1024u); glds16_x11<7>(src, boff + 22, dst + 22u * 1024u); }
         }
     };
@@ -672,21 +679,55 @@
     const uint32_t runs = a.claim.runs_per_xcd, run_len = a.claim.run_len, short_from = a.claim.short_from < runs ? a.claim.short_from : runs;
     const uint32_t tpx = a.claim.tiles_per_xcd ? a.claim.tiles_per_xcd : runs * run_len;
     auto draw = [&]() -> unsigned int { unsigned int t = 0; if (lane == 0) t = __hip_atomic_fetch_add(my_ctr, 1u, __ATOMIC_RELAXED, __HIP_MEMORY_SCOPE_AGENT); return t; };
-    uint32_t s = 0, tile = 0, left = 0, this_run = 0;
+    constexpr bool CH = D == 32;
+    const bool chain_mode = CH && a.claim.chain_rl >= 2u;
+    uint32_t s = 0, left = 0, this_run = 0;
+    int32_t row0 = 0;
     auto take_run = [&](const unsigned int ticket) -> bool {
         const uint32_t t = (uint32_t)__builtin_amdgcn_readfirstlane((int)ticket);
         if (t == runs && lane == 0) (void)__hip_atomic_exchange(next_ctr, 0u, __ATOMIC_RELAXED, __HIP_MEMORY_SCOPE_AGENT);
         if (t >= runs) return false;
+        auto uni = [](const uint32_t v) { return (uint32_t)__builtin_amdgcn_readfirstlane((int)v); };
+        if (chain_mode) {
+            RingSchedule ch{}, pl{};
+            ch.rows = pl.rows = rows; ch.hr = pl.hr = (uint32_t)HR;
+            ch.chained = true; ch.rl = a.claim.chain_rl; ch.n_full = a.claim.chain_nfull; ch.k_close = a.claim.chain_kclose; ch.run_out = 64u * ch.rl - (uint32_t)HR;
+            ch.close_row0 = (int32_t)rows - (int32_t)(64u * ch.k_close); ch.nruns = ch.n_full + (ch.k_close ? 1u : 0u); ch.ntiles = ch.n_full * ch.rl + ch.k_close;
+            pl.run_out = ADV; pl.ntiles = pl.nruns = a.claim.chain_ntp;
+            const RingTicket k = ring_ticket(ch, pl, a.claim.chain_sc, t);
+            s = uni(xcd * a.claim.chain_sx + k.stream); left = this_run = uni(k.ntiles); row0 = (int32_t)uni((uint32_t)k.row0);
+            return true;
+        }
         const uint32_t g0 = xcd * tpx + (t < short_from ? t * run_len : short_from * run_len + (t - short_from));
-        s = g0 / a.ntiles; tile = g0 - s * a.ntiles; left = this_run = t < short_from ? run_len : 1u;
+        s = uni(g0 / a.ntiles); left = this_run = t < short_from ? run_len : 1u;
+        row0 = (int32_t)uni((uint32_t)ring_plain_row0(rows, (uint32_t)HR, g0 - s * a.ntiles));
         return true;
     };
-    auto advance = [&]() { ++tile; --left; if (tile == a.ntiles) { tile = 0; ++s; } };
+    auto advance = [&]() {
+        --left;
+        if (chain_mode) row0 += 64;
+        else if (row0 + 64 == (int32_t)rows) { ++s; row0 = -HR; }
+        else row0 = row0 + (int32_t)ADV < (int32_t)rows - 64 ? row0 + (int32_t)ADV : (int32_t)rows - 64;
+    };
+    auto tile_here = [&]() -> uint32_t { return s | ((chain_mode && left != this_run) ? 0x80000000u : 0u); };
 
     asm volatile("s_waitcnt lgkmcnt(0)" ::: "memory");
     if (!take_run(draw())) { RSTAMP_WRITE(role, 0); return; }
-    uint32_t cs = s, ct = tile;
-    issue(cs, ct, true); advance();
+    uint32_t cs = tile_here();
+    int32_t crow0 = row0;
+    issue(s, crow0, true, false); advance();
+#ifdef HD_FAST_ARITH
+    typedef r_f32x4 kept_t;
+#else
+    typedef r_f32x2 kept_t;
+#endif
+    static_assert(!CH || sizeof(kept_t) * HR <= (size_t)kWorkKeepBytes, "the keep area");
+    uint32_t kept_at = CH ? lds_addr_of(keep_lds) : 0u;
+    if constexpr (CH) asm volatile("" : "+v"(kept_at));
+    typedef kept_t __attribute__((address_space(3)))* kept_ptr_t;
+    const kept_ptr_t kept = (kept_ptr_t)kept_at;
+    uint32_t kept_to = CH ? (lane == 63u ? lds_addr_of(keep_lds) : lds_addr_of(dump_lds)) : 0u;
+    const kept_ptr_t kept_w = (kept_ptr_t)kept_to;
     unsigned int ticket = 0;
     if (!left) ticket = draw();
 
@@ -715,15 +756,15 @@
         RSTAMP(3);
         bool more = true;
         if (!left) more = take_run(ticket);
-        uint32_t ns = 0, nt = 0;
+        uint32_t ns = 0;
+        int32_t nrow0 = 0;
         if (more) {
-            ns = s; nt = tile;
-            issue(ns, nt, left == this_run); advance();
+            ns = tile_here(); nrow0 = row0;
+            issue(s, nrow0, left == this_run, (ns >> 31) != 0u); advance();
             if (!left) ticket = draw();
         }
         RSTAMP(4);
 
-        const uint32_t origin = ct * ADV < rows - ADV ? ct * ADV : rows - ADV;
         r_f32x2 acc = {0.f, 0.f};
 #ifdef HD_FAST_ARITH
         r_f32x2 acc_b = {0.f, 0.f};
@@ -753,15 +794,25 @@
             }
 #endif
         };
-        auto rot1 = [&](r_f32x2& v) {
-            const float re = v.x, im = v.y;
-            v.x = __builtin_bit_cast(float, __builtin_amdgcn_update_dpp(0, __builtin_bit_cast(int, re), 0x13C, 0xF, 0xF, false));
-            v.y = __builtin_bit_cast(float, __builtin_amdgcn_update_dpp(0, __builtin_bit_cast(int, im), 0x13C, 0xF, 0xF, false));
+        kept_t kin{}, kout{};
+        auto rot1 = [&](r_f32x2& v, const r_f32x2 k0) {
+            const float re = v.x, im = v.y, kre = k0.x, kim = k0.y;
+            if constexpr (CH) {
+                v.x = __builtin_bit_cast(float, __builtin_amdgcn_update_dpp(__builtin_bit_cast(int, kre), __builtin_bit_cast(int, re), 0x138, 0xF, 0xF, false));
+                v.y = __builtin_bit_cast(float, __builtin_amdgcn_update_dpp(__builtin_bit_cast(int, kim), __builtin_bit_cast(int, im), 0x138, 0xF, 0xF, false));
+            } else {
+                v.x = __builtin_bit_cast(float, __builtin_amdgcn_update_dpp(0, __builtin_bit_cast(int, re), 0x13C, 0xF, 0xF, false));
+                v.y = __builtin_bit_cast(float, __builtin_amdgcn_update_dpp(0, __builtin_bit_cast(int, im), 0x13C, 0xF, 0xF, false));
+            }
         };
         auto rot = [&]() {
-            rot1(acc);
 #ifdef HD_FAST_ARITH
-            rot1(acc_b);
+            if constexpr (CH) kout = (kept_t){acc.x, acc.y, acc_b.x, acc_b.y};
+            rot1(acc, kin.xy);
+            rot1(acc_b, kin.zw);
+#else
+            if constexpr (CH) kout = acc;
+            rot1(acc, kin);
 #endif
         };
         auto arrived = [&](const r_f32x2 (&k)[2][8]) {
@@ -775,6 +826,8 @@
                 ldk(kk[(u + 1) & 1][0], std::integral_constant<int, 2 * u + 2>{});
                 ldk(kk[(u + 1) & 1][1], std::integral_constant<int, 2 * u + 3>{});
             }
+            if constexpr (CH && u % UPS == 0 && u > 0) kept_w[u / UPS - 1] = kout;
+            if constexpr (CH && (u + 1) % UPS == 0 && u + 1 < NU) kin = kept[(u + 1) / UPS - 1];
             __builtin_amdgcn_sched_barrier(0);
             if constexpr (JS < 32 * u + 16 && 32 * u < NS) mac_chunk(kk[u & 1][0], std::integral_constant<int, 2 * u>{});
             if constexpr (32 * u + 16 < NS && JS < 32 * u + 32) mac_chunk(kk[u & 1][1], std::integral_constant<int, 2 * u + 1>{});
@@ -788,10 +841,11 @@
         ++n_done;
 #endif
         RSTAMP(1);
-        if (lane >= (uint32_t)HR) a.out[(size_t)cs * a.out_stride + origin + lane - (uint32_t)HR] = make_float2(acc.x, acc.y);
-        if (ct + 1 == a.ntiles) {
-            const float2* in_s = a.in + (size_t)cs * a.in_stride + (a.n - (uint32_t)(T - 1));
-            float2* hout = a.hist_out + (size_t)cs * (T - 1);
+        const uint32_t cstream = cs & 0x7FFFFFFFu;
+        if (lane >= (uint32_t)HR || (cs >> 31)) a.out[(size_t)cstream * a.out_stride + (size_t)(uint32_t)(crow0 + (int32_t)lane)] = make_float2(acc.x, acc.y);
+        if (crow0 + 64 == (int32_t)rows) {
+            const float2* in_s = a.in + (size_t)cstream * a.in_stride + (a.n - (uint32_t)(T - 1));
+            float2* hout = a.hist_out + (size_t)cstream * (T - 1);
             constexpr int NH = (T - 1 + 63) / 64;
             float2 h[NH];
 #pragma unroll
@@ -800,7 +854,7 @@
             for (int k = 0; k < NH; ++k) if (lane + 64u * k < (uint32_t)(T - 1)) hout[lane + 64u * k] = h[k];
         }
         if (!more) break;
-        cs = ns; ct = nt;
+        cs = ns; crow0 = nrow0;
     }
     RSTAMP(2);
     RSTAMP_WRITE(role, n_done);
```

Result: faster. 506,900, median of 6 (+3.2%).
